# Tomeu7/AO-MARL

Measured on AMD Instinct MI355X. Metric: env steps/sec (AO frames/sec), higher is better.
Workload: dtype f32

## Files before the change

### ao_marl_amd/agents.py

```python
import math
from collections import OrderedDict

import numpy as np
import torch

LOG_SIG_MIN = -20.0


class AgentLayout(object):

    def __init__(self, nmodes, n_zernike_start_end, n_agents_modal, include_tip_tilt=True,
                 window_n_zernike=-1, include_tip_tilt_windowed=False, n_filtered=0,
                 state_keys=("dm_history_2", "dm_history_1", "dm_before_linear", "dm_residual"),
                 state_block=None):
        lo, hi = n_zernike_start_end
        assert lo > -1 and hi > -1 and hi > lo
        total_controlled = hi - lo
        assert total_controlled % n_agents_modal == 0
        local = total_controlled // n_agents_modal
        self.nmodes = nmodes
        self.start = lo
        self.local_controlled_modes = local
        self.agents = OrderedDict()
        wid = 1
        for m in range(lo, hi, local):
            self.agents[wid] = (m, m + local)
            wid += 1
        self.include_tip_tilt = include_tip_tilt
        if include_tip_tilt:
            self.agents[wid] = (nmodes - 2, nmodes)
            total_controlled += 2
        self.total_controlled_modes = total_controlled
        self.n_agents = len(self.agents)
        self.window = window_n_zernike
        self.block = state_block if state_block is not None else \
            (nmodes if window_n_zernike > -1 else total_controlled)
        self.state_keys = tuple(state_keys)
        self.indices_of_state = OrderedDict()
        o = 0
        for k in self.state_keys:
            self.indices_of_state[k] = (o, o + self.block)
            o += self.block
        self.state_dim = o
        if window_n_zernike > -1:
            self.modes_chosen = self._windowed(window_n_zernike, include_tip_tilt_windowed,
                                               n_filtered)
        else:
            self.modes_chosen = self._original()
        self.action_slices = OrderedDict()
        for w, (a, b) in self.agents.items():
            if include_tip_tilt and (a, b) == (nmodes - 2, nmodes):
                self.action_slices[w] = (total_controlled - 2, total_controlled)
            else:
                self.action_slices[w] = (a - lo, b - lo)
        self.action_dim = total_controlled
        self.action_modes = np.r_[np.arange(lo, hi), [nmodes - 2, nmodes - 1]] \
            if include_tip_tilt else np.arange(lo, hi)

    def _original(self):
        out = OrderedDict()
        for w, (a, b) in self.agents.items():
            if self.include_tip_tilt and (a, b) == (self.nmodes - 2, self.nmodes):
                bot, top = self.total_controlled_modes - 2 - self.start, \
                    self.total_controlled_modes - self.start
            else:
                bot, top = a - self.start, b - self.start
            parts = []
            for k, (s0, s1) in self.indices_of_state.items():
                if k in "wfs":
                    parts.append(np.arange(s0, s1))
                else:
                    parts.append(np.arange(s0 + bot, s0 + top))
            out[w] = np.concatenate(parts)
        return out

    def _windowed(self, w_n, tt_windowed, n_filtered):
        out = OrderedDict()
        n_ag = len(self.agents)
        for w, (a, b) in self.agents.items():
            parts = []
            if self.include_tip_tilt and w == n_ag:
                for k, (s0, s1) in self.indices_of_state.items():
                    if k in "wfs":
                        parts.append(np.arange(s0, s1))
                    else:
                        idx = np.arange(s1 - 2, s1)
                        if tt_windowed:
                            idx = np.concatenate([idx, np.arange(0, int(2 * w_n))])
                        parts.append(idx)
                out[w] = np.concatenate(parts)
                break
            for k, (s0, s1) in self.indices_of_state.items():
                if k in "wfs":
                    parts.append(np.arange(s0, s1))
                    continue
                end_point = s1 - (n_filtered - 2)
                length = end_point - s0
                if a - w_n < 0:
                    diff = a - w_n
                    ini, end = 0, b + w_n - diff
                elif b + w_n > length:
                    diff = b + w_n - length
                    ini, end = a - int(w_n) - diff, length
                else:
                    ini, end = a - w_n, b + w_n
                parts.append(np.arange(s0 + ini, s0 + end))
            out[w] = np.concatenate(parts)
        return out

    def state_shapes(self):
        return [len(v) for v in self.modes_chosen.values()]

    def action_shapes(self):
        return [b - a for (a, b) in self.agents.values()]


def _xavier_uniform(gen, fan_out, fan_in, gain=1.0):
    a = gain * math.sqrt(6.0 / (fan_in + fan_out))
    return (torch.rand(fan_out, fan_in, generator=gen) * 2 - 1) * a


class BatchedGaussianPolicy(object):

    def __init__(self, layout, hidden=256, num_layers=2, log_sig_max=2.0, action_scale=1.0,
                 action_bias=0.0, last_layer_zero=True, seed=1234, device="cuda:0"):
        self.layout, self.H, self.L = layout, hidden, num_layers
        self.log_sig_max, self.scale, self.bias = log_sig_max, action_scale, action_bias
        self.device = torch.device(device)
        ins, acts = layout.state_shapes(), layout.action_shapes()
        A, in_max, act_max = layout.n_agents, max(ins), max(acts)
        self.A, self.in_max, self.act_max = A, in_max, act_max
        g = torch.Generator().manual_seed(seed)
        W1 = torch.zeros(A, in_max, hidden)
        Wh = [torch.zeros(A, hidden, hidden) for _ in range(num_layers - 1)]
        Wm, Ws = torch.zeros(A, hidden, act_max), torch.zeros(A, hidden, act_max)
        gather = torch.full((A, in_max), layout.state_dim, dtype=torch.long)
        for i, (w, idx) in enumerate(layout.modes_chosen.items()):
            W1[i, :ins[i], :] = _xavier_uniform(g, hidden, ins[i]).T
            for h in Wh:
                h[i] = _xavier_uniform(g, hidden, hidden).T
            if not last_layer_zero:
                Wm[i, :, :acts[i]] = _xavier_uniform(g, acts[i], hidden).T
                Ws[i, :, :acts[i]] = _xavier_uniform(g, acts[i], hidden).T
            gather[i, :ins[i]] = torch.as_tensor(idx, dtype=torch.long)
        dev = self.device
        self.W1, self.Wh, self.Wm, self.Ws = W1.to(dev), [h.to(dev) for h in Wh], Wm.to(dev), \
            Ws.to(dev)
        self.b1 = torch.zeros(A, 1, hidden, device=dev)
        self.bh = [torch.zeros(A, 1, hidden, device=dev) for _ in range(num_layers - 1)]
        self.bm = torch.zeros(A, 1, act_max, device=dev)
        self.bs = torch.zeros(A, 1, act_max, device=dev)
        self.gather = gather.to(dev)
        ag = torch.zeros(layout.action_dim, dtype=torch.long)
        lo = torch.zeros(layout.action_dim, dtype=torch.long)
        for i, (w, (a, b)) in enumerate(layout.action_slices.items()):
            ag[a:b] = i
            lo[a:b] = torch.arange(b - a)
        self.sc_agent, self.sc_local = ag.to(dev), lo.to(dev)
        self.gen = torch.Generator(device=dev).manual_seed(seed)
        self.gather_i32 = self.gather.to(torch.int32).contiguous()
        self.sc_agent_i32, self.sc_local_i32 = self.sc_agent.to(torch.int32), self.sc_local.to(torch.int32)
        self.seed, self._draws = int(seed), 0
        self._native = None
        self.use_native = self.device.type == "cuda"
        self.native_forward, self._desc = True, None
        self.layer_by_layer = False

    def _refresh_native(self):
        t = lambda w: w.transpose(1, 2).contiguous()
        self._native = dict(
                W1=t(self.W1), b1=self.b1[:, 0].contiguous(),
                Wh=[t(w) for w in self.Wh], bh=[b[:, 0].contiguous() for b in self.bh],
                Whead=torch.cat([t(self.Wm), t(self.Ws)], dim=1).contiguous(),
                bhead=torch.cat([self.bm[:, 0], self.bs[:, 0]], dim=1).contiguous())

    def load_agent(self, i, state_dict):
        ins, acts = self.layout.state_shapes()[i], self.layout.action_shapes()[i]
        with torch.no_grad():
            self.W1[i].zero_()
            self.W1[i, :ins] = state_dict["linear1.weight"].T.to(self.device)
            self.b1[i, 0] = state_dict["linear1.bias"].to(self.device)
            for j in range(self.L - 1):
                self.Wh[j][i] = state_dict["hidden.%d.weight" % j].T.to(self.device)
                self.bh[j][i, 0] = state_dict["hidden.%d.bias" % j].to(self.device)
            self.Wm[i].zero_(); self.Ws[i].zero_()
            self.Wm[i, :, :acts] = state_dict["mean_linear.weight"].T.to(self.device)
            self.Ws[i, :, :acts] = state_dict["log_std_linear.weight"].T.to(self.device)
            self.bm[i, 0, :acts] = state_dict["mean_linear.bias"].to(self.device)
            self.bs[i, 0, :acts] = state_dict["log_std_linear.bias"].to(self.device)
        self._native = None

    def split_states(self, state):
        if self.use_native and not state.requires_grad:
            from . import libaomarl as la
            return la.split_states(state.to(torch.float32), self.gather_i32)
        padded = torch.cat([state, state.new_zeros(state.shape[0], 1)], dim=1)
        return padded[:, self.gather].permute(1, 0, 2).contiguous()

    def _native_head(self, state):
        from . import libaomarl as la
        if self._native is None:
            self._refresh_native()
        n = self._native
        x = self.split_states(state.to(torch.float32))
        x = la.linear_batched(x, n["W1"], n["b1"], relu=True)
        for W, b in zip(n["Wh"], n["bh"]):
            x = la.linear_batched(x, W, b, relu=True)
        return la.linear_batched(x, n["Whead"], n["bhead"], relu=False)

    def _actor_desc(self, nenv):
        from . import libaomarl as la
        import ctypes as C
        if self._native is None:
            self._refresh_native()
        if self._desc is not None and self._desc[0].nenv == nenv and self._desc[4] is self._native and \
                bool(self._desc[0].flags) == self.layer_by_layer:
            return self._desc[0]
        n, A, H = self._native, self.A, self.H
        d = la.ActorDesc()
        d.n_agents, d.nenv, d.state_dim, d.in_max, d.act_max = A, nenv, self.layout.state_dim, \
            self.in_max, self.act_max
        d.hidden, d.n_hidden, d.action_dim = H, self.L, self.layout.action_dim
        z = lambda *sh: torch.empty(*sh, dtype=torch.float32, device=self.device)
        scratch = dict(x=z(A, nenv, self.in_max), h0=z(A, nenv, H), h1=z(A, nenv, H),
                       head=z(A, nenv, 2 * self.act_max))
        nh = max(self.L - 1, 1)
        Wh = (C.c_void_p * nh)(*[w.data_ptr() for w in n["Wh"]])
        bh = (C.c_void_p * nh)(*[b.data_ptr() for b in n["bh"]])
        d.gather, d.W1, d.b1 = self.gather_i32.data_ptr(), n["W1"].data_ptr(), n["b1"].data_ptr()
        d.Wh, d.bh = Wh, bh
        d.Whead, d.bhead = n["Whead"].data_ptr(), n["bhead"].data_ptr()
        d.sc_agent, d.sc_local = self.sc_agent_i32.data_ptr(), self.sc_local_i32.data_ptr()
        d.log_sig_min, d.log_sig_max, d.scale, d.bias = LOG_SIG_MIN, self.log_sig_max, self.scale, self.bias
        for k, t in scratch.items():
            setattr(d, k, t.data_ptr())
        d.flags = la.ACTOR_LAYER_BY_LAYER if self.layer_by_layer else 0
        tiled = None
        if not self.layer_by_layer and H % 16 == 0:
            tiled = dict(W1=la.tile_weights(n["W1"]), Wh=[la.tile_weights(w) for w in n["Wh"]],
                         Whead=la.tile_weights(n["Whead"]))
            tiled["ptrs"] = (C.c_void_p * nh)(*[w.data_ptr() for w in tiled["Wh"]])
            d.W1_tiled, d.Wh_tiled, d.Whead_tiled = tiled["W1"].data_ptr(), tiled["ptrs"], \
                tiled["Whead"].data_ptr()
        self._desc = (d, scratch, Wh, bh, n, tiled)
        return d

    out_ring, _ring, _ring_i = 0, None, 0

    def reset_output_ring(self):
        self._ring_i = 0

    def _select_action_one_call(self, state, eval_mode, eps, out=None):
        from . import libaomarl as la
        import ctypes as C
        nenv = state.shape[0]
        d = self._actor_desc(nenv)
        self._draws += 1
        if self.out_ring:
            if self._ring is None or self._ring[0][0].shape[0] != nenv:
                self._ring = [(torch.empty(nenv, self.layout.action_dim, dtype=torch.float32, device=self.device),
                               torch.empty(nenv, self.layout.action_dim, dtype=torch.float32, device=self.device))
                              for _ in range(self.out_ring)]
                self._ring_i = 0
            a, m = self._ring[self._ring_i]
            self._ring_i = (self._ring_i + 1) % self.out_ring
        else:
            a = torch.empty(nenv, self.layout.action_dim, dtype=torch.float32, device=self.device)
            m = torch.empty_like(a)
        if out is not None:
            if out.shape != a.shape or out.dtype != torch.float32 or not out.is_contiguous() or out.device != a.device:
                raise ValueError("select_action: out must be a contiguous float32 [nenv, action_dim] tensor on the policy's device")
            if eval_mode:
                m = out
            else:
                a = out
        if eps is not None:
            eps = eps.to(torch.float32).contiguous()
        la.check(la.load().aomarl_actor_forward(
                C.byref(d), state.data_ptr(), eps.data_ptr() if eps is not None else None,
                self.seed & 0xFFFFFFFF, self._draws & 0xFFFFFFFF, a.data_ptr(), m.data_ptr(),
                la.raw_stream(self.device)))
        return (m if eval_mode else a), m

    def forward(self, state):
        if self.use_native:
            head = self._native_head(state)
            mean = head[:, :, :self.act_max]
            log_std = head[:, :, self.act_max:].clamp(LOG_SIG_MIN, self.log_sig_max)
            return mean, log_std
        x = self.split_states(state.to(torch.float32))
        x = torch.relu(torch.baddbmm(self.b1, x, self.W1))
        for W, b in zip(self.Wh, self.bh):
            x = torch.relu(torch.baddbmm(b, x, W))
        mean = torch.baddbmm(self.bm, x, self.Wm)
        log_std = torch.baddbmm(self.bs, x, self.Ws).clamp(LOG_SIG_MIN, self.log_sig_max)
        return mean, log_std

    def _assemble(self, per_agent):
        return per_agent[self.sc_agent, :, self.sc_local].T.contiguous()

    def select_action(self, state, eval_mode=False, eps=None, out=None):
        if self.use_native and self.native_forward and state.dtype == torch.float32 and \
                state.dim() == 2 and state.shape[1] == self.layout.state_dim:
            return self._select_action_one_call(state if state.is_contiguous() else state.contiguous(), eval_mode, eps, out)
        a, m = self._select_action(state, eval_mode, eps)
        if out is not None:
            out.copy_(a)
            a = out
        return a, m

    @torch.no_grad()
    def _select_action(self, state, eval_mode=False, eps=None):
        if self.use_native and self.native_forward and state.dtype == torch.float32 and \
                state.dim() == 2 and state.shape[1] == self.layout.state_dim:
            return self._select_action_one_call(state.contiguous(), eval_mode, eps)
        if self.use_native:
            from . import libaomarl as la
            head = self._native_head(state)
            self._draws += 1
            a, m = la.policy_sample(head, self.act_max, self.sc_agent_i32, self.sc_local_i32,
                                    LOG_SIG_MIN, self.log_sig_max, self.scale, self.bias, self.seed,
                                    self._draws, eps=eps)
            return (m if eval_mode else a), m
        mean, log_std = self.forward(state)
        if eps is None:
            e = torch.randn(mean.shape, generator=self.gen, device=self.device)
        else:
            e = torch.zeros_like(mean)
            e[self.sc_agent, :, self.sc_local] = eps.T
        x_t = mean + log_std.exp() * e
        action = torch.tanh(x_t) * self.scale + self.bias
        mu = torch.tanh(mean) * self.scale + self.bias
        a, m = self._assemble(action), self._assemble(mu)
        return (m if eval_mode else a), m


class BatchedQNetwork(object):

    def __init__(self, layout, hidden=256, extra_hidden=0, seed=4321, device="cuda:0"):
        self.layout, self.device = layout, torch.device(device)
        ins, acts = layout.state_shapes(), layout.action_shapes()
        A = layout.n_agents
        self.in_max, self.act_max = max(ins), max(acts)
        g = torch.Generator().manual_seed(seed)
        dev = self.device

        def stack(fan_in_list, fan_out, pad_in):
            W = torch.zeros(A, pad_in, fan_out)
            for i, fi in enumerate(fan_in_list):
                W[i, :fi] = _xavier_uniform(g, fan_out, fi).T
            return W.to(dev)

        self.q = []
        for _ in range(2):
            Win = torch.zeros(A, self.in_max + self.act_max, hidden)
            for i in range(A):
                w = _xavier_uniform(g, hidden, ins[i] + acts[i]).T
                Win[i, :ins[i]] = w[:ins[i]]
                Win[i, self.in_max:self.in_max + acts[i]] = w[ins[i]:]
            hid = [stack([hidden] * A, hidden, hidden) for _ in range(extra_hidden)]
            out = stack([hidden] * A, 1, hidden)
            self.q.append((Win.to(dev), hid, out))

    @torch.no_grad()
    def forward(self, split_state, split_action):
        x = torch.cat([split_state, split_action], dim=2)
        res = []
        for Win, hid, out in self.q:
            h = torch.relu(torch.bmm(x, Win))
            for W in hid:
                h = torch.relu(torch.bmm(h, W))
            res.append(torch.bmm(h, out))
        return res[0], res[1]
```

### ao_marl_amd/csrc/aomarl_capi.hip

```cpp
#include "aomarl_kernels.hip"
#include "aomarl_qf4_host.h"
#include "aomarl_step_plan_host.h"

#include <math.h>
#include <stdlib.h>
#include <stdarg.h>
#include <stdio.h>
#include <string.h>

#include <algorithm>
#include <climits>
#include <string>
#include <vector>

static thread_local char g_err[512] = "";

int fail(const char *fmt, ...) {
  va_list ap;
  va_start(ap, fmt);
  vsnprintf(g_err, sizeof(g_err), fmt, ap);
  va_end(ap);
  return 1;
}


struct aomarl_ctx {
  DevSys sys;
  std::vector<void *> owned;
  int nlayers = 0, ndm = 0;
  int dim[AOMARL_MAX_LAYERS], ns[AOMARL_MAX_LAYERS], abclass[AOMARL_MAX_LAYERS];
  float deltax[AOMARL_MAX_LAYERS], deltay[AOMARL_MAX_LAYERS];
  int nclass = 0;
  int maxdim = 0, maxK = 0;
  float gain = 0.f, delay = 0.f;
  bool spot_fast = false;
  bool force_generic_dm = false, force_valu_target = false;
  bool force_generic_spot = false, force_generic_target = false, force_unfused_frame = false;
  int dft_mode = -1;
  bool reset_untransposed = false;
  int small_chain = 1;
  hipEvent_t ride_ev = nullptr;
  bool rode = false;
  int residual_shortcut = 0;
  int small_move = 1;
  bool small_ok = false;
  int reset_streams = 2;
  bool reset_prefetch_whole = true;
  hipEvent_t ev_reset = nullptr, ev_reset2[3] = {nullptr, nullptr, nullptr};
  bool no_extrude_sg = false;
  bool defer_dm_shape = false;
  int fused_debug = 0;
  bool prefetch_atmos = false, premoved = false;
  bool frame_wait_pending = false;
  bool screens_dirty_main = true;
  float cmat_scale = 1.f, v2m_scale = 1.f, m2v_scale = 1.f, s2m_scale = 1.f, ab_scale[AOMARL_MAX_LAYERS] = {1.f, 1.f, 1.f, 1.f, 1.f, 1.f, 1.f, 1.f};
  bool subpixel_flow = false;
  float frac_x[AOMARL_MAX_LAYERS] = {0, 0, 0, 0, 0, 0, 0, 0}, frac_y[AOMARL_MAX_LAYERS] = {0, 0, 0, 0, 0, 0, 0, 0};
  bool graph_step = false, capturing = false, side_joined = false, fork_recorded = false;
  hipEvent_t ev_fork = nullptr;
  struct StepGraph { std::vector<long long> key; hipGraphExec_t exec; hipGraph_t graph; unsigned long long arith[AR_N]; int fw_variant[6]; };
  std::vector<StepGraph> graphs;
  unsigned long long graph_hits = 0, graph_captures = 0;
  unsigned long long cfg_epoch = 0;
  const int32_t *sel_checked = nullptr;
  int sel_checked_n = 0, sel_checked_nm = 0;
  int fw_variant[6] = {0, 0, 0, 0, 0, 0};
  char fw_name[96] = {0};
  bool time_fw = false;
  std::vector<hipEvent_t> fw_ev;
  size_t fw_ev_used = 0;
  std::vector<hipEvent_t> fw_ev_retired;
  hipStream_t atm_stream = nullptr, psf_stream = nullptr;
  hipEvent_t ev_frame = nullptr, ev_moved = nullptr, ev_psf = nullptr;
  hipEvent_t ev_frame_cur = nullptr;
  bool frame_marked = false;
  struct FramePipe {
    bool have_twin = false, active = false;
    const float *owner_screens = nullptr;
    aomarl_state twin;
    int par = 0;
    hipStream_t fstream = nullptr;
    hipEvent_t ev_cmd = nullptr, ev_commit = nullptr, ev_done[2] = {nullptr, nullptr}, ev_psf[2] = {nullptr, nullptr};
    hipEvent_t ev_done_cur[2] = {nullptr, nullptr};
    bool psf_out[2] = {false, false};
    bool cmd_covers_commit = false;
    bool cmd_covers_psf = false;
    int32_t *snap[2] = {nullptr, nullptr};
    size_t snap_ints = 0;
    unsigned long long steps = 0, overlapped = 0, behind = 0;
  } pipe;
  int32_t *snap_target = nullptr;
  bool snap_complete = false;
  bool pipe_enabled = true;
  bool pipe_internal = false;
  hipEvent_t ev_frame_prev = nullptr;
  bool need_prev = false, group_overlap = false;
  bool psf_side = false;
  const float *pre_screens = nullptr;
  int pre_b = 0, pre_n = 0;
  float *cmat = nullptr;
  int ld_cmat = 0;
  int nmodes = 0, nact = 0, ld_v2m = 0, ld_m2v = 0;
  float *v2m = nullptr, *m2v = nullptr, *freedom = nullptr;
  float *s2m = nullptr;
  int s2m_nmodes = 0;
  int32_t *amodes = nullptr, *amode_inv = nullptr;
  float *env_gain = nullptr;
  int env_gain_n = 0;
  float *mgain = nullptr;
  int mgain_rows = 0, mgain_nm = 0;
  std::vector<float> h_mgain;
  uint32_t *seed_stage = nullptr;
  int seed_stage_n = 0;
  struct ResetPrefetch *rp = nullptr;
  float *timg = nullptr;
  std::vector<int32_t> h_grid;
  std::vector<float> h_prof, h_spupil, h_tt;
  float *geoW = nullptr, *geoUx = nullptr, *geoUy = nullptr, *geoPlanes = nullptr;
  int32_t *geoMap = nullptr;
  int geo_ldw = 0, geo_gw = 0, geo_gh = 0, geo_npzt = 0, geo_ldr = 0;
};

static int pipe_drop(aomarl_ctx *c, void *stream);
static void rp_free(aomarl_ctx *c);
static int fw_ev_rewind(aomarl_ctx *c) {
  const hipEvent_t held[4] = {c->pipe.ev_done_cur[0], c->pipe.ev_done_cur[1], c->ev_frame_cur, c->ev_frame_prev};
  for (size_t i = 0; i < c->fw_ev.size(); i++)
    for (int k = 0; k < 4; k++)
      if (held[k] && c->fw_ev[i] == held[k]) {
        hipEvent_t ne;
        HIPCHK(hipEventCreate(&ne));
        c->fw_ev_retired.push_back(c->fw_ev[i]);
        c->fw_ev[i] = ne;
        break;
      }
  if (c->fw_ev_retired.size() > 64 && !c->pipe.active) {
    bool live = false;
    for (hipEvent_t e : c->fw_ev_retired) for (int k = 0; k < 4; k++) live = live || e == held[k];
    if (!live) { for (hipEvent_t e : c->fw_ev_retired) (void)hipEventDestroy(e); c->fw_ev_retired.clear(); }
  }
  c->fw_ev_used = 0;
  return 0;
}
static int frame_fused_impl(aomarl_ctx *c, aomarl_state *st, int b, int n, int flags, void *stream, int slot);
static int next_part_one_sense(aomarl_ctx *c, aomarl_state *st, int b, int n, float *accumx, float *accumy, int image_flags, void *stream);

static unsigned long long g_cfg_epoch = 0;
const char *aomarl_last_error(void) { return g_err; }
int aomarl_abi_version(void) { return AOMARL_ABI_VERSION; }

int aomarl_set_precision(int mode) {
  g_cfg_epoch++;
  if (mode != AOMARL_PRECISION_F32 && mode != AOMARL_PRECISION_SPLIT_F16) return fail("set_precision: unknown mode %d", mode);
  g_precision = mode;
  g_gemm.split_f16 = mode == AOMARL_PRECISION_SPLIT_F16;
  return 0;
}
int aomarl_get_precision(void) { return g_precision; }
int aomarl_gemm_saturated(unsigned *count, void *stream) {
  if (!count) return fail("gemm_saturated: null argument");
  *count = 0;
  int dev = 0;
  HIPCHK(hipGetDevice(&dev));
  if (dev < 0 || dev >= 64 || !g_gemm_sat[dev]) return 0;
  hipStream_t s = (hipStream_t)stream;
  HIPCHK(hipMemcpyAsync(count, g_gemm_sat[dev], sizeof(unsigned), hipMemcpyDeviceToHost, s));
  HIPCHK(hipStreamSynchronize(s));
  if (*count) HIPCHK(hipMemsetAsync(g_gemm_sat[dev], 0, sizeof(unsigned), s));
  return 0;
}
int aomarl_arith_families(void) { return AR_N; }
const char *aomarl_arith_family_name(int i) { return (i >= 0 && i < AR_N) ? g_arith_name[i] : ""; }
unsigned long long aomarl_arith_launches(int i) { return (i >= 0 && i < AR_N) ? g_arith[i] : 0ULL; }
void aomarl_arith_reset(void) { for (int i = 0; i < AR_N; i++) g_arith[i] = 0ULL; }

template <typename T>
static int upload(aomarl_ctx *c, const T *host, size_t n, T **dev) {
  *dev = nullptr;
  if (n == 0) return 0;
  if (!host) return fail("null host array in descriptor");
  void *p = nullptr;
  HIPCHK(hipMalloc(&p, n * sizeof(T)));
  c->owned.push_back(p);
  HIPCHK(hipMemcpy(p, host, n * sizeof(T), hipMemcpyHostToDevice));
  *dev = (T *)p;
  return 0;
}

static bool is_int(float v) { return floorf(v) == v; }

int aomarl_create(const aomarl_desc *d, aomarl_ctx **out) {
  if (!d || !out) return fail("aomarl_create: null argument");
  if (d->abi_version != AOMARL_ABI_VERSION)
    return fail("aomarl_create: ABI version %d, library is %d", d->abi_version, AOMARL_ABI_VERSION);
  if (d->nlayers < 0 || d->nlayers > AOMARL_MAX_LAYERS) return fail("nlayers out of range");
// ... 684 lines not shown
```

### ao_marl_amd/csrc/aomarl_capi_agents.hip

```cpp
__global__ void k_split_states(int nenv, int state_dim, int in_max, const int32_t *__restrict__ gather,
                               const float *__restrict__ state, float *__restrict__ out) {
  const int a = blockIdx.z, e = blockIdx.y, k = blockIdx.x * blockDim.x + threadIdx.x;
  if (k >= in_max) return;
  const int g = gather[a * in_max + k];
  out[((long long)a * nenv + e) * in_max + k] = g < state_dim ? state[(long long)e * state_dim + g] : 0.f;
}

__global__ void k_policy_sample(int nenv, int act_max, int action_dim, const float *__restrict__ head,
                                float ls_min, float ls_max, float scale, float bias,
                                const int32_t *__restrict__ sc_agent, const int32_t *__restrict__ sc_local,
                                const float *__restrict__ eps_in, uint32_t seed, uint32_t counter,
                                float *__restrict__ action, float *__restrict__ mean) {
  const int e = blockIdx.y, g = blockIdx.x * blockDim.x + threadIdx.x;
  if (g >= action_dim) return;
  const int a = sc_agent[g], l = sc_local[g];
  const float *h = head + ((long long)a * nenv + e) * (2 * act_max);
  const float m = h[l];
  const float ls = fminf(fmaxf(h[act_max + l], ls_min), ls_max);
  const float eps = eps_in ? eps_in[(long long)e * action_dim + g]
                           : philox_normal(seed, 7u, counter, (uint32_t)e, (uint32_t)g);
  const float x = m + expf(ls) * eps;
  action[(long long)e * action_dim + g] = tanhf(x) * scale + bias;
  mean[(long long)e * action_dim + g] = tanhf(m) * scale + bias;
}

struct ActorArgs {
  int A, nenv, state_dim, in_max, act_max, H, n_hidden, action_dim;
  const int32_t *gather;
  const float *W1, *b1, *Wh[8], *bh[8], *Whead, *bhead;
  const int32_t *sc_agent, *sc_local;
  float ls_min, ls_max, scale, bias;
  const float *state, *eps;
  uint32_t seed, counter;
  float *action, *mean;
};

__global__ void k_actor_tile_weights(int N, int K, int ntile, int ksteps, const float *__restrict__ src,
                                     float *__restrict__ dst) {
  const long long per = (long long)ntile * ksteps * 256;
  const long long i = (long long)blockIdx.x * blockDim.x + threadIdx.x;
  if (i >= per) return;
  const int a = blockIdx.y;
  const int jj = (int)(i & 3), lane = (int)((i >> 2) & 63);
  const long long t = i >> 8;
  const int sidx = (int)(t % ksteps), n = (int)(t / ksteps);
  const int row = 16 * n + (lane & 15), col = 16 * sidx + 4 * (lane >> 4) + jj;
  dst[(long long)a * per + i] = (row < N && col < K) ? src[((long long)a * N + row) * K + col] : 0.f;
}

__device__ __forceinline__ int af_at(int row, int col) {
  return (((col >> 4) * 64 + ((col >> 2) & 3) * 16 + row) << 2) + (col & 3);
}

__device__ __forceinline__ void af_layer(const float *__restrict__ Xs, int ksteps, const float *__restrict__ W,
                                         const float *__restrict__ b, int N, bool relu, float *__restrict__ Out) {
  const int lane = threadIdx.x & 63, wave = threadIdx.x >> 6, r = lane & 15, kk = lane >> 4;
  const int ntile = (N + 15) / 16, npairs = (ntile + 1) / 2;
  constexpr int D = 2;
  for (int pair = wave; pair < npairs; pair += 8) {
    const float4 *wa = reinterpret_cast<const float4 *>(W) + (long long)(2 * pair) * ksteps * 64 + lane;
    const float4 *wb = reinterpret_cast<const float4 *>(W) + (long long)min(2 * pair + 1, ntile - 1) * ksteps * 64 + lane;
    const float4 *xs = reinterpret_cast<const float4 *>(Xs) + lane;
    f32x4 acc0 = {0.f, 0.f, 0.f, 0.f}, acc1 = {0.f, 0.f, 0.f, 0.f};
    auto fma8 = [&](const float4 x, const float4 a, const float4 c) {
      acc0 = __builtin_amdgcn_mfma_f32_16x16x4f32(x.x, a.x, acc0, 0, 0, 0);
      acc1 = __builtin_amdgcn_mfma_f32_16x16x4f32(x.x, c.x, acc1, 0, 0, 0);
      acc0 = __builtin_amdgcn_mfma_f32_16x16x4f32(x.y, a.y, acc0, 0, 0, 0);
      acc1 = __builtin_amdgcn_mfma_f32_16x16x4f32(x.y, c.y, acc1, 0, 0, 0);
      acc0 = __builtin_amdgcn_mfma_f32_16x16x4f32(x.z, a.z, acc0, 0, 0, 0);
      acc1 = __builtin_amdgcn_mfma_f32_16x16x4f32(x.z, c.z, acc1, 0, 0, 0);
      acc0 = __builtin_amdgcn_mfma_f32_16x16x4f32(x.w, a.w, acc0, 0, 0, 0);
      acc1 = __builtin_amdgcn_mfma_f32_16x16x4f32(x.w, c.w, acc1, 0, 0, 0);
    };
    float4 ra[D], rb[D], qa[D], qb[D];
    auto fill = [&](float4 (&a)[D], float4 (&c)[D], int s0) {
#pragma unroll
      for (int u = 0; u < D; u++) {
        const int st = min(s0 + u, ksteps - 1) * 64;
        a[u] = wa[st]; c[u] = wb[st];
      }
    };
    auto drain = [&](const float4 (&a)[D], const float4 (&c)[D], int s0) {
#pragma unroll
      for (int u = 0; u < D; u++) fma8(xs[(s0 + u) * 64], a[u], c[u]);
    };
    fill(ra, rb, 0);
    int s = 0;
    for (; s + 2 * D <= ksteps; s += 2 * D) {
      fill(qa, qb, s + D);
      __builtin_amdgcn_sched_barrier(0);
      drain(ra, rb, s);
      __builtin_amdgcn_sched_barrier(0);
      fill(ra, rb, s + 2 * D);
      __builtin_amdgcn_sched_barrier(0);
      drain(qa, qb, s + D);
      __builtin_amdgcn_sched_barrier(0);
    }
    fill(qa, qb, s + D);
    __builtin_amdgcn_sched_barrier(0);
#pragma unroll
    for (int u = 0; u < D; u++)
      if (s + u < ksteps) fma8(xs[(s + u) * 64], ra[u], rb[u]);
#pragma unroll
    for (int u = 0; u < D; u++)
      if (s + D + u < ksteps) fma8(xs[(s + D + u) * 64], qa[u], qb[u]);
    const int ca = 32 * pair + r, cb = ca + 16;
    const float ba = (b && ca < N) ? b[ca] : 0.f, bb = (b && cb < N) ? b[cb] : 0.f;
#pragma unroll
    for (int t = 0; t < 4; t++) {
      float va = acc0[t] + ba, vb = acc1[t] + bb;
      if (relu) { va = fmaxf(va, 0.f); vb = fmaxf(vb, 0.f); }
      if (ca < N) Out[af_at(4 * kk + t, ca)] = va;
      if (cb < N) Out[af_at(4 * kk + t, cb)] = vb;
    }
  }
}

__global__ __launch_bounds__(512) void k_actor_fused(ActorArgs p) {
  extern __shared__ __attribute__((aligned(16))) float af_lds[];
  const int tiles = (p.nenv + 15) / 16;
  const int q = blockIdx.x & 7, idx = blockIdx.x >> 3;
  const int a = q + 8 * (idx / tiles), e0 = (idx % tiles) * 16;
  if (a >= p.A) return;
  const int tid = threadIdx.x;
  const int H = p.H, no = 2 * p.act_max;
  const int ks1 = (p.in_max + 15) / 16, ksh = H / 16, nth = H / 16, nto = (no + 15) / 16;
  const int img1 = 256 * max(ksh, nto), img0 = max(256 * ks1, img1);
  float *R0 = af_lds, *R1 = af_lds + img0;
  int *alist = reinterpret_cast<int *>(af_lds + img0 + img1);
  if (tid == 0) alist[0] = 0;
  __syncthreads();
  for (int g = tid; g < p.action_dim; g += 512)
    if (p.sc_agent[g] == a) alist[1 + atomicAdd(&alist[0], 1)] = g;
  for (int k = tid; k < 16 * ks1; k += 512) {
    const int g = k < p.in_max ? p.gather[a * p.in_max + k] : p.state_dim;
    const bool col = g < p.state_dim;
    const float *src = p.state + (col ? g : 0);
    float v[16];
#pragma unroll
    for (int r = 0; r < 16; r++) v[r] = src[(long long)min(e0 + r, p.nenv - 1) * p.state_dim];
#pragma unroll
    for (int r = 0; r < 16; r++) R0[af_at(r, k)] = (col && e0 + r < p.nenv) ? v[r] : 0.f;
  }
  __syncthreads();
  af_layer(R0, ks1, p.W1 + (long long)a * nth * ks1 * 256, p.b1 + (long long)a * H, H, true, R1);
  __syncthreads();
  float *cur = R1, *nxt = R0;
  for (int l = 0; l + 1 < p.n_hidden; l++) {
    af_layer(cur, ksh, p.Wh[l] + (long long)a * nth * ksh * 256, p.bh[l] + (long long)a * H, H, true, nxt);
    __syncthreads();
    float *t = cur; cur = nxt; nxt = t;
  }
  af_layer(cur, ksh, p.Whead + (long long)a * nto * ksh * 256, p.bhead + (long long)a * no, no, false, nxt);
  __syncthreads();
  const int r = tid & 15, e = e0 + r;
  if (e >= p.nenv) return;
  const int nact = min(alist[0], p.act_max);
  for (int i = tid >> 4; i < nact; i += 32) {
    const int g = alist[1 + i];
    const int l = p.sc_local[g];
    const float m = nxt[af_at(r, l)];
    const float ls = fminf(fmaxf(nxt[af_at(r, p.act_max + l)], p.ls_min), p.ls_max);
    const float eps = p.eps ? p.eps[(long long)e * p.action_dim + g]
                            : philox_normal(p.seed, 7u, p.counter, (uint32_t)e, (uint32_t)g);
    const float x = m + expf(ls) * eps;
    p.action[(long long)e * p.action_dim + g] = tanhf(x) * p.scale + p.bias;
    p.mean[(long long)e * p.action_dim + g] = tanhf(m) * p.scale + p.bias;
  }
}

struct StateBlocks {
  const float *src[8], *mean[8], *std[8];
  int ld[8], dim[8], off[8];
  int nblocks, total;
  const int32_t *sel;
  const float *part; int nsplit, pn; float alpha; float *sum_out;
};

__global__ void k_assemble_state(int nenv, StateBlocks sb, float *__restrict__ out) {
  const int e = blockIdx.y, j = blockIdx.x * blockDim.x + threadIdx.x;
  auto psum = [&](int col) {
    return sb.alpha * slab_sum<4>(sb.nsplit, [&](int z) { return sb.part[((long long)z * nenv + e) * sb.pn + col]; });
  };
  if (j >= sb.total) {
    const int col = j - sb.total;
    if (sb.part && col < sb.pn) sb.sum_out[(long long)e * sb.pn + col] = psum(col);
    return;
  }
  int b = 0;
#pragma unroll
  for (int k = 1; k < 8; k++) if (k < sb.nblocks && j >= sb.off[k]) b = k;
  const int i = j - sb.off[b];
  const int col = sb.sel ? sb.sel[i] : i;
  float v = (sb.part && b == sb.nblocks - 1) ? psum(col) : sb.src[b][(long long)e * sb.ld[b] + col];
  if (sb.mean[b]) v = (v - sb.mean[b][i]) / sb.std[b][i];
  out[(long long)e * sb.total + j] = v;
}

__global__ void k_agent_rewards(int nenv, int nmodes, int n_agents, const float *__restrict__ res, int ld,
                                const int32_t *__restrict__ lohi, float factor, float *__restrict__ out) {
  const int e = blockIdx.y, a = blockIdx.x, lane = threadIdx.x;
  const int lo = lohi[2 * a], hi = lohi[2 * a + 1];
  float s = 0.f;
  for (int m = lo + lane; m < hi; m += 64) { const float v = res[(long long)e * ld + m]; s += v * v; }
  s = wave_sum(s);
  if (lane == 0) out[(long long)e * n_agents + a] = -factor * s / (float)(hi - lo);
}

int aomarl_split_states(int nenv, int state_dim, int n_agents, int in_max, const int32_t *gather,
                        const float *state, float *out, void *stream) {
  if (!gather || !state || !out) return fail("split_states: null pointer");
  if (nenv <= 0 || n_agents <= 0 || in_max <= 0) return 0;
  hipLaunchKernelGGL(k_split_states, dim3((in_max + 255) / 256, nenv, n_agents), dim3(256), 0,
                     (hipStream_t)stream, nenv, state_dim, in_max, gather, state, out);
  LAUNCHCHK();
  return 0;
}

int aomarl_policy_sample(int nenv, int act_max, int action_dim, const float *head, float log_sig_min,
                         float log_sig_max, float scale, float bias, const int32_t *sc_agent,
                         const int32_t *sc_local, const float *eps, uint32_t seed, uint32_t counter,
                         float *action, float *mean, void *stream) {
  if (!head || !sc_agent || !sc_local || !action || !mean) return fail("policy_sample: null pointer");
  if (nenv <= 0 || action_dim <= 0) return 0;
  hipLaunchKernelGGL(k_policy_sample, dim3((action_dim + 255) / 256, nenv), dim3(256), 0,
                     (hipStream_t)stream, nenv, act_max, action_dim, head, log_sig_min, log_sig_max, scale,
                     bias, sc_agent, sc_local, eps, seed, counter, action, mean);
  LAUNCHCHK();
  return 0;
}

static int state_blocks_fill(int nblocks, const float *const *src, const int32_t *ld, const int32_t *dim,
                             const float *const *mean, const float *const *std_, const int32_t *sel, StateBlocks *out) {
  if (!src || !ld || !dim) return fail("assemble_state: null pointer");
  if (nblocks < 1 || nblocks > 8) return fail("assemble_state: 1..8 blocks");
  StateBlocks &sb = *out;
  int off = 0;
  for (int k = 0; k < 8; k++) {
    const bool on = k < nblocks;
    sb.src[k] = on ? src[k] : nullptr; sb.ld[k] = on ? ld[k] : 0; sb.dim[k] = on ? dim[k] : 0;
    sb.mean[k] = (on && mean) ? mean[k] : nullptr; sb.std[k] = (on && std_) ? std_[k] : nullptr;
    sb.off[k] = off;
    if (on) {
      if (!src[k] || dim[k] <= 0 || (!sel && ld[k] < dim[k])) return fail("assemble_state: bad block %d", k);
      if ((sb.mean[k] == nullptr) != (sb.std[k] == nullptr)) return fail("assemble_state: mean/std must come together");
      off += dim[k];
    }
  }
  sb.nblocks = nblocks; sb.total = off; sb.sel = sel;
  sb.part = nullptr; sb.nsplit = 0; sb.pn = 0; sb.alpha = 1.f; sb.sum_out = nullptr;
  return 0;
}

struct AssemblePart { const float *part; int nsplit, pn; float alpha; float *sum_out; };
static int assemble_state_impl(int nenv, int nblocks, const float *const *src, const int32_t *ld,
                               const int32_t *dim, const float *const *mean, const float *const *std_,
                               const int32_t *sel, float *out, void *stream, const AssemblePart *pt = nullptr);

int aomarl_assemble_state(int nenv, int nblocks, const float *const *src, const int32_t *ld,
                          const int32_t *dim, const float *const *mean, const float *const *std_,
                          float *out, void *stream) {
  return assemble_state_impl(nenv, nblocks, src, ld, dim, mean, std_, nullptr, out, stream);
}

int aomarl_assemble_state_cols(int nenv, int nblocks, const float *const *src, const int32_t *ld,
                               const int32_t *dim, const float *const *mean, const float *const *std_,
                               const int32_t *sel, float *out, void *stream) {
  return assemble_state_impl(nenv, nblocks, src, ld, dim, mean, std_, sel, out, stream);
}

static int assemble_state_impl(int nenv, int nblocks, const float *const *src, const int32_t *ld,
                               const int32_t *dim, const float *const *mean, const float *const *std_,
                               const int32_t *sel, float *out, void *stream, const AssemblePart *pt) {
  if (!out) return fail("assemble_state: null pointer");
  StateBlocks sb;
  int rc = state_blocks_fill(nblocks, src, ld, dim, mean, std_, sel, &sb);
  if (rc) return rc;
  int extra = 0;
  if (pt && pt->part && pt->nsplit > 0) {
    sb.part = pt->part; sb.nsplit = pt->nsplit; sb.pn = pt->pn; sb.alpha = pt->alpha; sb.sum_out = pt->sum_out;
    extra = pt->pn;
  }
  if (nenv <= 0) return 0;
  hipLaunchKernelGGL(k_assemble_state, dim3((sb.total + extra + 255) / 256, nenv), dim3(256), 0, (hipStream_t)stream,
                     nenv, sb, out);
  LAUNCHCHK();
  return 0;
}

int aomarl_agent_rewards(int nenv, int nmodes, int n_agents, const float *res_modes, int ld,
                         const int32_t *lohi, float factor, float *out, void *stream) {
  if (!res_modes || !lohi || !out) return fail("agent_rewards: null pointer");
  if (ld < nmodes) return fail("agent_rewards: ld < nmodes");
  if (nenv <= 0 || n_agents <= 0) return 0;
  hipLaunchKernelGGL(k_agent_rewards, dim3(n_agents, nenv), dim3(64), 0, (hipStream_t)stream, nenv, nmodes,
                     n_agents, res_modes, ld, lohi, factor, out);
  LAUNCHCHK();
  return 0;
}
```

### ao_marl_amd/csrc/aomarl_capi_stages.hip

```cpp
static int dm_shape_impl(aomarl_ctx *c, aomarl_state *st, int b, int n, const float *volts,
                         bool skip_stack, void *stream) {
  const float *v = volts ? volts : st->voltage + (size_t)b * st->ld_actu;
  const int ldv = volts ? c->sys.nactu : st->ld_actu;
  DevState ds = dev_state(st);
  for (int k = 0; k < c->ndm; k++) {
    const DevDm &D = c->sys.dms[k];
    const int np = D.dim * D.dim;
    if (D.type == AOMARL_DM_TT)
      hipLaunchKernelGGL(k_dm_shape, dim3(1, n), dim3(64), 0, (hipStream_t)stream, c->sys, ds, b, k, v, ldv);
    else if (skip_stack)
      continue;
    else if (D.sep && !c->force_generic_dm)
      hipLaunchKernelGGL(k_dm_shape_sep, dim3((D.dim + DMS_TX - 1) / DMS_TX, (D.dim + DMS_TY - 1) / DMS_TY, n),
                         dim3(256), 0, (hipStream_t)stream, c->sys, ds, b, k, v, ldv);
    else
      hipLaunchKernelGGL(k_dm_shape, dim3((np + 255) / 256, n), dim3(256), 0, (hipStream_t)stream, c->sys, ds, b, k, v, ldv);
    LAUNCHCHK();
  }
  return 0;
}

int aomarl_comp_dm_shape(aomarl_ctx *c, aomarl_state *st, int b, int n, const float *volts, void *stream) {
  int rc = check_range(c, st, b, n);
  if (rc) return rc;
  if (n == 0) return 0;
  return dm_shape_impl(c, st, b, n, volts, false, stream);
}

int aomarl_dm_from_voltage_available(aomarl_ctx *c) {
  return c && c->sys.fused_ok && c->sys.otf_ok && !c->force_unfused_frame ? 1 : 0;
}

int aomarl_get_dm_shape(aomarl_ctx *c, aomarl_state *st, int b, int n, int k, float *dst, void *stream) {
  int rc = check_range(c, st, b, n);
  if (rc) return rc;
  if (k < 0 || k >= c->ndm || !dst) return fail("get_dm_shape: bad argument");
  if (n == 0) return 0;
  hipLaunchKernelGGL(k_get_dm_shape, dim3(256, n), dim3(256), 0, (hipStream_t)stream, c->sys, dev_state(st), b, k, dst);
  LAUNCHCHK();
  return 0;
}

int aomarl_set_option(aomarl_ctx *c, const char *name, int value) {
  if (!name) return fail("set_option: null argument");
  g_cfg_epoch++;
  if (c) c->cfg_epoch++;
  if (!strcmp(name, "gemm_kgroups")) {
    if (value != 0 && value != 1 && value != 2 && value != 4) return fail("gemm_kgroups: 0, 1, 2 or 4");
    g_gemm_kgroups = value;
    return 0;
  }
  if (!strcmp(name, "gemm_xcd_map")) { g_gemm.xcd = value != 0; return 0; }
  if (!strcmp(name, "gemm_target_blocks")) { g_gemm.target_blocks = value > 0 ? value : 0; return 0; }
  if (!strcmp(name, "gemm_split_f16")) { g_gemm.split_f16 = value != 0; return 0; }
  if (!strcmp(name, "precision")) return aomarl_set_precision(value);
  if (!c) return fail("set_option: null context");
  if (!strcmp(name, "force_generic_dm")) { c->force_generic_dm = value != 0; return 0; }
  if (!strcmp(name, "force_valu_target")) { c->force_valu_target = value != 0; return 0; }
  if (!strcmp(name, "defer_dm_shape")) { c->defer_dm_shape = value != 0; return 0; }
  if (!strcmp(name, "frame_pipeline")) {
    if (c->pipe.active) return fail("frame_pipeline: a frame is in flight (reset first)");
    c->pipe_enabled = value != 0; return 0;
  }
  if (!strcmp(name, "small_move")) { c->small_move = value != 0; return 0; }
  if (!strcmp(name, "small_chain")) { c->small_chain = value != 0; return 0; }
  if (!strcmp(name, "renew_frame_stream")) {
    auto &P = c->pipe;
    if (P.active) return fail("renew_frame_stream: a frame is in flight (reset first)");
    if (P.fstream) {
      HIPCHK(hipStreamSynchronize(P.fstream));
      HIPCHK(hipStreamDestroy(P.fstream));
      P.fstream = nullptr;
      HIPCHK(hipStreamCreateWithFlags(&P.fstream, hipStreamNonBlocking));
    }
    return 0;
  }
  if (!strcmp(name, "residual_shortcut")) {
    if (value && (!c->s2m || c->s2m_nmodes < 1)) return fail("residual_shortcut: no v2m . cmat matrix (aomarl_set_slopes2modes)");
    c->residual_shortcut = value != 0;
    return 0;
  }
  if (!strcmp(name, "reset_streams")) { c->reset_streams = value < 1 ? 1 : (value > 4 ? 4 : value); return 0; }
  if (!strcmp(name, "reset_prefetch_whole")) { c->reset_prefetch_whole = value != 0; return 0; }
  if (!strcmp(name, "extrude_unfused")) { c->no_extrude_sg = value != 0; return 0; }
  if (!strcmp(name, "reset_untransposed")) { c->reset_untransposed = value != 0; return 0; }
  if (!strcmp(name, "time_frame_kernel")) {
    c->time_fw = value > 0;
    { const int rrc = fw_ev_rewind(c); if (rrc) return rrc; }
    while (c->fw_ev.size() < 2 * (size_t)std::max(value, 0)) {
      hipEvent_t e;
      HIPCHK(hipEventCreate(&e));
      c->fw_ev.push_back(e);
    }
    return 0;
  }
  if (!strcmp(name, "prefetch_atmos")) { c->prefetch_atmos = value != 0; return 0; }
  if (!strcmp(name, "subpixel_flow")) { c->subpixel_flow = value != 0; return 0; }
  if (!strcmp(name, "graph_step")) { c->graph_step = value != 0; return 0; }
  if (!strcmp(name, "fused_debug")) { c->fused_debug = value; return 0; }
  if (!strcmp(name, "force_f32_dft")) { c->dft_mode = value < 0 ? -1 : (value != 0 ? 0 : 1); return 0; }
  if (!strcmp(name, "force_unfused_frame")) { c->force_unfused_frame = value != 0; return 0; }
  if (!strcmp(name, "force_generic_spot")) { c->force_generic_spot = value != 0; return 0; }
  if (!strcmp(name, "force_generic_target")) { c->force_generic_target = value != 0; return 0; }
  return fail("set_option: unknown option %s", name);
}

static DevSys traced_sys(const aomarl_ctx *c) {
  DevSys sy = c->sys;
  if (c->subpixel_flow)
    for (int l = 0; l < c->nlayers; l++) {
      sy.layers[l].wxo += c->frac_x[l]; sy.layers[l].txo += c->frac_x[l];
      sy.layers[l].wyo += c->frac_y[l]; sy.layers[l].tyo += c->frac_y[l];
    }
  return sy;
}

int aomarl_raytrace_wfs(aomarl_ctx *c, aomarl_state *st, int b, int n, int flags, void *stream) {
  int rc = check_range(c, st, b, n);
  if (rc) return rc;
  rc = atmos_wait_pending(c, stream);
  if (rc) return rc;
  if (!st->wfs_phase) return fail("raytrace_wfs needs st->wfs_phase");
  if (n == 0) return 0;
  const int np = c->sys.n * c->sys.n;
  hipLaunchKernelGGL(k_raytrace<false>, dim3((np + 255) / 256, n), dim3(256), 0, (hipStream_t)stream, traced_sys(c), dev_state(st), b, flags);
  LAUNCHCHK();
  return 0;
}

int aomarl_raytrace_target(aomarl_ctx *c, aomarl_state *st, int b, int n, int flags, void *stream) {
  int rc = check_range(c, st, b, n);
  if (rc) return rc;
  rc = atmos_wait_pending(c, stream);
  if (rc) return rc;
  if (!st->tar_phase) return fail("raytrace_target needs st->tar_phase");
  if (n == 0) return 0;
  const int np = c->sys.pupdiam * c->sys.pupdiam;
  hipLaunchKernelGGL(k_raytrace<true>, dim3((np + 255) / 256, n), dim3(256), 0, (hipStream_t)stream, traced_sys(c), dev_state(st), b, flags);
  LAUNCHCHK();
  return 0;
}

__global__ void k_inc_u32(uint32_t *p, int n) {
  int i = blockIdx.x * blockDim.x + threadIdx.x;
  if (i < n) p[i] += 1u;
}

int aomarl_comp_image(aomarl_ctx *c, aomarl_state *st, int b, int n, int flags, void *stream) {
  int rc = check_range(c, st, b, n);
  if (rc) return rc;
  rc = atmos_wait_pending(c, stream);
  if (rc) return rc;
  if (n == 0) return 0;
  const bool from_buf = flags & AOMARL_IMG_FROM_PHASE_BUFFER;
  const bool noise = (flags & AOMARL_IMG_NOISE) && c->sys.noise >= 0.f;
  const bool cube = flags & AOMARL_IMG_WRITE_BINCUBE;
  const int cog = (flags & AOMARL_IMG_COG) ? 1 : 0;
  if (from_buf && !st->wfs_phase) return fail("comp_image: FROM_PHASE_BUFFER needs st->wfs_phase");
  if (!from_buf && !c->sys.wfs_all_int)
    return fail("comp_image: fused raytrace needs integer layer offsets; use raytrace_wfs + FROM_PHASE_BUFFER");
  if (cube && !st->bincube) return fail("comp_image: WRITE_BINCUBE needs st->bincube");
  if (!cube && !cog) return fail("comp_image: nothing to produce (neither bincube nor slopes)");
  const int na = (flags & AOMARL_IMG_NO_ATMOS) ? 1 : 0, nd = (flags & AOMARL_IMG_NO_DMS) ? 1 : 0;
  hipStream_t s = (hipStream_t)stream;
  DevState ds = dev_state(st);
  int gx = (16384 + 4 * n - 1) / (4 * n);
  gx = std::max(1, std::min(gx, (c->sys.nvalid + 3) / 4));
  dim3 grid(gx, n), blk(256);
#define SPOT(FB, NZ, WC) hipLaunchKernelGGL((k_wfs_spot<FB, NZ, WC>), grid, blk, 0, s, c->sys, ds, b, na, nd, cog)
#define FAST(NL, NZ, WC) hipLaunchKernelGGL((k_wfs_spot_fast<NL, NZ, WC>), grid, blk, 0, s, c->sys, ds, b, cog)
  const bool fast_ok = !from_buf && !na && !nd && !c->force_generic_spot && c->ndm == 2 &&
                       c->sys.dms[0].type == AOMARL_DM_PZT && c->sys.dms[1].type == AOMARL_DM_TT &&
                       (c->nlayers == 1 || c->nlayers == 3);
  if (fast_ok) {
    if (c->nlayers == 1) {
      if (noise) { if (cube) FAST(1, true, true); else FAST(1, true, false); }
      else { if (cube) FAST(1, false, true); else FAST(1, false, false); }
    } else {
      if (noise) { if (cube) FAST(3, true, true); else FAST(3, true, false); }
      else { if (cube) FAST(3, false, true); else FAST(3, false, false); }
    }
  } else if (from_buf) {
    if (noise) { if (cube) SPOT(true, true, true); else SPOT(true, true, false); }
    else { if (cube) SPOT(true, false, true); else SPOT(true, false, false); }
  } else {
    if (noise) { if (cube) SPOT(false, true, true); else SPOT(false, true, false); }
    else { if (cube) SPOT(false, false, true); else SPOT(false, false, false); }
  }
#undef SPOT
#undef FAST
  LAUNCHCHK();
  hipLaunchKernelGGL(k_inc_u32, dim3((n + 255) / 256), dim3(256), 0, s, st->frame + b, n);
  LAUNCHCHK();
  return 0;
}

int aomarl_do_centroids(aomarl_ctx *c, aomarl_state *st, int b, int n, void *stream) {
  int rc = check_range(c, st, b, n);
  if (rc) return rc;
  if (!st->bincube) return fail("do_centroids needs st->bincube");
  if (n == 0) return 0;
  hipLaunchKernelGGL(k_cog, dim3((c->sys.nvalid + 3) / 4, n), dim3(256), 0, (hipStream_t)stream, c->sys, dev_state(st), b);
  LAUNCHCHK();
  return 0;
}

int aomarl_slopes_geom(aomarl_ctx *c, aomarl_state *st, int b, int n, void *stream) {
  int rc = check_range(c, st, b, n);
  if (rc) return rc;
  if (!st->wfs_phase) return fail("slopes_geom needs st->wfs_phase");
  if (n == 0) return 0;
  hipLaunchKernelGGL(k_slopes_geom, dim3((c->sys.nvalid + 3) / 4, n), dim3(256), 0, (hipStream_t)stream, c->sys, dev_state(st), b);
  LAUNCHCHK();
  return 0;
}

__global__ void k_mgain_scale(float *__restrict__ modes, int ldm, int nm, float gain, const float *__restrict__ env_gain,
                              const float *__restrict__ mgain, int mg_rows, int env_begin) {
// ... 331 lines not shown
```

### ao_marl_amd/csrc/aomarl_capi_step.hip

```cpp
long long aomarl_actor_tiled_floats(int n_agents, int N, int K) {
  return (long long)n_agents * ((N + 15) / 16) * ((K + 15) / 16) * 256;
}

int aomarl_actor_tile_weights(int n_agents, int N, int K, const float *src, float *dst, void *stream) {
  if (!src || !dst) return fail("actor_tile_weights: null pointer");
  if (n_agents <= 0 || N <= 0 || K <= 0) return fail("actor_tile_weights: bad sizes");
  const int ntile = (N + 15) / 16, ksteps = (K + 15) / 16;
  const long long per = (long long)ntile * ksteps * 256;
  hipLaunchKernelGGL(k_actor_tile_weights, dim3((unsigned)((per + 255) / 256), n_agents), dim3(256), 0,
                     (hipStream_t)stream, N, K, ntile, ksteps, src, dst);
  LAUNCHCHK();
  return 0;
}

int aomarl_actor_forward(const aomarl_actor_desc *d, const float *state, const float *eps, uint32_t seed,
                         uint32_t counter, float *action, float *mean, void *stream) {
  if (!d || !state || !action || !mean) return fail("actor_forward: null argument");
  if (d->n_hidden < 1 || d->n_hidden > 8) return fail("actor_forward: 1..8 hidden layers");
  const int A = d->n_agents, n = d->nenv, H = d->hidden;
  if (A <= 0 || n <= 0) return 0;
  if (!(d->flags & AOMARL_ACTOR_LAYER_BY_LAYER) && d->W1_tiled && d->Whead_tiled && H % 16 == 0) {
    const int ks1 = (d->in_max + 15) / 16, nto = (2 * d->act_max + 15) / 16;
    const size_t img1 = (size_t)256 * std::max(H / 16, nto), img0 = std::max((size_t)256 * ks1, img1);
    const size_t lds = (img0 + img1 + d->act_max + 4) * sizeof(float);
    static bool big_lds = false;
    if (!big_lds && lds > 64 * 1024 && lds <= 128 * 1024) {
      HIPCHK(hipFuncSetAttribute(reinterpret_cast<const void *>(k_actor_fused), hipFuncAttributeMaxDynamicSharedMemorySize, 128 * 1024));
      big_lds = true;
    }
    if (lds <= 128 * 1024) {
      ActorArgs p;
      p.A = A; p.nenv = n; p.state_dim = d->state_dim; p.in_max = d->in_max; p.act_max = d->act_max; p.H = H;
      p.n_hidden = d->n_hidden; p.action_dim = d->action_dim;
      p.gather = d->gather; p.W1 = d->W1_tiled; p.b1 = d->b1;
      for (int l = 0; l < 8; l++) {
        p.Wh[l] = l + 1 < d->n_hidden ? d->Wh_tiled[l] : nullptr;
        p.bh[l] = l + 1 < d->n_hidden ? d->bh[l] : nullptr;
        if (l + 1 < d->n_hidden && !p.Wh[l]) return fail("actor_forward: tiled hidden weights missing");
      }
      if (((uintptr_t)p.W1 | (uintptr_t)d->Whead_tiled) & 15) return fail("actor_forward: tiled weights must be 16-byte aligned");
      p.Whead = d->Whead_tiled; p.bhead = d->bhead; p.sc_agent = d->sc_agent; p.sc_local = d->sc_local;
      p.ls_min = d->log_sig_min; p.ls_max = d->log_sig_max; p.scale = d->scale; p.bias = d->bias;
      p.state = state; p.eps = eps; p.seed = seed; p.counter = counter; p.action = action; p.mean = mean;
      const int tiles = (n + 15) / 16, groups = (A + 7) / 8;
      hipLaunchKernelGGL(k_actor_fused, dim3(8 * tiles * groups), dim3(512), lds, (hipStream_t)stream, p);
      g_arith[AR_ACTOR_F32]++;
      LAUNCHCHK();
      return 0;
    }
  }
  if (!d->x || !d->h0 || !d->h1 || !d->head) return fail("actor_forward: the layer-by-layer path needs its scratch buffers");
  int rc = aomarl_split_states(n, d->state_dim, A, d->in_max, d->gather, state, d->x, stream);
  if (rc) return rc;
  rc = aomarl_gemm_nt_batched(A, n, H, d->in_max, d->x, d->in_max, (long long)n * d->in_max, d->W1, d->in_max,
                              (long long)H * d->in_max, d->b1, H, d->h0, H, (long long)n * H, 1, stream);
  if (rc) return rc;
  float *cur = d->h0, *nxt = d->h1;
  for (int l = 0; l + 1 < d->n_hidden; l++) {
    rc = aomarl_gemm_nt_batched(A, n, H, H, cur, H, (long long)n * H, d->Wh[l], H, (long long)H * H, d->bh[l], H,
                                nxt, H, (long long)n * H, 1, stream);
    if (rc) return rc;
    std::swap(cur, nxt);
  }
  const int no = 2 * d->act_max;
  rc = aomarl_gemm_nt_batched(A, n, no, H, cur, H, (long long)n * H, d->Whead, H, (long long)no * H, d->bhead, no,
                              d->head, no, (long long)n * no, 0, stream);
  if (rc) return rc;
  return aomarl_policy_sample(n, d->act_max, d->action_dim, d->head, d->log_sig_min, d->log_sig_max, d->scale,
                              d->bias, d->sc_agent, d->sc_local, eps, seed, counter, action, mean, stream);
}

static int env_step_validate(aomarl_ctx *c, aomarl_state *st, aomarl_env_glue *g, const float *action, float *state_out,
                             float *reward_out) {
  if (!c || !st || !g || !state_out) return fail("env_step: null argument");
  if (g->nhist < 0 || g->nhist > 5) return fail("env_step: 0..5 command histories");
  const int n = st->nenv, nm = g->nmodes, R = g->nhist + 1;
  if (g->ring_pos < 0 || g->ring_pos >= R) return fail("env_step: ring position out of range");
  int rc = check_range(c, st, 0, n);
  if (rc) return rc;
  if (!c->v2m || !c->m2v) return fail("env_step: no modal basis (aomarl_set_modal)");
  if (nm != c->nmodes) return fail("env_step: glue has %d modes, the basis %d", nm, c->nmodes);
  if (action && c->nact <= 0) return fail("env_step: no action modes set");
  if (!g->modes_ring || !g->res_modes) return fail("env_step: glue->modes_ring / glue->res_modes are null");
  if (reward_out && (g->n_agents <= 0 || !g->lohi)) return fail("env_step: reward_out needs glue->n_agents > 0 and glue->lohi");
  if (g->dm_dim <= 0 || g->dm_dim > nm || (!g->sel && g->dm_dim != nm))
    return fail("env_step: glue->dm_dim = %d does not fit %d modes%s", g->dm_dim, nm, g->sel ? "" : " (no column selection given)");
  if ((g->mean_dm || g->std_dm || g->mean_res || g->std_res) && !(g->mean_dm && g->std_dm && g->mean_res && g->std_res))
    return fail("env_step: standardisation needs all of mean_dm, std_dm, mean_res, std_res (or none)");
  if (c->env_gain)
    return fail("env_step: per-environment integrator gains are set on this context (aomarl_set_env_gains); env_step "
                "takes ONE scalar gain -- clear them (aomarl_set_env_gains(ctx, NULL, 0)) or step call by call");
  if (g->sel && (c->sel_checked != g->sel || c->sel_checked_n != g->dm_dim || c->sel_checked_nm != nm)) {
    std::vector<int32_t> h((size_t)g->dm_dim);
    HIPCHK(hipDeviceSynchronize());
    HIPCHK(hipMemcpy(h.data(), g->sel, sizeof(int32_t) * h.size(), hipMemcpyDeviceToHost));
    for (size_t i = 0; i < h.size(); i++)
      if (h[i] < 0 || h[i] >= nm) return fail("env_step: glue->sel[%zu] = %d is outside the %d modes", i, h[i], nm);
    c->sel_checked = g->sel; c->sel_checked_n = g->dm_dim; c->sel_checked_nm = nm;
  }
  return 0;
}

template <class F>
__device__ __forceinline__ void small_gemv(const float *__restrict__ W, int ldw, int no, int K, const float *xs, F done) {
  const int tid = threadIdx.x, q = tid & 3, per = blockDim.x >> 2;
  for (int o0 = 0; o0 < no; o0 += per) {
    const int o = o0 + (tid >> 2);
    float a0 = 0.f, a1 = 0.f;
    if (o < no) {
      const float *row = W + (long long)o * ldw;
      int k = q;
      for (; k + 28 < K; k += 32) {
        float r[8];
#pragma unroll
        for (int u = 0; u < 8; u++) r[u] = row[k + 4 * u];
#pragma unroll
        for (int u = 0; u < 8; u += 2) { a0 = fmaf(xs[k + 4 * u], r[u], a0); a1 = fmaf(xs[k + 4 * u + 4], r[u + 1], a1); }
      }
      for (; k + 4 < K; k += 8) { a0 = fmaf(xs[k], row[k], a0); a1 = fmaf(xs[k + 4], row[k + 4], a1); }
      if (k < K) a0 = fmaf(xs[k], row[k], a0);
    }
    float y = a0 + a1;
    y += __shfl_xor(y, 1);
    y += __shfl_xor(y, 2);
    if (o < no && q == 0) done(o, y);
  }
}
struct SmallHead {
  int nm, na, nact, n_agents, ld_m2v, ld_actu, ktt, do_strehl;
  float gain, factor, wa, wb, wc;
  const float *m0, *m1, *action, *freedom, *m2v, *PEND;
  const int32_t *amode_inv, *lohi;
  float *modes_out, *rew;
};
__global__ __launch_bounds__(256) void k_small_head(DevSys sys, DevState st, SmallHead p) {
  __shared__ float sm[SMALL_NM], sv[SMALL_NA];
  const int e = blockIdx.x, tid = threadIdx.x, lane = tid & 63, wv = tid >> 6;
  for (int m = tid; m < p.nm; m += 256) {
    float v = p.m0[(long long)e * p.nm + m] + p.gain * p.m1[(long long)e * p.nm + m];
    if (p.action) {
      const int j = p.amode_inv[m];
      if (j >= 0) v += p.action[(long long)e * p.nact + j] * p.freedom[m];
    }
    sm[m] = v;
    if (p.modes_out) p.modes_out[(long long)e * p.nm + m] = v;
  }
  if (p.rew)
    for (int a = wv; a < p.n_agents; a += 4) {
      const int lo = p.lohi[2 * a], hi = p.lohi[2 * a + 1];
      float q = 0.f;
      for (int m = lo + lane; m < hi; m += 64) { const float v = p.m1[(long long)e * p.nm + m]; q += v * v; }
      q = wave_sum(q);
      if (lane == 0) p.rew[(long long)e * p.n_agents + a] = -p.factor * q / (float)(hi - lo);
    }
  __syncthreads();
  small_gemv(p.m2v, p.ld_m2v, p.na, p.nm, sm, [&](int a, float c0) {
    const long long o = (long long)e * p.ld_actu + a;
    const float c1 = st.com1[o], c2 = st.com2[o];
    const float v = p.wa * c0 + p.wb * c1 + p.wc * c2;
    st.com[o] = c0; st.voltage[o] = v; st.com2[o] = c1; st.com1[o] = c0;
    sv[a] = v;
  });
  __syncthreads();
  if (p.ktt >= 0 && tid < 3) {
    const DevDm &D = sys.dms[p.ktt];
    float *shape = st.dm_shape + (long long)e * sys.shape_stride + D.shape_off;
    if (tid < 2) shape[tid] = sv[D.com_off + tid];
    if (tid == 2 && sys.fused_ok) {
      const DevDm &Z = sys.dms[0];
      const int half = sys.pupdiam / 2, zp = (half + Z.toy) * Z.dim + half + Z.tox;
      const int ss2 = Z.ss * Z.ss, s0 = Z.influstart[zp], cn = Z.ninflu[zp];
      float acc = 0.f;
      for (int t = 0; t < cn; t++) {
        const int pos = Z.influpos[s0 + t];
        acc += Z.influ[pos] * sv[Z.com_off + pos / ss2];
      }
      shape[2] = acc;
    }
  }
  if (p.do_strehl) strehl_commit_body(sys, st, 0, e, p.PEND);
}

struct SmallTail {
  int nsl, na, nm, ld_cmat, ld_v2m, ld_actu;
  float gain;
  const float *cmat, *v2m;
  float *res_modes;
};
__global__ __launch_bounds__(256) void k_small_tail(DevState st, SmallTail p, StateBlocks sb, float *__restrict__ out) {
  __shared__ float ss[SMALL_NSL], se[SMALL_NA], sr[SMALL_NM];
  const int e = blockIdx.x, tid = threadIdx.x;
  for (int k = tid; k < p.nsl; k += 256) ss[k] = st.slopes[(long long)e * p.nsl + k];
  __syncthreads();
  small_gemv(p.cmat, p.ld_cmat, p.na, p.nsl, ss, [&](int a, float acc) {
    const float v = -acc;
    const long long o = (long long)e * p.ld_actu + a;
    st.err[o] = v;
    st.com[o] += p.gain * v;
    se[a] = v;
  });
  __syncthreads();
  small_gemv(p.v2m, p.ld_v2m, p.nm, p.na, se, [&](int m, float acc) {
    p.res_modes[(long long)e * p.nm + m] = acc;
    sr[m] = acc;
  });
  __syncthreads();
  for (int j = tid; j < sb.total; j += 256) {
    int b = 0;
#pragma unroll
    for (int k = 1; k < 8; k++) if (k < sb.nblocks && j >= sb.off[k]) b = k;
    const int i = j - sb.off[b];
    const int col = sb.sel ? sb.sel[i] : i;
    float v = (b == sb.nblocks - 1) ? sr[col] : sb.src[b][(long long)e * sb.ld[b] + col];
    if (sb.mean[b]) v = (v - sb.mean[b][i]) / sb.std[b][i];
    out[(long long)e * sb.total + j] = v;
  }
}

static StepFacts step_facts(aomarl_ctx *c, const aomarl_state *st, const aomarl_env_glue *g, const float *accumx,
                            const float *accumy) {
  StepFacts f;
  int ntt = 0, nother = 0;
  f.ktt = -1;
  for (int k = 0; k < c->ndm; k++) {
    if (c->sys.dms[k].type == AOMARL_DM_TT) { f.ktt = k; ntt++; } else nother++;
  }
  f.unfused = (g->flags & AOMARL_ENV_STEP_UNFUSED) != 0;
  f.one_tt = ntt == 1; f.no_other_dm = nother == 0;
  f.defer_shape = c->defer_dm_shape && aomarl_dm_from_voltage_available(c);
  f.mgain = c->mgain != nullptr; f.env_gain = c->env_gain != nullptr;
  f.small_opt = c->small_chain != 0;
  f.nactu = c->sys.nactu; f.nslope = c->sys.nslope; f.nmodes = g->nmodes;
  f.cmat = c->cmat != nullptr;
  f.shortcut_opt = c->residual_shortcut != 0;
  f.s2m_match = c->s2m && c->s2m_nmodes == g->nmodes;
  f.denoiser = g->denoiser != nullptr;
  const auto &P = c->pipe;
  f.twin = P.have_twin; f.pipe_opt = c->pipe_enabled; f.owner = st && P.owner_screens == st->screens;
  f.prefetch = c->prefetch_atmos; f.delay_one = c->delay == 1.f; f.noiseless = c->sys.noise < 0.f;
  f.accum = accumx && accumy; f.subpixel = c->subpixel_flow; f.frame_fused = aomarl_frame_fused_available(c) != 0;
  f.in_flight = P.active && f.owner;
  f.graph_step = c->graph_step; f.capturing = c->capturing;
  return f;
}

static int env_step_head_fused(aomarl_ctx *c, aomarl_state *st, aomarl_state *stv, aomarl_env_glue *g, const float *action,
                               float gain, float *reward_out, HeadKind head, int ktt, bool ahead, hipEvent_t psf_ev, void *stream) {
  hipStream_t s = (hipStream_t)stream;
  const int n = st->nenv, nm = g->nmodes, R = g->nhist + 1, na = c->sys.nactu;
  const size_t slot = (size_t)n * nm;
  float *newest = g->modes_ring + (size_t)g->ring_pos * slot;
  float *mnew = g->modes_ring + (size_t)((g->ring_pos + 1) % R) * slot;
  Work w = work_layout(c, st->nenv);
  DevState dsv = dev_state(stv);
  const DelayWeights dw = delay_weights(c->delay, ahead);
  if (head == HEAD_SMALL) {
    SmallHead p;
    p.wa = dw.wa; p.wb = dw.wb; p.wc = dw.wc;
    p.nm = nm; p.na = na; p.nact = c->nact; p.n_agents = reward_out ? g->n_agents : 0; p.ld_m2v = c->ld_m2v;
    p.ld_actu = st->ld_actu; p.ktt = ktt; p.do_strehl = 1; p.gain = gain; p.factor = g->reward_factor;
    p.m0 = newest; p.m1 = g->res_modes; p.action = action; p.freedom = c->freedom; p.m2v = c->m2v;
    p.PEND = stv->work + w.PEND; p.amode_inv = c->amode_inv; p.lohi = g->lohi; p.modes_out = mnew; p.rew = reward_out;
    if (psf_ev) HIPCHK(hipStreamWaitEvent(s, psf_ev, 0));
    else if (stv == st) { int rc = psf_wait_pending(c, stream); if (rc) return rc; }
    hipExtLaunchKernelGGL(k_small_head, dim3(n), dim3(256), 0, s, nullptr, ahead ? c->pipe.ev_cmd : nullptr, 0, c->sys, dsv, p);
    LAUNCHCHK();
    if (ahead) c->pipe.cmd_covers_commit = true;
    return 0;
  }
  float *modes = st->work + w.MODES;
  const int cx = (nm + 255) / 256;
  bool psf_waited = false;
  if (ahead && psf_ev) { HIPCHK(hipStreamWaitEvent(s, psf_ev, 0)); psf_waited = true; }
  hipLaunchKernelGGL(k_compose_rewards, dim3(cx + (reward_out ? g->n_agents : 0), n), dim3(256), 0, s, nm, newest,
                     g->res_modes, gain, action, c->nact, c->amode_inv, c->freedom, modes, w.ldm, mnew, cx,
                     g->n_agents, g->lohi, g->reward_factor, reward_out);
  LAUNCHCHK();
  GemmArgs ga(n, na, nm, 1.0f, modes, w.ldm, c->m2v, c->ld_m2v, 0.0f, st->com, st->ld_actu, s);
  ga.ws = st->work + w.GEMM; ga.ws_floats = w.gemm_floats; ga.slabs_only = true; ga.min_chunk = 288;
  ga.fast = true; ga.sa = 16.f; ga.sb = c->m2v_scale;
  const GemmDone gd = launch_gemm_nt(ga);
  const int nsp = gd.slabs;
  const float alpha = gd.slab_alpha;
  LAUNCHCHK();
  if (ahead) {
    hipExtLaunchKernelGGL(k_delay_ahead, dim3((na + 255) / 256, 2 * n), dim3(256), 0, s, nullptr, c->pipe.ev_cmd, 0, c->sys, dsv, na,
                          st->ld_actu, n, nsp > 0 ? st->work + w.GEMM : nullptr, nsp, alpha, ktt);
    LAUNCHCHK();
    c->pipe.cmd_covers_psf = psf_waited;
  } else {
    if (nsp > 0)
      hipLaunchKernelGGL(k_delay_sum, dim3((na + 255) / 256, n), dim3(256), 0, s, dsv, na, st->ld_actu, dw.wa, dw.wb, dw.wc, 0, 1,
                         st->work + w.GEMM, nsp, alpha, n);
    else
      hipLaunchKernelGGL(k_delay, dim3((na + 255) / 256, n), dim3(256), 0, s, dsv, na, st->ld_actu, dw.wa, dw.wb, dw.wc, 0, 1);
    LAUNCHCHK();
  }
  if (psf_ev) { if (!psf_waited) HIPCHK(hipStreamWaitEvent(s, psf_ev, 0)); }
  else if (stv == st) { int rc = psf_wait_pending(c, stream); if (rc) return rc; }
  hipLaunchKernelGGL(k_post_delay, dim3(ahead ? n : 2 * n), dim3(256), 0, s, c->sys, dsv, 0, n, stv->work + w.PEND, 1, ktt,
                     stv->voltage, st->ld_actu);
  LAUNCHCHK();
  if (ahead) { HIPCHK(hipEventRecord(c->pipe.ev_commit, s)); c->pipe.cmd_covers_commit = false; }
  return 0;
}

struct StepBlocks {
  const float *src[8], *mean[8], *sd[8];
  int32_t ld[8], dim[8];
  int nb;
  bool norm;
};
static StepBlocks step_blocks(const aomarl_env_glue *g, int n, int nxt) {
  const int nm = g->nmodes, R = g->nhist + 1;
  const size_t slot = (size_t)n * nm;
  StepBlocks B;
  B.nb = 0;
  auto add = [&](const float *src, const float *mean, const float *sd) {
    B.src[B.nb] = src; B.mean[B.nb] = mean; B.sd[B.nb] = sd; B.ld[B.nb] = nm; B.dim[B.nb] = g->dm_dim; B.nb++;
  };
  for (int h = g->nhist; h >= 1; h--) add(g->modes_ring + (size_t)((nxt - h + R * 8) % R) * slot, g->mean_dm, g->std_dm);
  add(g->modes_ring + (size_t)nxt * slot, g->mean_dm, g->std_dm);
  add(g->res_modes, g->mean_res, g->std_res);
  B.norm = g->mean_dm && g->std_dm && g->mean_res && g->std_res;
  return B;
}

static int tail_slab_product(aomarl_ctx *c, aomarl_state *st, aomarl_env_glue *g, int K, float alpha, const float *A, int lda,
                             const float *B, int ldb, float scale_b, hipStream_t s, AssemblePart *part) {
  const int n = st->nenv, nm = g->nmodes;
  Work w = work_layout(c, n);
  GemmArgs ga(n, nm, K, alpha, A, lda, B, ldb, 0.0f, g->res_modes, nm, s);
  ga.ws = st->work + w.GEMM; ga.ws_floats = w.gemm_floats; ga.slabs_only = true; ga.min_chunk = 288;
  ga.fast = true; ga.sb = scale_b;
  const GemmDone gd = launch_gemm_nt(ga);
  LAUNCHCHK();
  if (gd.slabs > 0) *part = {st->work + w.GEMM, gd.slabs, nm, gd.slab_alpha, g->res_modes};
  return 0;
}

static int env_step_tail(aomarl_ctx *c, aomarl_state *st, aomarl_env_glue *g, TailKind kind, aomarl_state *view,
                         float *state_out, void *stream) {
  hipStream_t s = (hipStream_t)stream;
  const int n = st->nenv, nm = g->nmodes, na = c->sys.nactu, nsl = c->sys.nslope;
  const int nxt = (g->ring_pos + 1) % (g->nhist + 1);
  int rc = 0;
  if (tail_runs_do_control(kind)) {
    rc = aomarl_do_control(c, view, 0, n, stream);
    if (rc) return rc;
  }
  const StepBlocks B = step_blocks(g, n, nxt);
  const float *const *mean = B.norm ? B.mean : nullptr, *const *sd = B.norm ? B.sd : nullptr;
  AssemblePart part = {nullptr, 0, 0, 1.f, nullptr};
  switch (kind) {
  case TAIL_SMALL: {
    StateBlocks sb;
    rc = state_blocks_fill(B.nb, B.src, B.ld, B.dim, mean, sd, g->sel, &sb);
    if (rc) return rc;
    SmallTail p;
    p.nsl = nsl; p.na = na; p.nm = nm; p.ld_cmat = c->ld_cmat; p.ld_v2m = c->ld_v2m; p.ld_actu = st->ld_actu;
    p.gain = c->gain; p.cmat = c->cmat; p.v2m = c->v2m; p.res_modes = g->res_modes;
    hipLaunchKernelGGL(k_small_tail, dim3(n), dim3(256), 0, s, dev_state(view), p, sb, state_out);
    LAUNCHCHK();
    g->ring_pos = nxt;
    return 0;
  }
  case TAIL_SHORTCUT:
    rc = tail_slab_product(c, st, g, nsl, -1.0f, view->slopes, nsl, c->s2m, c->ld_cmat, c->s2m_scale, s, &part);
    break;
  case TAIL_FUSED:
    rc = tail_slab_product(c, st, g, na, 1.0f, st->err, st->ld_actu, c->v2m, c->ld_v2m, c->v2m_scale, s, &part);
    break;
  case TAIL_STAGES:
    rc = aomarl_volts2modes(c, st, n, st->err, st->ld_actu, g->res_modes, stream);
    break;
  }
  if (rc) return rc;
  rc = assemble_state_impl(n, B.nb, B.src, B.ld, B.dim, mean, sd, g->sel, state_out, stream, &part);
  if (rc) return rc;
  g->ring_pos = nxt;
  return 0;
}

static int env_step_body(aomarl_ctx *c, aomarl_state *st, aomarl_env_glue *g, const float *action, float gain,
                         float *accumx, float *accumy, float *state_out, float *reward_out, const StepFacts &f,
                         const StepPlan &plan, void *stream) {
  int rc = env_step_validate(c, st, g, action, state_out, reward_out);
  if (rc) return rc;
  const int n = st->nenv, nm = g->nmodes, R = g->nhist + 1;
  const size_t slot = (size_t)n * nm;
  float *newest = g->modes_ring + (size_t)g->ring_pos * slot;
  float *mnew = g->modes_ring + (size_t)((g->ring_pos + 1) % R) * slot;
  if (plan.head != HEAD_STAGES) {
    rc = env_step_head_fused(c, st, st, g, action, gain, reward_out, plan.head, f.ktt, false, nullptr, stream);
    if (rc) return rc;
  } else {
    rc = aomarl_rl_control_modes(c, st, 0, n, newest, g->res_modes, gain, action, mnew, stream);
    if (rc) return rc;
    rc = aomarl_apply_control(c, st, 0, n, AOMARL_APPLY_COMP_VOLTAGE | (c->defer_dm_shape ? AOMARL_APPLY_DEFER_STACK_SHAPE : 0), stream);
    if (rc) return rc;
    rc = aomarl_comp_strehl(c, st, 0, n, stream);
    if (rc) return rc;
    if (reward_out) {
      rc = aomarl_agent_rewards(n, nm, g->n_agents, g->res_modes, nm, g->lohi, g->reward_factor, reward_out, stream);
      if (rc) return rc;
    }
  }
  if (plan.sense == SENSE_DENOISER) {
    if (!st->bincube) return fail("env_step: the denoiser needs st->bincube");
    if (!aomarl_frame_fused_available(c)) return fail("env_step: denoiser branch needs the one-pass frame kernel");
    rc = aomarl_move_atmos(c, st, 0, n, accumx, accumy, stream);
    if (rc) return rc;
    const bool defer = c->defer_dm_shape && aomarl_dm_from_voltage_available(c);
    rc = aomarl_frame_fused(c, st, 0, n, AOMARL_IMG_NOISE | AOMARL_IMG_WRITE_BINCUBE | (defer ? AOMARL_IMG_DM_FROM_VOLTAGE : 0), stream);
    if (rc) return rc;
    const long long nimg = (long long)n * c->sys.nvalid;
    rc = g->denoiser_f32 ? aomarl_denoiser_apply_f32((aomarl_denoiser *)g->denoiser, st->bincube, nimg, stream)
                         : aomarl_denoiser_apply_split_f16((aomarl_denoiser *)g->denoiser, st->bincube, nimg, stream);
    if (rc) return rc;
    if (c->prefetch_atmos && !c->premoved) {
      rc = aomarl_prefetch_atmos(c, st, 0, n, accumx, accumy, stream);
      if (rc) return rc;
    }
    rc = aomarl_do_centroids(c, st, 0, n, stream);
  } else {
    rc = next_part_one_sense(c, st, 0, n, accumx, accumy, 0, stream);
  }
  if (rc) return rc;
  return env_step_tail(c, st, g, plan.tail, st, state_out, stream);
}

static aomarl_state pipe_view(aomarl_ctx *c, const aomarl_state *st, int par) {
  aomarl_state v = *st;
  if (par) {
    v.slopes = c->pipe.twin.slopes; v.voltage = c->pipe.twin.voltage; v.dm_shape = c->pipe.twin.dm_shape;
    v.work = c->pipe.twin.work;
  }
  return v;
}

static int pipe_init(aomarl_ctx *c, const aomarl_state *st) {
  auto &P = c->pipe;
  int rc = side_stream(c);
  if (rc) return rc;
  if (!P.fstream) {
    HIPCHK(hipStreamCreateWithFlags(&P.fstream, hipStreamNonBlocking));
    HIPCHK(hipEventCreateWithFlags(&P.ev_cmd, hipEventDisableTiming));
    HIPCHK(hipEventCreateWithFlags(&P.ev_commit, hipEventDisableTiming));
    for (int k = 0; k < 2; k++) {
      HIPCHK(hipEventCreateWithFlags(&P.ev_done[k], hipEventDisableTiming));
      HIPCHK(hipEventCreateWithFlags(&P.ev_psf[k], hipEventDisableTiming));
    }
  }
  const size_t ints = (size_t)st->nenv * c->nlayers * 2;
  if (P.snap_ints < ints) {
    for (int k = 0; k < 2; k++) {
      if (P.snap[k]) (void)hipFree(P.snap[k]);
      P.snap[k] = nullptr;
      HIPCHK(hipMalloc((void **)&P.snap[k], sizeof(int32_t) * ints));
    }
    P.snap_ints = ints;
  }
  return 0;
}

static int pipe_launch_frame(aomarl_ctx *c, aomarl_state *st, int q, void *stream) {
  auto &P = c->pipe;
  (void)stream;
  HIPCHK(hipStreamWaitEvent(P.fstream, P.ev_cmd, 0));
  if (!c->premoved || c->pre_screens != st->screens || c->pre_b != 0 || c->pre_n != st->nenv)
    return fail("frame pipeline: no prefetched atmosphere frame of the whole batch is pending");
  HIPCHK(hipStreamWaitEvent(P.fstream, c->ev_moved, 0));
  c->premoved = false;
  aomarl_state v = pipe_view(c, st, q);
  v.origin = P.snap[q];
  return frame_fused_impl(c, &v, 0, st->nenv, AOMARL_IMG_COG | AOMARL_IMG_NOISE | AOMARL_IMG_DM_FROM_VOLTAGE,
                          (void *)P.fstream, q);
}

static int pipe_prefetch(aomarl_ctx *c, aomarl_state *st, float *accumx, float *accumy, int older, int newest) {
  auto &P = c->pipe;
  if (c->premoved) return fail("frame pipeline: a prefetched frame is already pending");
  c->side_joined = false;
  c->ev_frame_prev = P.ev_done_cur[older]; c->need_prev = true;
  c->ev_frame_cur = P.ev_done_cur[newest]; c->frame_wait_pending = true;
  c->snap_target = P.snap[older]; c->snap_complete = true;
  c->ride_ev = c->ev_moved; c->rode = false;
  int rc = move_atmos_now(c, st, 0, st->nenv, accumx, accumy, (void *)c->atm_stream);
  c->ride_ev = nullptr;
  const bool complete = c->snap_complete;
  c->snap_target = nullptr;
  if (!rc && !complete && c->need_prev && c->frame_wait_pending)
    rc = hipStreamWaitEvent(c->atm_stream, c->ev_frame_prev, 0) == hipSuccess ? 0 : fail("frame pipeline: hipStreamWaitEvent failed");
  c->ev_frame_prev = nullptr; c->need_prev = false; c->frame_wait_pending = false; c->group_overlap = false;
  if (rc) return rc;
  if (!complete)
    HIPCHK(hipMemcpyAsync(P.snap[older], st->origin, sizeof(int32_t) * (size_t)st->nenv * c->nlayers * 2,
                          hipMemcpyDeviceToDevice, c->atm_stream));
  c->screens_dirty_main = false;
  if (!(c->rode && complete)) HIPCHK(hipEventRecord(c->ev_moved, c->atm_stream));
  c->premoved = true; c->pre_screens = st->screens; c->pre_b = 0; c->pre_n = st->nenv;
  return 0;
}

static int env_step_pipelined(aomarl_ctx *c, aomarl_state *st, aomarl_env_glue *g, const float *action, float gain,
                              float *accumx, float *accumy, float *state_out, float *reward_out, const StepFacts &f,
                              const StepPlan &plan, void *stream) {
  auto &P = c->pipe;
  hipStream_t s = (hipStream_t)stream;
  const int n = st->nenv, ktt = f.ktt;
  if (!P.active) {
    int rc = env_step_body(c, st, g, action, gain, accumx, accumy, state_out, reward_out, f, plan, stream);
    if (rc) return rc;
    if (!c->premoved || !c->psf_side) return 0;
    rc = pipe_init(c, st);
    if (rc) return rc;
    P.ev_done_cur[0] = c->ev_frame_cur;
    HIPCHK(hipEventRecord(P.ev_psf[0], c->psf_stream));
    P.psf_out[0] = true; P.psf_out[1] = false;
    c->psf_side = false;
    aomarl_state v1 = pipe_view(c, st, 1);
    HIPCHK(hipMemcpyAsync(v1.voltage, st->com1, sizeof(float) * (size_t)n * st->ld_actu, hipMemcpyDeviceToDevice, s));
    Work w = work_layout(c, st->nenv);
    hipLaunchKernelGGL(k_post_delay, dim3(2 * n), dim3(256), 0, s, c->sys, dev_state(&v1), 0, n, v1.work + w.PEND, 0, ktt,
                       v1.voltage, st->ld_actu);
    LAUNCHCHK();
    HIPCHK(hipEventRecord(P.ev_cmd, s));
    HIPCHK(hipEventRecord(P.ev_commit, s));
    P.cmd_covers_commit = false;
    HIPCHK(hipMemcpyAsync(P.snap[1], st->origin, sizeof(int32_t) * (size_t)n * c->nlayers * 2, hipMemcpyDeviceToDevice,
                          c->atm_stream));
    HIPCHK(hipEventRecord(c->ev_moved, c->atm_stream));
    c->pipe_internal = true;
    rc = pipe_launch_frame(c, st, 1, stream);
    if (!rc) rc = pipe_prefetch(c, st, accumx, accumy, 0, 1);
    c->pipe_internal = false;
    if (rc) return rc;
    P.active = true; P.par = 1;
    return 0;
  }
  const int p = P.par, q = 1 - p;
  c->pipe_internal = true;
  int rc = env_step_validate(c, st, g, action, state_out, reward_out);
  aomarl_state vq = pipe_view(c, st, q), vp = pipe_view(c, st, p);
  hipEvent_t pe = P.psf_out[q] ? P.ev_psf[q] : nullptr;
  if (!rc) rc = env_step_head_fused(c, st, &vq, g, action, gain, reward_out, plan.head, ktt, true, pe, stream);
  if (!rc && pe && !P.cmd_covers_commit && !P.cmd_covers_psf && hipStreamWaitEvent(P.fstream, pe, 0) != hipSuccess) rc = fail("frame pipeline: hipStreamWaitEvent failed");
  if (!rc) { P.psf_out[q] = false; P.cmd_covers_psf = false; rc = pipe_launch_frame(c, st, q, stream); }
  if (!rc) rc = pipe_prefetch(c, st, accumx, accumy, p, q);
  if (!rc && hipStreamWaitEvent(s, P.ev_done_cur[p], 0) != hipSuccess) rc = fail("frame pipeline: hipStreamWaitEvent failed");
  if (!rc) rc = env_step_tail(c, st, g, plan.tail, &vp, state_out, stream);
  c->pipe_internal = false;
  if (rc) return rc;
  P.par = q; P.steps++;
  return 0;
}

static int pipe_drop(aomarl_ctx *c, void *stream) {
  auto &P = c->pipe;
  hipStream_t s = (hipStream_t)stream;
  if (P.ev_done_cur[P.par]) HIPCHK(hipStreamWaitEvent(s, P.ev_done_cur[P.par], 0));
  for (int k = 0; k < 2; k++)
    if (P.psf_out[k]) { HIPCHK(hipStreamWaitEvent(s, P.ev_psf[k], 0)); P.psf_out[k] = false; }
  P.active = false; P.par = 0;
  return 0;
}

int aomarl_set_frame_pipeline(aomarl_ctx *c, const aomarl_state *st, const aomarl_state *twin) {
  if (!c) return fail("set_frame_pipeline: null context");
  auto &P = c->pipe;
  if (P.active) return fail("set_frame_pipeline: a frame is in flight (reset first)");
  if (!twin) { P.have_twin = false; P.owner_screens = nullptr; return 0; }
  if (!st) return fail("set_frame_pipeline: null state");
  int rc = check_range(c, st, 0, st->nenv);
  if (rc) return rc;
  if (twin->nenv != st->nenv || twin->ld_actu != st->ld_actu) return fail("set_frame_pipeline: the twin's nenv / ld_actu differ");
  if (twin->screens != st->screens || twin->origin != st->origin || twin->seeds != st->seeds || twin->ext_count != st->ext_count ||
      twin->com != st->com || twin->com1 != st->com1 || twin->com2 != st->com2 || twin->err != st->err ||
      twin->strehl != st->strehl || twin->le_img != st->le_img || twin->frame != st->frame)
    return fail("set_frame_pipeline: the twin must share every buffer of the state except slopes, voltage, dm_shape, work");
  if (!twin->slopes || !twin->voltage || !twin->dm_shape || !twin->work || twin->slopes == st->slopes ||
      twin->voltage == st->voltage || twin->dm_shape == st->dm_shape || twin->work == st->work)
    return fail("set_frame_pipeline: the twin needs slopes, voltage, dm_shape and work buffers of its own");
  P.twin = *twin; P.have_twin = true; P.owner_screens = st->screens;
  return 0;
}

int aomarl_frame_pipeline_state(aomarl_ctx *c, int *in_flight, int *consumed_in_twin, unsigned long long *steps,
                                unsigned long long *overlapped) {
  if (!c) return fail("frame_pipeline_state: null context");
  if (in_flight) *in_flight = c->pipe.active ? 1 : 0;
  if (consumed_in_twin) *consumed_in_twin = c->pipe.active ? (1 - c->pipe.par) : 0;
  if (steps) *steps = c->pipe.steps;
  if (overlapped) *overlapped = c->pipe.overlapped;
  return 0;
}



static bool step_plan_uniform(const aomarl_ctx *c, int n, const float *accumx, const float *accumy, Plan &p) {
  const int nl = c->nlayers;
  for (int e = 0; e < n; e++)
    for (int l = 0; l < nl; l++) {
      const int kx = (int)(accumx[(size_t)e * nl + l] + c->deltax[l]), ky = (int)(accumy[(size_t)e * nl + l] + c->deltay[l]);
      if (e == 0) { p.kx[l] = kx; p.ky[l] = ky; }
      else if (p.kx[l] != kx || p.ky[l] != ky) return false;
    }
  return true;
}

int aomarl_policy_env_step(aomarl_ctx *c, aomarl_state *st, aomarl_env_glue *g, const aomarl_actor_desc *d,
                           const float *state, const float *eps, uint32_t seed, uint32_t counter, float gain,
                           float *accumx, float *accumy, float *action, float *mean, float *state_out,
                           float *reward_out, void *stream) {
  if (!c || !st || !g || !d || !state || !action || !mean || !state_out) return fail("policy_env_step: null argument");
  if (d->nenv != st->nenv) return fail("policy_env_step: the actors are set up for %d environments, the state has %d", d->nenv, st->nenv);
  int rc = aomarl_actor_forward(d, state, eps, seed, counter, action, mean, stream);
  if (rc) return rc;
  return aomarl_env_step(c, st, g, action, gain, accumx, accumy, state_out, reward_out, stream);
}

int aomarl_do_control_reduced(aomarl_ctx *c, aomarl_state *st, void *stream) {
  if (!c || !st) return fail("do_control_reduced: null argument");
  auto &P = c->pipe;
  if (!(P.active && P.owner_screens == st->screens)) return aomarl_do_control(c, st, 0, st->nenv, stream);
  aomarl_state v = pipe_view(c, st, 1 - P.par);
  c->pipe_internal = true;
  const int rc = aomarl_do_control(c, &v, 0, st->nenv, stream);
  c->pipe_internal = false;
  return rc;
}

int aomarl_env_step_shortcut(aomarl_ctx *c, const aomarl_env_glue *g) {
  if (!c || !g) return 0;
  return step_plan(step_facts(c, nullptr, g, nullptr, nullptr)).tail == TAIL_SHORTCUT ? 1 : 0;
}

int aomarl_env_step(aomarl_ctx *c, aomarl_state *st, aomarl_env_glue *g, const float *action, float gain,
                    float *accumx, float *accumy, float *state_out, float *reward_out, void *stream) {
  if (!c || !st || !g || !state_out) return fail("env_step: null argument");
  const StepFacts f = step_facts(c, st, g, accumx, accumy);
  const StepPlan sp = step_plan(f);
  if (sp.route == PIPELINED)
    return env_step_pipelined(c, st, g, action, gain, accumx, accumy, state_out, reward_out, f, sp, stream);
  if (sp.route == REFUSED_IN_FLIGHT)
    return fail("env_step: a pipelined frame is in flight but this call is not eligible for the frame pipeline "
                "(options, glue or arguments changed within an episode, or aomarl_set_modal_gains): reset first");
  if (sp.route == PLAIN) return env_step_body(c, st, g, action, gain, accumx, accumy, state_out, reward_out, f, sp, stream);
  const int n = st->nenv, nl = c->nlayers;
  Plan plan;
  const bool pf = c->prefetch_atmos;
  const bool steady = stream && aomarl_frame_fused_available(c) && accumx && accumy &&
                      (pf ? (c->premoved && c->pre_screens == st->screens && c->pre_b == 0 && c->pre_n == n) : !c->premoved) &&
                      (!g->sel || (c->sel_checked == g->sel && c->sel_checked_n == g->dm_dim && c->sel_checked_nm == g->nmodes)) &&
                      g->nhist >= 0 && g->nhist <= 5 && g->ring_pos >= 0 && g->ring_pos <= g->nhist &&
                      step_plan_uniform(c, n, accumx, accumy, plan);
  if (!steady) return env_step_body(c, st, g, action, gain, accumx, accumy, state_out, reward_out, f, sp, stream);
  hipStream_t s = (hipStream_t)stream;
  int rc = 0;
  if (pf) {
    rc = side_stream(c);
    if (rc) return rc;
    if (!c->side_joined) {
      HIPCHK(hipStreamWaitEvent(s, c->ev_moved, 0));
      if (c->psf_side) HIPCHK(hipStreamWaitEvent(s, c->ev_psf, 0));
      c->side_joined = true;
    }
  } else if (c->psf_side) {
    rc = psf_wait_pending(c, stream);
    if (rc) return rc;
  }
  std::vector<long long> key;
  auto kp = [&](const void *p) { key.push_back((long long)(uintptr_t)p); };
  for (int l = 0; l < nl; l++) { key.push_back(plan.kx[l]); key.push_back(plan.ky[l]); }
  key.push_back(g->ring_pos); key.push_back(g->nhist); key.push_back(g->nmodes); key.push_back(g->dm_dim);
  key.push_back(g->n_agents); key.push_back(g->flags); key.push_back(g->denoiser_f32);
  { int gi; memcpy(&gi, &gain, sizeof(gi)); key.push_back(gi); memcpy(&gi, &g->reward_factor, sizeof(gi)); key.push_back(gi); }
  kp(st); kp(st->screens); kp(st->com); kp(st->voltage); kp(st->slopes); kp(st->work); kp(st->bincube); kp(st->strehl);
  kp(action); kp(state_out); kp(reward_out); kp(stream);
  kp(g->sel); kp(g->mean_dm); kp(g->std_dm); kp(g->mean_res); kp(g->std_res); kp(g->lohi); kp(g->modes_ring); kp(g->res_modes);
  kp(g->denoiser); kp(c->cmat); kp(c->v2m); kp(c->m2v); kp(c->freedom); kp(c->amode_inv);
  key.push_back(n); key.push_back(g_precision); key.push_back(g_gemm.split_f16 ? 1 : 0); key.push_back(c->dft_mode);
  key.push_back(pf ? 1 : 0); key.push_back(c->small_move); key.push_back(c->small_chain); key.push_back(c->residual_shortcut);
  key.push_back(c->defer_dm_shape ? 1 : 0); key.push_back(g_gemm.target_blocks); key.push_back(c->fused_debug);
  { int gi; memcpy(&gi, &c->gain, sizeof(gi)); key.push_back(gi); }
  key.push_back((long long)c->cfg_epoch); key.push_back((long long)g_cfg_epoch);
  aomarl_ctx::StepGraph *hit = nullptr;
  for (auto &sg : c->graphs)
    if (sg.key == key) { hit = &sg; break; }
  if (hit) {
    HIPCHK(hipGraphLaunch(hit->exec, s));
    for (int e = 0; e < n; e++)
      for (int l = 0; l < nl; l++) {
        const float ax = accumx[(size_t)e * nl + l] + c->deltax[l], ay = accumy[(size_t)e * nl + l] + c->deltay[l];
        accumx[(size_t)e * nl + l] = ax - (float)(int)ax;
        accumy[(size_t)e * nl + l] = ay - (float)(int)ay;
        if (e == 0) { c->frac_x[l] = ax - (float)(int)ax; c->frac_y[l] = ay - (float)(int)ay; }
      }
    g->ring_pos = (g->ring_pos + 1) % (g->nhist + 1);
    if (pf) {
      c->premoved = true; c->psf_side = true; c->side_joined = true;
      c->frame_marked = true; c->frame_wait_pending = false; c->screens_dirty_main = false;
    } else {
      c->frame_marked = false; c->screens_dirty_main = true;
    }
    for (int i = 0; i < AR_N; i++) g_arith[i] += hit->arith[i];
    memcpy(c->fw_variant, hit->fw_variant, sizeof(c->fw_variant));
    c->graph_hits++;
    return 0;
  }
  if (g_gemm.split_f16) (void)gemm_sat_counter();
  if (c->graphs.size() >= 256) {
    for (auto &sg : c->graphs) { (void)hipGraphExecDestroy(sg.exec); (void)hipGraphDestroy(sg.graph); }
    c->graphs.clear();
  }
  unsigned long long before[AR_N];
  for (int i = 0; i < AR_N; i++) before[i] = g_arith[i];
  struct Snap {
    std::vector<float> ax, ay; int ring_pos; bool premoved, psf_side, side_joined, frame_marked, frame_wait_pending, screens_dirty_main;
    float fx[AOMARL_MAX_LAYERS], fy[AOMARL_MAX_LAYERS];
  } snap;
  snap.ax.assign(accumx, accumx + (size_t)n * nl); snap.ay.assign(accumy, accumy + (size_t)n * nl);
  snap.ring_pos = g->ring_pos; snap.premoved = c->premoved; snap.psf_side = c->psf_side; snap.side_joined = c->side_joined;
  snap.frame_marked = c->frame_marked; snap.frame_wait_pending = c->frame_wait_pending; snap.screens_dirty_main = c->screens_dirty_main;
  memcpy(snap.fx, c->frac_x, sizeof(snap.fx)); memcpy(snap.fy, c->frac_y, sizeof(snap.fy));
  auto restore = [&]() {
    memcpy(accumx, snap.ax.data(), sizeof(float) * snap.ax.size()); memcpy(accumy, snap.ay.data(), sizeof(float) * snap.ay.size());
    g->ring_pos = snap.ring_pos; c->premoved = snap.premoved; c->psf_side = snap.psf_side; c->side_joined = snap.side_joined;
    c->frame_marked = snap.frame_marked; c->frame_wait_pending = snap.frame_wait_pending; c->screens_dirty_main = snap.screens_dirty_main;
    memcpy(c->frac_x, snap.fx, sizeof(snap.fx)); memcpy(c->frac_y, snap.fy, sizeof(snap.fy));
    for (int i = 0; i < AR_N; i++) g_arith[i] = before[i];
  };
  HIPCHK(hipStreamBeginCapture(s, hipStreamCaptureModeRelaxed));
  c->capturing = true; c->fork_recorded = false;
  rc = env_step_body(c, st, g, action, gain, accumx, accumy, state_out, reward_out, f, sp, stream);
  hipError_t je = hipSuccess;
  if (!rc && pf) {
    if (c->psf_side) je = hipStreamWaitEvent(s, c->ev_psf, 0);
    if (je == hipSuccess && c->premoved) je = hipStreamWaitEvent(s, c->ev_moved, 0);
  }
  c->capturing = false;
  hipGraph_t graph = nullptr;
  const hipError_t ee = hipStreamEndCapture(s, &graph);
  if (rc) { if (graph) (void)hipGraphDestroy(graph); restore(); return rc; }
  if (je != hipSuccess || ee != hipSuccess || !graph) {
    if (graph) (void)hipGraphDestroy(graph);
    restore();
    return fail("env_step: graph capture failed: %s", hipGetErrorString(je != hipSuccess ? je : ee));
  }
  if (pf) c->side_joined = true;
  aomarl_ctx::StepGraph sg;
  sg.key = key; sg.graph = graph; sg.exec = nullptr;
  for (int i = 0; i < AR_N; i++) sg.arith[i] = g_arith[i] - before[i];
  memcpy(sg.fw_variant, c->fw_variant, sizeof(sg.fw_variant));
  {
    const hipError_t ie = hipGraphInstantiate(&sg.exec, graph, nullptr, nullptr, 0);
    if (ie != hipSuccess) {
      (void)hipGraphDestroy(graph);
      restore();
      return fail("env_step: hipGraphInstantiate failed: %s", hipGetErrorString(ie));
    }
  }
  {
    const hipError_t le = hipGraphLaunch(sg.exec, s);
    if (le != hipSuccess) {
      (void)hipGraphExecDestroy(sg.exec); (void)hipGraphDestroy(graph);
      restore();
      return fail("env_step: hipGraphLaunch failed: %s", hipGetErrorString(le));
    }
  }
  c->graphs.push_back(sg);
  c->graph_captures++;
  return 0;
}

int aomarl_graph_stats(aomarl_ctx *c, unsigned long long *captures, unsigned long long *replays) {
  if (!c || !captures || !replays) return fail("graph_stats: null argument");
  *captures = c->graph_captures; *replays = c->graph_hits;
  return 0;
}
```

### ao_marl_amd/csrc/aomarl_step_plan_host.h

```cpp
#pragma once

constexpr int SMALL_NM = 512, SMALL_NA = 512, SMALL_NSL = 1024;
constexpr long long SMALL_CMAT = 65536;

struct StepFacts {
  bool unfused;
  bool one_tt;
  bool no_other_dm;
  bool defer_shape;
  int ktt;
  bool mgain, env_gain;
  bool small_opt;
  int nactu, nslope, nmodes;
  bool cmat;
  bool shortcut_opt;
  bool s2m_match;
  bool denoiser;
  bool twin, pipe_opt, owner;
  bool prefetch, delay_one, noiseless, accum, subpixel, frame_fused;
  bool in_flight;
  bool graph_step, capturing;
};

enum StepRoute { PIPELINED, REFUSED_IN_FLIGHT, PLAIN, PLAIN_MAY_REPLAY };
enum HeadKind { HEAD_STAGES, HEAD_FUSED, HEAD_SMALL };
enum SenseKind { SENSE_DENOISER, SENSE_FRAME };
enum TailKind { TAIL_STAGES, TAIL_FUSED, TAIL_SMALL, TAIL_SHORTCUT };

struct StepPlan {
  StepRoute route;
  HeadKind head;
  SenseKind sense;
  TailKind tail;
};

static inline bool step_small_fits(int nactu, int nslope, int nmodes) {
  return nactu <= SMALL_NA && nslope <= SMALL_NSL && nmodes <= SMALL_NM && (long long)nactu * nslope <= SMALL_CMAT;
}

static inline bool tail_runs_do_control(TailKind t) { return t == TAIL_STAGES || t == TAIL_FUSED; }

static inline StepPlan step_plan(const StepFacts &f) {
  const bool fused = !f.unfused && f.one_tt && (f.defer_shape || f.no_other_dm) && !f.mgain;
  const bool small = fused && f.small_opt && step_small_fits(f.nactu, f.nslope, f.nmodes) && f.cmat && !f.env_gain;
  const bool shortcut = fused && !small && !f.denoiser && f.shortcut_opt && f.s2m_match && !f.env_gain;
  const bool pipelined = fused && !f.denoiser && !f.graph_step && !f.capturing && f.defer_shape && f.twin && f.pipe_opt &&
                         f.owner && f.prefetch && f.delay_one && f.noiseless && f.accum && !f.subpixel && f.frame_fused;
  StepPlan p;
  p.head = !fused ? HEAD_STAGES : small ? HEAD_SMALL : HEAD_FUSED;
  p.sense = f.denoiser ? SENSE_DENOISER : SENSE_FRAME;
  p.tail = !fused ? TAIL_STAGES : shortcut ? TAIL_SHORTCUT : (small && !f.denoiser) ? TAIL_SMALL : TAIL_FUSED;
  p.route = pipelined ? PIPELINED
          : f.in_flight ? REFUSED_IN_FLIGHT
          : (!f.graph_step || f.capturing || f.mgain) ? PLAIN : PLAIN_MAY_REPLAY;
  return p;
}

struct DelayWeights { float wa, wb, wc; };
static inline DelayWeights delay_weights(float delay, bool ahead) {
  DelayWeights w = delay <= 1.f ? DelayWeights{1.f - delay, delay, 0.f} : DelayWeights{0.f, 2.f - delay, delay - 1.f};
  if (ahead) w = DelayWeights{w.wb, w.wc, 0.f};
  return w;
}
```

### ao_marl_amd/csrc/step_plan_host_check.cpp

```cpp
#include "aomarl_step_plan_host.h"
#include <stdio.h>
#include <string.h>

#define REQUIRE(c)                                                                       \
  do {                                                                                   \
    if (!(c)) { fprintf(stderr, "%s:%d: %s failed\n", __FILE__, __LINE__, #c); return 1; } \
  } while (0)

static const char *const kNames[24] = {"unfused", "one_tt", "no_other_dm", "defer_shape", "mgain", "env_gain", "small_opt", "fits",
                                       "cmat", "shortcut_opt", "s2m_match", "denoiser", "in_flight", "graph_step", "capturing",
                                       "twin", "pipe_opt", "owner", "prefetch", "delay_one", "noiseless", "accum", "!subpixel", "frame_fused"};
enum { CHAIN_BITS = 12, ROUTE_BITS = 3, PIPE_BITS = 9, ALL_BITS = CHAIN_BITS + ROUTE_BITS + PIPE_BITS };
static const unsigned PIPE_ALL = ((1u << PIPE_BITS) - 1) << (CHAIN_BITS + ROUTE_BITS);

static StepFacts facts(unsigned b) {
#define bit(k) (((b >> (k)) & 1u) != 0)
  StepFacts f;
  f.unfused = bit(0); f.one_tt = bit(1); f.no_other_dm = bit(2); f.defer_shape = bit(3); f.ktt = f.one_tt ? 1 : -1;
  f.mgain = bit(4); f.env_gain = bit(5); f.small_opt = bit(6);
  f.nactu = bit(7) ? 90 : SMALL_NA + 1; f.nslope = 152; f.nmodes = 85;
  f.cmat = bit(8); f.shortcut_opt = bit(9); f.s2m_match = bit(10); f.denoiser = bit(11);
  f.in_flight = bit(12); f.graph_step = bit(13); f.capturing = bit(14);
  f.twin = bit(15); f.pipe_opt = bit(16); f.owner = bit(17); f.prefetch = bit(18); f.delay_one = bit(19);
  f.noiseless = bit(20); f.accum = bit(21); f.subpixel = !bit(22); f.frame_fused = bit(23);
  return f;
#undef bit
}

static const char *const kRoute[] = {"PIPELINED", "REFUSED_IN_FLIGHT", "PLAIN", "PLAIN_MAY_REPLAY"};
static const char *const kHead[] = {"HEAD_STAGES", "HEAD_FUSED", "HEAD_SMALL"};
static const char *const kSense[] = {"SENSE_DENOISER", "SENSE_FRAME"};
static const char *const kTail[] = {"TAIL_STAGES", "TAIL_FUSED", "TAIL_SMALL", "TAIL_SHORTCUT"};

int main(int argc, char **argv) {
  const bool table = argc >= 2 && !strcmp(argv[1], "--table");
  REQUIRE(step_small_fits(SMALL_NA, 128, SMALL_NM) && !step_small_fits(SMALL_NA + 1, 1, 1));
  REQUIRE(step_small_fits(64, SMALL_NSL, 1) && !step_small_fits(1, SMALL_NSL + 1, 1) && !step_small_fits(65, SMALL_NSL, 1));
  REQUIRE(!step_small_fits(1, 1, SMALL_NM + 1) && step_small_fits(256, 256, 1) && !step_small_fits(257, 256, 1));
  REQUIRE(step_small_fits(90, 152, 85));
  const struct { float d; bool ahead; float wa, wb, wc; } dw[] = {
      {0.f, false, 1.f, 0.f, 0.f}, {0.25f, false, 0.75f, 0.25f, 0.f}, {1.f, false, 0.f, 1.f, 0.f}, {1.75f, false, 0.f, 0.25f, 0.75f},
      {2.f, false, 0.f, 0.f, 1.f}, {1.f, true, 1.f, 0.f, 0.f}, {0.25f, true, 0.25f, 0.f, 0.f}, {1.75f, true, 0.25f, 0.75f, 0.f}};
  for (const auto &t : dw) {
    const DelayWeights w = delay_weights(t.d, t.ahead);
    REQUIRE(w.wa == t.wa && w.wb == t.wb && w.wc == t.wc);
  }
  unsigned long long count = 0, seen_route[4] = {0, 0, 0, 0}, seen_head[3] = {0, 0, 0}, seen_tail[4] = {0, 0, 0, 0};
  static StepPlan chain[1u << CHAIN_BITS];
  for (unsigned b = 0; b < (1u << CHAIN_BITS); b++) chain[b] = step_plan(facts(b));
  for (unsigned b = 0; b < (1u << ALL_BITS); b++) {
    const StepFacts f = facts(b);
    const StepPlan p = step_plan(f);
    const bool fused_head = p.head != HEAD_STAGES;
    const bool pipe_conditions = (b & PIPE_ALL) == PIPE_ALL;
    count++; seen_route[p.route]++; seen_head[p.head]++; seen_tail[p.tail]++;
    REQUIRE(fused_head == (p.tail != TAIL_STAGES));
    REQUIRE(p.tail != TAIL_SMALL || p.head == HEAD_SMALL);
    if (p.tail == TAIL_SHORTCUT || p.tail == TAIL_SMALL) REQUIRE(fused_head && !f.denoiser && !f.env_gain);
    if (p.route == PIPELINED) REQUIRE(fused_head && !f.denoiser && !f.mgain && !f.graph_step && !f.capturing && pipe_conditions && f.defer_shape);
    if (f.mgain) REQUIRE(p.head == HEAD_STAGES && p.tail == TAIL_STAGES && p.route != PIPELINED && p.route != PLAIN_MAY_REPLAY);
    if (f.unfused) REQUIRE(p.head == HEAD_STAGES && p.tail == TAIL_STAGES);
    REQUIRE((p.sense == SENSE_DENOISER) == f.denoiser);
    if (p.sense == SENSE_DENOISER) REQUIRE(tail_runs_do_control(p.tail));
    REQUIRE(tail_runs_do_control(p.tail) == (p.tail == TAIL_STAGES || p.tail == TAIL_FUSED));
    REQUIRE(chain[b & ((1u << CHAIN_BITS) - 1) & ~(1u << 11)].head == p.head);
    if (fused_head && !f.denoiser && !f.env_gain && f.small_opt && f.cmat && step_small_fits(f.nactu, f.nslope, f.nmodes)) REQUIRE(p.tail == TAIL_SMALL);
    if (p.tail == TAIL_SHORTCUT) REQUIRE(p.head == HEAD_FUSED && f.shortcut_opt && f.s2m_match);
    if (p.head == HEAD_SMALL) REQUIRE(f.small_opt && f.cmat && step_small_fits(f.nactu, f.nslope, f.nmodes));
    REQUIRE((p.route == REFUSED_IN_FLIGHT) == (f.in_flight && p.route != PIPELINED));
    if (p.route == PLAIN_MAY_REPLAY) REQUIRE(f.graph_step && !f.capturing);
    if (p.route == PLAIN && !f.mgain) REQUIRE(!f.graph_step || f.capturing);
    { const StepPlan &q = chain[b & ((1u << CHAIN_BITS) - 1)]; REQUIRE(q.head == p.head && q.sense == p.sense && q.tail == p.tail); }
  }
  for (int k = 0; k < 4; k++) REQUIRE(seen_route[k] > 0 && seen_tail[k] > 0);
  for (int k = 0; k < 3; k++) REQUIRE(seen_head[k] > 0);
  if (table) {
    printf("# chain:");
    for (int k = 0; k < CHAIN_BITS; k++) printf(" %s", kNames[k]);
    printf(" -> head sense tail\n");
    for (unsigned b = 0; b < (1u << CHAIN_BITS); b++) {
      const StepPlan p = step_plan(facts(b));
      for (int k = 0; k < CHAIN_BITS; k++) putchar('0' + ((b >> k) & 1u));
      printf(" %s %s %s\n", kHead[p.head], kSense[p.sense], kTail[p.tail]);
    }
    const int rbits[9] = {0, 1, 2, 3, 4, 11, 12, 13, 14};
    printf("# route:");
    for (int k : rbits) printf(" %s", kNames[k]);
    printf(" -> the pipeline's own conditions (");
    for (int k = CHAIN_BITS + ROUTE_BITS; k < ALL_BITS; k++) printf("%s%s", kNames[k], k + 1 < ALL_BITS ? ", " : "");
    printf(") all hold | each one alone fails\n");
    for (unsigned r = 0; r < (1u << 9); r++) {
      unsigned b = 0;
      for (int k = 0; k < 9; k++) b |= ((r >> k) & 1u) << rbits[k];
      const StepRoute all = step_plan(facts(b | PIPE_ALL)).route;
      const StepRoute one = step_plan(facts((b | PIPE_ALL) & ~(1u << (CHAIN_BITS + ROUTE_BITS)))).route;
      for (int k = CHAIN_BITS + ROUTE_BITS; k < ALL_BITS; k++) REQUIRE(step_plan(facts((b | PIPE_ALL) & ~(1u << k))).route == one);
      for (unsigned o = 0; o < (1u << CHAIN_BITS); o++) {
        if (o & 0x81Fu) continue;
        REQUIRE(step_plan(facts(b | o | PIPE_ALL)).route == all && step_plan(facts((b | o | PIPE_ALL) & ~(1u << 20))).route == one);
      }
      for (int k = 0; k < 9; k++) putchar('0' + ((r >> k) & 1u));
      printf(" %s | %s\n", kRoute[all], kRoute[one]);
    }
  }
  printf("step_plan_host_check: ok (%llu combinations)\n", count);
  return 0;
}
```

### ao_marl_amd/libaomarl.py

```python
import ctypes as C
import os
import subprocess

import numpy as np

HERE = os.path.dirname(os.path.abspath(__file__))
LIB_PATH = os.environ.get("AOMARL_LIB") or os.path.join(HERE, "libaomarl_hip.so")
MAX_LAYERS, MAX_DMS, ABI_VERSION = 8, 4, 4
PRECISION_F32, PRECISION_SPLIT_F16 = 0, 1

DM_PZT, DM_TT = 0, 1
TRACE_ATMOS, TRACE_DMS, TRACE_RESET, TRACE_MASK = 1, 2, 4, 8
IMG_FROM_PHASE_BUFFER, IMG_NOISE, IMG_WRITE_BINCUBE, IMG_COG, IMG_NO_ATMOS, IMG_NO_DMS = \
    1, 2, 4, 8, 16, 32
IMG_DM_FROM_VOLTAGE = 64
APPLY_COMP_VOLTAGE, APPLY_DEFER_STACK_SHAPE = 1, 2

_fp = C.POINTER(C.c_float)
_ip = C.POINTER(C.c_int32)
_up = C.POINTER(C.c_uint32)


class DmDesc(C.Structure):
    _fields_ = [("type", C.c_int32), ("dim", C.c_int32), ("nact", C.c_int32),
                ("influsize", C.c_int32), ("ninflupos", C.c_int64), ("influ", _fp),
                ("influpos", _ip), ("ninflu", _ip), ("influstart", _ip),
                ("wfs_xoff", C.c_float), ("wfs_yoff", C.c_float), ("tar_xoff", C.c_float),
                ("tar_yoff", C.c_float)]


class LayerDesc(C.Structure):
    _fields_ = [("dim", C.c_int32), ("nstencil", C.c_int32), ("A", _fp), ("B", _fp),
                ("istx", _up), ("isty", _up), ("deltax", C.c_float), ("deltay", C.c_float),
                ("amplitude", C.c_float), ("wfs_xoff", C.c_float), ("wfs_yoff", C.c_float),
                ("tar_xoff", C.c_float), ("tar_yoff", C.c_float)]


class Desc(C.Structure):
    _fields_ = [("abi_version", C.c_int32), ("n", C.c_int32), ("pupdiam", C.c_int32),
                ("mpupil", _fp), ("spupil", _fp),
                ("nvalid", C.c_int32), ("pdiam", C.c_int32), ("nfft", C.c_int32),
                ("npix", C.c_int32), ("nrebin", C.c_int32), ("nxsub", C.c_int32),
                ("phasemap", _ip), ("halfxy", _fp), ("binmap", _ip), ("flux", _fp),
                ("validsubsx", _ip), ("validsubsy", _ip),
                ("nphot", C.c_float), ("wfs_lambda", C.c_float), ("noise", C.c_float),
                ("cog_offset", C.c_float), ("cog_scale", C.c_float), ("subapd", C.c_float),
                ("nlayers", C.c_int32), ("layers", LayerDesc * MAX_LAYERS),
                ("ndm", C.c_int32), ("dms", DmDesc * MAX_DMS),
                ("tar_lambda", C.c_float), ("npsf", C.c_int32), ("strehl_halfwin", C.c_int32),
                ("nactu", C.c_int32), ("nslope", C.c_int32), ("gain", C.c_float),
                ("delay", C.c_float)]


class State(C.Structure):
    _fields_ = [("nenv", C.c_int32), ("ld_actu", C.c_int32), ("screens", C.c_void_p),
                ("origin", C.c_void_p), ("seeds", C.c_void_p), ("ext_count", C.c_void_p),
                ("com", C.c_void_p), ("com1", C.c_void_p), ("com2", C.c_void_p),
                ("err", C.c_void_p), ("voltage", C.c_void_p), ("slopes", C.c_void_p),
                ("dm_shape", C.c_void_p), ("bincube", C.c_void_p), ("wfs_phase", C.c_void_p),
                ("tar_phase", C.c_void_p), ("strehl", C.c_void_p), ("le_img", C.c_void_p),
                ("frame", C.c_void_p), ("work", C.c_void_p)]


_vp, _i, _f = C.c_void_p, C.c_int, C.c_float
_range = [_vp, C.POINTER(State), _i, _i]
SYMBOLS = [
    ("aomarl_last_error", C.c_char_p, []),
    ("aomarl_abi_version", _i, []),
    ("aomarl_set_precision", _i, [_i]),
    ("aomarl_get_precision", _i, []),
    ("aomarl_gemm_saturated", _i, [C.POINTER(C.c_uint), _vp]),
    ("aomarl_arith_families", _i, []),
    ("aomarl_arith_family_name", C.c_char_p, [_i]),
    ("aomarl_arith_launches", C.c_ulonglong, [_i]),
    ("aomarl_arith_reset", None, []),
    ("aomarl_create", _i, [C.POINTER(Desc), C.POINTER(_vp)]),
    ("aomarl_destroy", _i, [_vp]),
    ("aomarl_set_cmat", _i, [_vp, _fp]),
    ("aomarl_set_gain", _i, [_vp, _f]),
    ("aomarl_set_env_gains", _i, [_vp, _fp, _i]),
    ("aomarl_set_modal_gains", _i, [_vp, _fp, _i, _i]),
    ("aomarl_get_modal_gains", _i, [_vp, _fp, C.POINTER(_i), C.POINTER(_i)]),
    ("aomarl_set_modal", _i, [_vp, _i, _fp, _fp, _fp, _i, _ip]),
    ("aomarl_workspace_floats", C.c_size_t, [_vp, _i]),
    ("aomarl_screen_stride", C.c_size_t, [_vp]),
    ("aomarl_dmshape_stride", C.c_size_t, [_vp]),
    ("aomarl_reset", _i, _range + [_up, _fp, _fp, _vp]),
    ("aomarl_target_image", _i, _range + [_vp, _vp]),
    ("aomarl_strehl_fit", _i, _range + [_vp]),
    ("aomarl_reset_prefetch_begin", _i, _range + [_up, _vp]),
    ("aomarl_reset_prefetch_advance", _i, [_vp, _i, _vp, C.POINTER(_i)]),
    ("aomarl_reset_prefetch_cancel", _i, [_vp]),
    ("aomarl_reset_adopt", _i, _range + [_up, _fp, _fp, _vp, _vp]),
    ("aomarl_move_atmos", _i, _range + [_fp, _fp, _vp]),
    ("aomarl_prefetch_atmos", _i, _range + [_fp, _fp, _vp]),
    ("aomarl_set_wind", _i, [_vp, _i, C.c_float, C.c_float, _i]),
    ("aomarl_set_stencil", _i, [_vp, _i, _i, _up, _i]),
    ("aomarl_set_r0", _i, [_vp, _fp, _i]),
    ("aomarl_get_layer", _i, [_vp, _i, _fp, _fp, _fp]),
    ("aomarl_extrude", _i, _range + [_i, _ip, _ip, _vp]),
    ("aomarl_get_screen", _i, _range + [_i, _vp, _vp]),
    ("aomarl_set_screen", _i, _range + [_i, _vp, _vp]),
    ("aomarl_raytrace_wfs", _i, _range + [_i, _vp]),
    ("aomarl_raytrace_target", _i, _range + [_i, _vp]),
    ("aomarl_comp_image", _i, _range + [_i, _vp]),
    ("aomarl_do_centroids", _i, _range + [_vp]),
    ("aomarl_slopes_geom", _i, _range + [_vp]),
    ("aomarl_do_control", _i, _range + [_vp]),
    ("aomarl_set_com", _i, _range + [_vp, _vp]),
    ("aomarl_rl_control", _i, _range + [_vp, _vp]),
    ("aomarl_rl_control_modes", _i, _range + [_vp, _vp, C.c_float, _vp, _vp, _vp]),
    ("aomarl_apply_control", _i, _range + [_i, _vp]),
    ("aomarl_comp_dm_shape", _i, _range + [_vp, _vp]),
    ("aomarl_get_dm_shape", _i, _range + [_i, _vp, _vp]),
    ("aomarl_set_option", _i, [_vp, C.c_char_p, _i]),
    ("aomarl_target_psf", _i, _range + [_vp]),
    ("aomarl_gemm_batched", _i, [_i, _i, _i, _i, _i, _i, _vp, _i, C.c_longlong, _vp, _i, C.c_longlong, _vp,
                                 C.c_longlong, _vp, _i, C.c_longlong, _i, _i, _vp]),
    ("aomarl_sac_layout", _i, [_vp, _vp, _vp, _vp, _vp]),
    ("aomarl_sac_create", _i, [_vp, C.POINTER(C.c_void_p)]),
    ("aomarl_sac_destroy", _i, [_vp]),
    ("aomarl_sac_update", _i, [_vp, _vp, _vp, _vp, _vp, _vp, C.c_longlong, _vp, _vp, _vp, C.c_uint32,
                               C.c_uint32, _i, _i, _vp, _vp]),
    ("aomarl_split_states", _i, [_i, _i, _i, _i, _vp, _vp, _vp, _vp]),
    ("aomarl_policy_sample", _i, [_i, _i, _i, _vp, C.c_float, C.c_float, C.c_float, C.c_float, _vp, _vp,
                                  _vp, C.c_uint32, C.c_uint32, _vp, _vp, _vp]),
    ("aomarl_assemble_state", _i, [_i, _i, C.POINTER(C.c_void_p), _ip, _ip, C.POINTER(C.c_void_p),
                                   C.POINTER(C.c_void_p), _vp, _vp]),
    ("aomarl_assemble_state_cols", _i, [_i, _i, C.POINTER(C.c_void_p), _ip, _ip, C.POINTER(C.c_void_p),
                                        C.POINTER(C.c_void_p), _vp, _vp, _vp]),
    ("aomarl_agent_rewards", _i, [_i, _i, _i, _vp, _i, _vp, C.c_float, _vp, _vp]),
    ("aomarl_actor_tiled_floats", C.c_longlong, [_i, _i, _i]),
    ("aomarl_actor_tile_weights", _i, [_i, _i, _i, _vp, _vp, _vp]),
    ("aomarl_actor_forward", _i, [_vp, _vp, _vp, C.c_uint32, C.c_uint32, _vp, _vp, _vp]),
    ("aomarl_env_step", _i, [_vp, C.POINTER(State), _vp, _vp, _f, _fp, _fp, _vp, _vp, _vp]),
    ("aomarl_policy_env_step", _i, [_vp, C.POINTER(State), _vp, _vp, _vp, _vp, C.c_uint32, C.c_uint32, _f, _fp, _fp,
                                    _vp, _vp, _vp, _vp, _vp]),
    ("aomarl_env_step_shortcut", _i, [_vp, _vp]),
    ("aomarl_do_control_reduced", _i, [_vp, C.POINTER(State), _vp]),
    ("aomarl_graph_stats", _i, [_vp, C.POINTER(C.c_ulonglong), C.POINTER(C.c_ulonglong)]),
    ("aomarl_set_frame_pipeline", _i, [_vp, C.POINTER(State), C.POINTER(State)]),
    ("aomarl_frame_pipeline_state", _i, [_vp, C.POINTER(_i), C.POINTER(_i), C.POINTER(C.c_ulonglong),
                                         C.POINTER(C.c_ulonglong)]),
    ("aomarl_frame_kernel_name", C.c_char_p, [_vp]),
    ("aomarl_frame_kernel_time", _i, [_vp, C.POINTER(C.c_double), C.POINTER(_i)]),
    ("aomarl_denoiser_create", _i, [C.POINTER(_fp), C.POINTER(_fp), C.POINTER(C.c_void_p)]),
    ("aomarl_denoiser_apply", _i, [_vp, _vp, C.c_longlong, _vp]),
    ("aomarl_denoiser_apply_f32", _i, [_vp, _vp, C.c_longlong, _vp]),
    ("aomarl_denoiser_apply_split_f16", _i, [_vp, _vp, C.c_longlong, _vp]),
    ("aomarl_denoiser_overflow", _i, [_vp, C.POINTER(C.c_uint), _vp]),
    ("aomarl_denoiser_destroy", _i, [_vp]),
    ("aomarl_denoiser_trainer_create", _i, [C.POINTER(_fp), C.POINTER(_fp), C.c_double, C.c_double, C.c_double,
                                            C.c_double, _i, C.POINTER(C.c_void_p)]),
    ("aomarl_denoiser_trainer_destroy", _i, [_vp]),
    ("aomarl_denoiser_trainer_step", _i, [_vp, _vp, _vp, C.c_longlong, _vp, _vp]),
    ("aomarl_denoiser_trainer_grads", _i, [_vp, _vp, _vp, C.c_longlong, C.POINTER(C.c_void_p),
                                           C.POINTER(C.c_void_p), _vp, _vp]),
    ("aomarl_denoiser_trainer_get", _i, [_vp, C.POINTER(C.c_void_p), C.POINTER(C.c_void_p), _vp]),
    ("aomarl_roket_create", _i, [_vp, C.POINTER(C.c_void_p)]),
    ("aomarl_roket_destroy", _i, [_vp]),
    ("aomarl_roket_step", _i, [_vp, _vp, _vp, _vp, _vp, _vp, _vp, _vp, _i, _vp]),
    ("aomarl_roket_moments", _i, [_vp, _vp, _vp, C.POINTER(C.c_longlong), _vp]),
    ("aomarl_roket_reset", _i, [_vp]),
    ("aomarl_roket_history", _i, [_vp, _vp, _vp, _vp]),
    ("aomarl_modopti_create", _i, [_vp, C.POINTER(C.c_void_p)]),
    ("aomarl_modopti_destroy", _i, [_vp]),
    ("aomarl_modopti_reset", _i, [_vp]),
    ("aomarl_modopti_accumulate", _i, [_vp, _vp, _i, C.c_longlong, _vp]),
    ("aomarl_modopti_result", _i, [_vp, _vp, _vp, _ip, C.POINTER(C.c_longlong), _vp]),
    ("aomarl_psfrec_create", _i, [_vp, C.POINTER(C.c_void_p)]),
    ("aomarl_psfrec_destroy", _i, [_vp]),
    ("aomarl_psfrec_accumulate", _i, [_vp, _vp, _vp, _i, _vp]),
    ("aomarl_psfrec_finish", _i, [_vp, _vp, _vp, _vp, _vp, _vp]),
    ("aomarl_psfrec_reset", _i, [_vp]),
    ("aomarl_groot_create", _i, [_vp, C.POINTER(C.c_void_p)]),
    ("aomarl_groot_destroy", _i, [_vp]),
    ("aomarl_groot_form", _i, [_vp, _vp, _vp, _vp, _i, _vp, _i, C.c_longlong, _vp]),
    ("aomarl_groot_sandwich", _i, [_vp, _vp, _i, _i, _vp, _i, _i, _vp, _i, _i, _vp]),
    ("aomarl_target_psf_buffer", _i, _range + [_vp]),
    ("aomarl_set_geo", _i, [_vp, _fp]),
    ("aomarl_geo_workspace_floats", C.c_size_t, [_vp, _i]),
    ("aomarl_geo_control", _i, _range + [_vp, _vp]),
    ("aomarl_frame_fused_available", _i, [_vp]),
    ("aomarl_dm_from_voltage_available", _i, [_vp]),
    ("aomarl_materialize_dm_shape", _i, _range + [_vp]),
    ("aomarl_frame_fused", _i, _range + [_i, _vp]),
    ("aomarl_comp_strehl", _i, _range + [_vp]),
    ("aomarl_reset_strehl", _i, _range + [_vp]),
    ("aomarl_volts2modes", _i, [_vp, C.POINTER(State), _i, _vp, _i, _vp, _vp]),
    ("aomarl_set_slopes2modes", _i, [_vp, _i, _fp]),
    ("aomarl_slopes2modes", _i, _range + [_vp, _vp]),
    ("aomarl_next_part_one", _i, _range + [_fp, _fp, _i, _vp]),
    ("aomarl_next_part_two", _i, _range + [_vp, _vp]),
    ("aomarl_gemm_nt", _i, [_i, _i, _i, _f, _vp, _i, _vp, _i, _f, _vp, _i, _vp]),
    ("aomarl_gemm_nt_split", _i, [_i, _i, _i, _f, _vp, _i, _vp, _i, _f, _vp, _i, _f, _f, _vp, C.c_longlong, _vp]),
    ("aomarl_gemm_nt_batched", _i, [_i, _i, _i, _i, _vp, _i, C.c_longlong, _vp, _i, C.c_longlong,
                                    _vp, C.c_longlong, _vp, _i, C.c_longlong, _i, _vp]),
    ("aomarl_gemm_nt_probe", _i, [_i, _i, _i, _f, _vp, _i, _vp, _i, _f, _vp, _i, _vp, C.c_longlong, _vp, _vp]),
    ("aomarl_gemm_g_probe", _i, [_vp, _vp]),
]

_lib = None


GEMM_KERNEL_P, GEMM_KERNEL_NT, GEMM_KERNEL_NT_H = 1, 2, 3
GEMM_XCD_ON, GEMM_XCD_OFF = 1, 2


class GemmProbe(C.Structure):
    _fields_ = [(n, C.c_int32) for n in ("kernel", "wm", "wn", "ksplit", "xcd", "pick_M", "slabs_only")] + \
               [("scale_a", C.c_float), ("scale_b", C.c_float)] + \
               [(n, C.c_int32) for n in ("r_kernel", "r_wm", "r_wn", "r_nz", "r_kchunk", "r_slabs")] + \
               [("r_alpha", C.c_float)] + \
               [(n, C.c_int32) for n in ("p_wm", "p_wn", "p_nz", "p_kchunk")] + \
               [(n, C.c_int32) for n in ("epi_mode", "epi_ldcom", "epi_nact")] + [("epi_gain", C.c_float)] + \
               [(n, C.c_void_p) for n in ("epi_com", "epi_gain_row", "epi_action", "epi_amode_inv", "epi_freedom")] + \
               [("r_fused", C.c_int32)]


class GemmGArgs(C.Structure):
    _fields_ = [(n, C.c_int32) for n in ("groups", "ak", "bk", "M", "N", "K")] + \
               [("A", C.c_void_p), ("lda", C.c_int32), ("sA", C.c_longlong),
                ("B", C.c_void_p), ("ldb", C.c_int32), ("sB", C.c_longlong),
                ("C", C.c_void_p), ("ldc", C.c_int32), ("sC", C.c_longlong),
                ("bias", C.c_void_p), ("sBias", C.c_longlong), ("relu", C.c_int32),
                ("mask", C.c_void_p), ("ldm", C.c_int32), ("sM", C.c_longlong),
                ("colsum", C.c_void_p), ("sCs", C.c_longlong),
                ("force_wm", C.c_int32), ("force_wn", C.c_int32)]


class SacDesc(C.Structure):
    _fields_ = [(n, C.c_int32) for n in ("n_agents", "batch", "in_max", "act_max", "hidden", "hidden_critic",
                                         "n_hidden",
                                         "state_dim", "action_dim")] + \
               [("state_gather", C.c_void_p), ("action_gather", C.c_void_p), ("n_act", C.c_void_p),
                ("target_entropy", C.c_void_p)] + \
               [(n, C.c_float) for n in ("gamma", "tau", "lr", "beta1", "beta2", "adam_eps", "log_sig_min",
                                         "log_sig_max", "action_scale", "action_bias")] + \
               [(n, C.c_void_p) for n in ("policy", "policy_m", "policy_v", "policy_grad", "critic",
                                          "critic_m", "critic_v", "critic_grad", "critic_target",
                                          "log_alpha", "log_alpha_m", "log_alpha_v", "log_alpha_grad",
                                          "alpha")]


class ActorDesc(C.Structure):
    _fields_ = [(n, C.c_int32) for n in ("n_agents", "nenv", "state_dim", "in_max", "act_max", "hidden",
                                         "n_hidden", "action_dim")] + \
               [("gather", C.c_void_p), ("W1", C.c_void_p), ("b1", C.c_void_p),
                ("Wh", C.POINTER(C.c_void_p)), ("bh", C.POINTER(C.c_void_p)),
                ("Whead", C.c_void_p), ("bhead", C.c_void_p), ("sc_agent", C.c_void_p),
                ("sc_local", C.c_void_p)] + \
               [(n, C.c_float) for n in ("log_sig_min", "log_sig_max", "scale", "bias")] + \
               [(n, C.c_void_p) for n in ("x", "h0", "h1", "head")] + [("flags", C.c_int32)] + \
               [("W1_tiled", C.c_void_p), ("Wh_tiled", C.POINTER(C.c_void_p)), ("Whead_tiled", C.c_void_p)]


ACTOR_LAYER_BY_LAYER = 1


class EnvGlue(C.Structure):
    _fields_ = [(n, C.c_int32) for n in ("nmodes", "dm_dim", "n_agents", "nhist", "ring_pos")] + \
               [(n, C.c_void_p) for n in ("sel", "mean_dm", "std_dm", "mean_res", "std_res", "lohi")] + \
               [("reward_factor", C.c_float), ("modes_ring", C.c_void_p), ("res_modes", C.c_void_p),
                ("denoiser", C.c_void_p), ("denoiser_f32", C.c_int32), ("flags", C.c_int32)]


ENV_STEP_UNFUSED = 1


class RoketDesc(C.Structure):
    _fields_ = [(n, C.c_int32) for n in ("nenv", "nactu", "ld_actu", "nmodes", "nfiltered", "delay")] + \
               [("g", C.c_float), ("gamma", C.c_float), ("RD", _fp), ("P", _fp), ("Btt", _fp)]


class ModoptiDesc(C.Structure):
    _fields_ = [(n, C.c_int32) for n in ("nenv", "nmodes", "ngain", "nskip")] + [("delay", C.c_float), ("gains", _fp)]


class PsfRecDesc(C.Structure):
    _fields_ = [(n, C.c_int32) for n in ("p", "N", "npts", "nactu", "ld_actu")] + \
               [("lit", _ip), ("if_data", _fp), ("if_indices", _ip), ("if_indptr", _ip), ("tt", _fp),
                ("denmask", _fp), ("mask", _fp), ("otftel", _fp)]


_dp = C.POINTER(C.c_double)
GROOT_CERR, GROOT_CALIAS_XX, GROOT_CALIAS_YY, GROOT_DCMM_XX, GROOT_DCMM_YY = range(5)


class GrootDesc(C.Structure):
    _fields_ = [(n, C.c_int32) for n in ("n_max", "batch_max", "m_max", "k_max")] + [("tabx", _dp), ("taby", _dp)]


class GrootFormDesc(C.Structure):
    _fields_ = [(n, C.c_int32) for n in ("model", "batch", "nlayers", "npts")] + [("x0", C.c_double)] + \
               [(n, _dp) for n in ("w", "sx", "sy", "L0")]


def dptr(a):
    return a.ctypes.data_as(_dp)


class AomarlError(RuntimeError):
    pass


def build(force=False):
    src_dir = os.path.join(HERE, "csrc")
    cmd = ["make", "-s", "-C", src_dir]
    if force:
        cmd.insert(1, "-B")
    subprocess.check_call(cmd)
    return LIB_PATH


def load():
    global _lib
    if _lib is not None:
        return _lib
    if not os.path.exists(LIB_PATH):
        raise AomarlError(
                "libaomarl_hip.so is missing (%s). Build it with `python -c 'import "
                "__graft_entry__ as g; g.build()'` or `make -C ao_marl_amd/csrc`. There is no CPU "
                "fallback for the product path." % LIB_PATH)
    try:
        import torch
    except ImportError:
        pass
    L = C.CDLL(LIB_PATH)
    for name, res, args in SYMBOLS:
        try:
            fn = getattr(L, name)
        except AttributeError:
            raise AomarlError("libaomarl_hip.so does not export %s" % name)
        fn.restype, fn.argtypes = res, args
    if L.aomarl_abi_version() != ABI_VERSION:
        raise AomarlError("libaomarl_hip.so ABI %d != binding %d" %
                          (L.aomarl_abi_version(), ABI_VERSION))
    _lib = L
    mode = os.environ.get("AOMARL_PRECISION", "").strip().lower()
    if mode:
        set_precision(mode)
    return L


_PRECISIONS = {"f32": PRECISION_F32, "fp32": PRECISION_F32, "split_f16": PRECISION_SPLIT_F16,
               "split-f16": PRECISION_SPLIT_F16, "fast": PRECISION_SPLIT_F16}


def set_precision(mode):
    if isinstance(mode, str):
        if mode.lower() not in _PRECISIONS:
            raise ValueError("unknown precision %r (f32 | split_f16)" % mode)
        mode = _PRECISIONS[mode.lower()]
    check(load().aomarl_set_precision(int(mode)))


def get_precision():
    return "split_f16" if load().aomarl_get_precision() == PRECISION_SPLIT_F16 else "f32"


def gemm_saturated(stream=None):
    n = C.c_uint(0)
    check(load().aomarl_gemm_saturated(C.byref(n), stream))
    return int(n.value)


def arith_launches(reset=False):
    L = load()
    out = {L.aomarl_arith_family_name(i).decode(): int(L.aomarl_arith_launches(i))
           for i in range(L.aomarl_arith_families())}
    if reset:
        L.aomarl_arith_reset()
    return out


def dtype_string(launches):
    split = sorted(k.split(":")[0] for k, v in launches.items() if v and k.endswith(":split_f16_mfma"))
    f32 = sorted(k.split(":")[0] for k, v in launches.items() if v and k.endswith(":f32_mfma"))
    if not split:
        return "f32"
    s = "f16x2-split operands (hi+lo, 22-bit mantissa), f32 accumulate in: " + ", ".join(split)
    if f32:
        s += "; f32 in: " + ", ".join(f32)
    return s + "; f32 vector arithmetic elsewhere"


def raw_stream(device):
    import torch
    idx = device.index if isinstance(device, torch.device) else torch.device(device).index
    if idx is None:
        idx = torch.cuda.current_device()
    return C.c_void_p(torch._C._cuda_getCurrentRawStream(idx))


def check(rc):
    if rc != 0:
        raise AomarlError(load().aomarl_last_error().decode("utf-8", "replace"))


def fptr(a):
    return a.ctypes.data_as(_fp)


def iptr(a):
    return a.ctypes.data_as(_ip)


# ... 178 lines not shown
```

### ao_marl_amd/sim.py

```python
import ctypes as C

import numpy as np
import torch

from . import libaomarl as la
from . import system


def _ld4(n):
    return (n + 3) & ~3


def hip_calibration_id():
    import os
    st = os.stat(la.LIB_PATH)
    return ("hip", os.path.abspath(la.LIB_PATH), int(st.st_size), int(st.st_mtime_ns), str(la.get_precision()))


class HipSim(object):
    def __init__(self, s, nenv, device="cuda:0", keep_bincube=False, keep_phase=False):
        if not torch.cuda.is_available():
            raise la.AomarlError("HipSim needs a GPU (torch.cuda.is_available() is False); the "
                                 "product path has no CPU fallback")
        self.lib = la.load()
# ... 44 lines not shown
            t[k] = torch.zeros(n, self.ld_actu, **f32)
        t["slopes"] = torch.zeros(n, s.nslope, **f32)
        t["dm_shape"] = torch.zeros(n, self.shape_stride, **f32)
        t["bincube"] = torch.zeros(n, s.nvalid, s.npix * s.npix, **f32) if self.keep_bincube \
            else None
        t["wfs_phase"] = torch.zeros(n, s.n, s.n, **f32) if self.keep_phase else None
        t["tar_phase"] = torch.zeros(n, s.pupdiam, s.pupdiam, **f32) if self.keep_phase else None
        t["strehl"] = torch.zeros(n, 8, **f32)
        t["le_img"] = torch.zeros(n, W * W, **f32)
        t["frame"] = torch.zeros(n, **i32)
        t["work"] = torch.zeros(int(self.lib.aomarl_workspace_floats(self.ctx, n)), **f32)
        self.t = t
        st = la.State()
        st.nenv, st.ld_actu = n, self.ld_actu
        for k, v in t.items():
            setattr(st, k, v.data_ptr() if v is not None else None)
        self.st = st
        self._st_ref = C.byref(st)
        self.accumx = np.zeros((n, max(s.nscreens, 1)), dtype=np.float32)
        self.accumy = np.zeros((n, max(s.nscreens, 1)), dtype=np.float32)

    def _stream(self):
        return la.raw_stream(self.device)

    def __del__(self):
        try:
            if getattr(self, "ctx", None):
                torch.cuda.synchronize(self.device)
                self.lib.aomarl_destroy(self.ctx)
                self.ctx = None
        except Exception:
            pass

    def _range(self, env_begin, env_count):
        if env_count is None:
            env_count = self.nenv - env_begin
        return env_begin, env_count

    @property
    def com(self):
        return self.t["com"][:, :self.s.nactu]

    @property
    def err(self):
        return self.t["err"][:, :self.s.nactu]

    @property
    def voltage(self):
        return self._frame_buf("voltage")[:, :self.s.nactu]

    @property
    def slopes(self):
        return self._frame_buf("slopes")

    def enable_frame_pipeline(self, on=True):
        if not on:
            la.check(self.lib.aomarl_set_frame_pipeline(self.ctx, C.byref(self.st), None))
            self._twin, self._twin_st = None, None
            return
        if getattr(self, "_twin", None) is not None:
            return
        f32 = dict(dtype=torch.float32, device=self.device)
        tw = {"voltage": torch.zeros(self.nenv, self.ld_actu, **f32),
              "slopes": torch.zeros(self.nenv, self.s.nslope, **f32),
              "dm_shape": torch.empty(self.nenv, self.shape_stride, **f32),
              "work": torch.zeros(self.t["work"].numel(), **f32)}
        st2 = la.State()
        for name, _ in la.State._fields_:
            setattr(st2, name, getattr(self.st, name))
        for k, v in tw.items():
            setattr(st2, k, v.data_ptr())
        la.check(self.lib.aomarl_set_frame_pipeline(self.ctx, C.byref(self.st), C.byref(st2)))
        self._twin, self._twin_st = tw, st2

    def frame_pipeline_state(self):
        a, b = C.c_int(0), C.c_int(0)
        n, o = C.c_ulonglong(0), C.c_ulonglong(0)
        la.check(self.lib.aomarl_frame_pipeline_state(self.ctx, C.byref(a), C.byref(b), C.byref(n), C.byref(o)))
        return bool(a.value), bool(b.value), int(n.value), int(o.value)

    def _frame_buf(self, name):
        if getattr(self, "_twin", None) is not None and self.frame_pipeline_state()[1]:
            return self._twin[name]
        return self.t[name]

    @property
    def strehl(self):
        s = self.t["strehl"]
        avg = torch.where(s[:, 4] > 0, s[:, 3] / s[:, 4].clamp(min=1), torch.zeros_like(s[:, 3]))
        return torch.stack([s[:, 0], s[:, 1], s[:, 2], avg], dim=1)

    @property
    def strehl_fit(self):
        la.check(self.lib.aomarl_strehl_fit(self.ctx, C.byref(self.st), 0, self.nenv, self._stream()))
        s = self.t["strehl"]
        avg = torch.where(s[:, 4] > 0, s[:, 3] / s[:, 4].clamp(min=1), torch.zeros_like(s[:, 3]))
        return torch.stack([s[:, 6], s[:, 7], s[:, 2], avg], dim=1)

    def dm_shape(self, k, env_begin=0, env_count=None):
        b, n = self._range(env_begin, env_count)
        self._ensure_shape()
        d = self.s.dms[k]
        out = torch.empty(n, d.dim, d.dim, dtype=torch.float32, device=self.device)
        la.check(self.lib.aomarl_get_dm_shape(self.ctx, C.byref(self.st), b, n, k,
                                              out.data_ptr(), self._stream()))
        return out

    def set_option(self, name, value):
        la.check(self.lib.aomarl_set_option(self.ctx, name.encode(), int(value)))
        if name == "prefetch_atmos":
            self.prefetch = bool(value)
        if name == "graph_step":
            self.graph_step = bool(value)
        if name == "force_unfused_frame" and value:
            self._set_defer(False)

    def dm_from_voltage_available(self):
        return bool(self.lib.aomarl_dm_from_voltage_available(self.ctx))

    def env_step(self, glue, action, gain, state_out, reward_out=None):
        want = self.defer_shape and (self._defer_on or self.dm_from_voltage_available())
        if want != self._defer_on:
            self._set_defer(want)
        ptrs = self.__dict__.get("_accum_ptrs")
        if ptrs is None or ptrs[0] is not self.accumx or ptrs[1] is not self.accumy:
            ptrs = self._accum_ptrs = (self.accumx, self.accumy, la.fptr(self.accumx), la.fptr(self.accumy))
        la.check(self.lib.aomarl_env_step(self.ctx, self._st_ref, glue._ref if hasattr(glue, "_ref") else C.byref(glue),
                                          action.data_ptr(), gain, ptrs[2], ptrs[3], state_out.data_ptr(),
                                          reward_out.data_ptr() if reward_out is not None else None,
                                          self._stream()))
        self._stale = self._defer_on
        if self.prefetch and not self.pending_atmos:
            self.pending_atmos, self._pending_range = True, (0, self.nenv)

    def policy_env_step(self, glue, desc, state, eps, seed, counter, gain, action, mean, state_out, reward_out=None):
        want = self.defer_shape and (self._defer_on or self.dm_from_voltage_available())
        if want != self._defer_on:
            self._set_defer(want)
        ptrs = self.__dict__.get("_accum_ptrs")
        if ptrs is None or ptrs[0] is not self.accumx or ptrs[1] is not self.accumy:
            ptrs = self._accum_ptrs = (self.accumx, self.accumy, la.fptr(self.accumx), la.fptr(self.accumy))
        la.check(self.lib.aomarl_policy_env_step(
                self.ctx, self._st_ref, glue._ref if hasattr(glue, "_ref") else C.byref(glue), C.byref(desc),
                state.data_ptr(), eps.data_ptr() if eps is not None else None, seed & 0xFFFFFFFF, counter & 0xFFFFFFFF,
                gain, ptrs[2], ptrs[3], action.data_ptr(), mean.data_ptr(), state_out.data_ptr(),
                reward_out.data_ptr() if reward_out is not None else None, self._stream()))
        self._stale = self._defer_on
        if self.prefetch and not self.pending_atmos:
            self.pending_atmos, self._pending_range = True, (0, self.nenv)

    def renew_frame_stream(self):
        la.check(self.lib.aomarl_set_option(self.ctx, b"renew_frame_stream", 1))

    def graph_stats(self):
        a, b = C.c_ulonglong(0), C.c_ulonglong(0)
        la.check(self.lib.aomarl_graph_stats(self.ctx, C.byref(a), C.byref(b)))
        return int(a.value), int(b.value)

    def _set_defer(self, on):
        on = bool(on)
        if on != self._defer_on:
            la.check(self.lib.aomarl_set_option(self.ctx, b"defer_dm_shape", int(on)))
            self._defer_on = on
        if not on:
            self._ensure_shape()

    def _ensure_shape(self):
        if self._stale:
            la.check(self.lib.aomarl_materialize_dm_shape(self.ctx, C.byref(self.st), 0, self.nenv,
                                                          self._stream()))
            self._stale = False

    def screen(self, layer, env_begin=0, env_count=None):
        b, n = self._range(env_begin, env_count)
        d = self.s.screen_dim[layer]
        out = torch.empty(n, d, d, dtype=torch.float32, device=self.device)
        la.check(self.lib.aomarl_get_screen(self.ctx, C.byref(self.st), b, n, layer,
                                            out.data_ptr(), self._stream()))
        return out

    def set_screen(self, layer, screens, env_begin=0, env_count=None):
        b, n = self._range(env_begin, env_count)
        d = self.s.screen_dim[layer]
        src = torch.as_tensor(screens, dtype=torch.float32, device=self.device).contiguous()
        if src.shape != (n, d, d):
            raise ValueError("screens must be [env_count, %d, %d]" % (d, d))
        la.check(self.lib.aomarl_set_screen(self.ctx, C.byref(self.st), b, n, layer,
                                            src.data_ptr(), self._stream()))

    def set_cmat(self, cmat):
        if getattr(self, "_s2m_rows", 0):
            self.set_slopes2modes(None)
        cmat = np.ascontiguousarray(cmat, dtype=np.float32)
        if cmat.shape != (self.s.nactu, self.s.nslope):
            raise ValueError("cmat must be [nactu, nslope]")
        la.check(self.lib.aomarl_set_cmat(self.ctx, la.fptr(cmat)))

    def set_gain(self, gain):
        la.check(self.lib.aomarl_set_gain(self.ctx, float(gain)))

    def set_env_gains(self, gains):
        if gains is None:
            la.check(self.lib.aomarl_set_env_gains(self.ctx, None, 0))
            return
        g = np.ascontiguousarray(gains, dtype=np.float32).reshape(-1)
        if g.size != self.nenv:
            raise ValueError("one gain per environment: expected %d, got %d" % (self.nenv, g.size))
        la.check(self.lib.aomarl_set_env_gains(self.ctx, la.fptr(g), int(g.size)))

    def set_modal_gains(self, mgain):
        if mgain is None:
            la.check(self.lib.aomarl_set_modal_gains(self.ctx, None, 0, 0))
            return
        g = np.ascontiguousarray(mgain, dtype=np.float32)
        if g.ndim == 1:
            g = g[None, :]
        if g.ndim != 2:
            raise ValueError("mgain must be [nmodes] or [nenv][nmodes], got shape %s" % (g.shape,))
        if g.shape[0] not in (1, self.nenv):
            raise ValueError("mgain: nrows = %d, expected 1 or nenv = %d" % (g.shape[0], self.nenv))
        la.check(self.lib.aomarl_set_modal_gains(self.ctx, la.fptr(g), int(g.shape[0]), int(g.shape[1])))

    def get_modal_gains(self):
        nr, nm = C.c_int(0), C.c_int(0)
        la.check(self.lib.aomarl_get_modal_gains(self.ctx, None, C.byref(nr), C.byref(nm)))
        if nr.value == 0:
            return None
        out = np.empty((nr.value, nm.value), dtype=np.float32)
        la.check(self.lib.aomarl_get_modal_gains(self.ctx, la.fptr(out), C.byref(nr), C.byref(nm)))
        return out

    def set_modal(self, v2m, m2v, freedom=None, action_modes=None):
        v2m = np.ascontiguousarray(v2m, dtype=np.float32)
        m2v = np.ascontiguousarray(m2v, dtype=np.float32)
        nm = v2m.shape[0]
        if v2m.shape != (nm, self.s.nactu) or m2v.shape != (self.s.nactu, nm):
            raise ValueError("v2m must be [nmodes, nactu] and m2v [nactu, nmodes]")
        fr = np.zeros(nm, dtype=np.float32) if freedom is None else \
            np.ascontiguousarray(freedom, dtype=np.float32)
        am = np.zeros(0, dtype=np.int32) if action_modes is None else \
            np.ascontiguousarray(np.asarray(action_modes) % nm, dtype=np.int32)
        la.check(self.lib.aomarl_set_modal(self.ctx, nm, la.fptr(v2m), la.fptr(m2v), la.fptr(fr),
                                           int(am.size), la.iptr(am) if am.size else None))
        self.nmodes, self.nact = nm, int(am.size)

    @staticmethod
    def calibration_id():
        return hip_calibration_id()

    def reload_dms(self):
        torch.cuda.synchronize(self.device)
        self._s2m_rows = 0
        self._create_ctx()
        self._alloc()

    def prefetch_reset_begin(self, seeds):
        n = self.nenv
        seeds = np.ascontiguousarray(np.broadcast_to(np.asarray(seeds, dtype=np.int64) & 0xFFFFFFFF, (n,)), dtype=np.uint32)
        if getattr(self, "_rp", None) is None:
            f32, i32 = dict(dtype=torch.float32, device=self.device), dict(dtype=torch.int32, device=self.device)
            t = {"screens": torch.zeros(n, self.screen_stride, **f32), "origin": torch.zeros_like(self.t["origin"]),
                 "seeds": torch.zeros(n, **i32), "ext_count": torch.zeros_like(self.t["ext_count"]),
                 "frame": torch.zeros(n, **i32), "work": torch.zeros(self.t["work"].numel(), **f32)}
            for k in ("com", "com1", "com2", "err", "voltage"):
                t[k] = torch.zeros(n, self.ld_actu, **f32)
            st2 = la.State()
            for name, _ in la.State._fields_:
                setattr(st2, name, getattr(self.st, name))
            for k, v in t.items():
                setattr(st2, k, v.data_ptr())
            own = torch.cuda.Stream(device=self.device) if getattr(self, "rp_own_stream", False) else None
            self._rp = dict(t=t, st=st2, stream=own, seeds=None, left=0)
            torch.cuda.current_stream(self.device).synchronize()
        rp = self._rp
        if rp["stream"] is not None:
            rp["stream"].wait_stream(torch.cuda.current_stream(self.device))
        la.check(self.lib.aomarl_reset_prefetch_begin(self.ctx, C.byref(rp["st"]), 0, n, la.uptr(seeds), self._rp_stream()))
        rp["seeds"], rp["left"] = seeds.copy(), -1

    def _rp_stream(self):
        st = self._rp["stream"]
        return C.c_void_p(st.cuda_stream) if st is not None else None

    def prefetch_reset_advance(self, nrounds):
        rp = getattr(self, "_rp", None)
        if rp is None or rp["seeds"] is None or rp["left"] == 0:
            return 0
        left = C.c_int(0)
        la.check(self.lib.aomarl_reset_prefetch_advance(self.ctx, int(nrounds), self._rp_stream(), C.byref(left)))
        rp["left"] = int(left.value)
        return rp["left"]

    def prefetch_reset_pending(self, seeds=None):
        rp = getattr(self, "_rp", None)
        if rp is None or rp["seeds"] is None:
            return False
        if seeds is None:
            return True
        seeds = np.ascontiguousarray(np.broadcast_to(np.asarray(seeds, dtype=np.int64) & 0xFFFFFFFF, (self.nenv,)), dtype=np.uint32)
        return bool(np.array_equal(seeds, rp["seeds"]))

    def reset(self, seeds, env_begin=0, env_count=None):
        b, n = self._range(env_begin, env_count)
        seeds = np.ascontiguousarray(np.broadcast_to(np.asarray(seeds, dtype=np.int64) &
                                                     0xFFFFFFFF, (n,)), dtype=np.uint32)
        rp = getattr(self, "_rp", None)
# ... 452 lines not shown
```

### include/aomarl.h

```cpp
#ifndef AOMARL_H
#define AOMARL_H
#include <stddef.h>
#include <stdint.h>

#ifdef __cplusplus
extern "C" {
#endif

#define AOMARL_MAX_LAYERS 8
#define AOMARL_MAX_DMS 4
#define AOMARL_ABI_VERSION 4

enum { AOMARL_DM_PZT = 0, AOMARL_DM_TT = 1 };

enum { AOMARL_TRACE_ATMOS = 1, AOMARL_TRACE_DMS = 2, AOMARL_TRACE_RESET = 4,
       AOMARL_TRACE_MASK = 8  };
enum {
  AOMARL_IMG_FROM_PHASE_BUFFER = 1,
  AOMARL_IMG_NOISE = 2,
  AOMARL_IMG_WRITE_BINCUBE = 4,
  AOMARL_IMG_COG = 8,
  AOMARL_IMG_NO_ATMOS = 16,
  AOMARL_IMG_NO_DMS = 32,
  AOMARL_IMG_DM_FROM_VOLTAGE = 64
// ... 64 lines not shown
  float *slopes;
  float *dm_shape;
  float *bincube;
  float *wfs_phase;
  float *tar_phase;
  float *strehl;
  float *le_img;
  uint32_t *frame;
  float *work;
} aomarl_state;

typedef struct aomarl_ctx aomarl_ctx;

const char *aomarl_last_error(void);
int aomarl_abi_version(void);

enum { AOMARL_PRECISION_F32 = 0, AOMARL_PRECISION_SPLIT_F16 = 1 };
int aomarl_set_precision(int mode);
int aomarl_get_precision(void);
int aomarl_gemm_saturated(unsigned *count, void *stream);
int aomarl_arith_families(void);
const char *aomarl_arith_family_name(int family);
unsigned long long aomarl_arith_launches(int family);
void aomarl_arith_reset(void);

int aomarl_create(const aomarl_desc *desc, aomarl_ctx **out);
int aomarl_destroy(aomarl_ctx *ctx);
int aomarl_set_cmat(aomarl_ctx *ctx, const float *cmat);
int aomarl_set_gain(aomarl_ctx *ctx, float gain);
int aomarl_set_env_gains(aomarl_ctx *ctx, const float *gains, int nenv);
int aomarl_set_modal_gains(aomarl_ctx *ctx, const float *mgain, int nrows, int nmodes);
int aomarl_get_modal_gains(aomarl_ctx *ctx, float *mgain_out, int *nrows_out, int *nmodes_out);
int aomarl_set_modal(aomarl_ctx *ctx, int nmodes, const float *v2m, const float *m2v,
                     const float *freedom, int nact, const int32_t *action_modes);
size_t aomarl_workspace_floats(const aomarl_ctx *ctx, int nenv);
size_t aomarl_screen_stride(const aomarl_ctx *ctx);
size_t aomarl_dmshape_stride(const aomarl_ctx *ctx);

int aomarl_reset(aomarl_ctx *ctx, aomarl_state *st, int env_begin, int env_count,
                 const uint32_t *seeds, float *accumx, float *accumy, void *stream);

int aomarl_reset_prefetch_begin(aomarl_ctx *ctx, const aomarl_state *shadow, int env_begin, int env_count,
                                const uint32_t *seeds, void *stream);
int aomarl_reset_prefetch_advance(aomarl_ctx *ctx, int nrounds, void *stream, int *remaining);
int aomarl_reset_prefetch_cancel(aomarl_ctx *ctx);
int aomarl_reset_adopt(aomarl_ctx *ctx, aomarl_state *st, int env_begin, int env_count, const uint32_t *seeds,
                       float *accumx, float *accumy, void *prefetch_stream, void *stream);
int aomarl_move_atmos(aomarl_ctx *ctx, aomarl_state *st, int env_begin, int env_count,
                      float *accumx, float *accumy, void *stream);
int aomarl_prefetch_atmos(aomarl_ctx *ctx, aomarl_state *st, int env_begin, int env_count,
                          float *accumx, float *accumy, void *stream);
int aomarl_set_wind(aomarl_ctx *ctx, int layer, float deltax, float deltay, int mirror_stencils);
int aomarl_set_stencil(aomarl_ctx *ctx, int layer, int axis, const uint32_t *istencil, int n);
int aomarl_set_r0(aomarl_ctx *ctx, const float *amplitude, int nlayers);
int aomarl_get_layer(const aomarl_ctx *ctx, int layer, float *deltax, float *deltay, float *amplitude);
int aomarl_extrude(aomarl_ctx *ctx, aomarl_state *st, int env_begin, int env_count, int nops,
                   const int32_t *layer, const int32_t *dir, void *stream);
int aomarl_set_screen(aomarl_ctx *ctx, aomarl_state *st, int env_begin, int env_count, int layer,
                      const float *src, void *stream);
int aomarl_get_screen(aomarl_ctx *ctx, aomarl_state *st, int env_begin, int env_count, int layer,
                      float *dst, void *stream);

int aomarl_raytrace_wfs(aomarl_ctx *ctx, aomarl_state *st, int env_begin, int env_count,
                        int flags, void *stream);
int aomarl_raytrace_target(aomarl_ctx *ctx, aomarl_state *st, int env_begin, int env_count,
                           int flags, void *stream);
int aomarl_comp_image(aomarl_ctx *ctx, aomarl_state *st, int env_begin, int env_count, int flags,
                      void *stream);
int aomarl_do_centroids(aomarl_ctx *ctx, aomarl_state *st, int env_begin, int env_count,
                        void *stream);
int aomarl_slopes_geom(aomarl_ctx *ctx, aomarl_state *st, int env_begin, int env_count,
                       void *stream);
int aomarl_do_control(aomarl_ctx *ctx, aomarl_state *st, int env_begin, int env_count,
                      void *stream);
int aomarl_set_com(aomarl_ctx *ctx, aomarl_state *st, int env_begin, int env_count,
                   const float *com_dev, void *stream);
int aomarl_rl_control(aomarl_ctx *ctx, aomarl_state *st, int env_begin, int env_count,
                      const float *action_dev, void *stream);
int aomarl_rl_control_modes(aomarl_ctx *ctx, aomarl_state *st, int env_begin, int env_count,
                            const float *m0_dev, const float *m1_dev, float g,
                            const float *action_dev, float *modes_out_dev, void *stream);
int aomarl_apply_control(aomarl_ctx *ctx, aomarl_state *st, int env_begin, int env_count,
                         int comp_voltage, void *stream);
int aomarl_dm_from_voltage_available(aomarl_ctx *ctx);
int aomarl_materialize_dm_shape(aomarl_ctx *ctx, aomarl_state *st, int env_begin, int env_count,
                                void *stream);
int aomarl_comp_dm_shape(aomarl_ctx *ctx, aomarl_state *st, int env_begin, int env_count,
                         const float *volts_dev, void *stream);
int aomarl_get_dm_shape(aomarl_ctx *ctx, aomarl_state *st, int env_begin, int env_count, int k,
                        float *dst, void *stream);
int aomarl_set_option(aomarl_ctx *ctx, const char *name, int value);
int aomarl_target_psf(aomarl_ctx *ctx, aomarl_state *st, int env_begin, int env_count,
                      void *stream);
int aomarl_frame_fused_available(aomarl_ctx *ctx);
const char *aomarl_frame_kernel_name(aomarl_ctx *ctx);
int aomarl_frame_kernel_time(aomarl_ctx *ctx, double *total_ms, int *launches);
int aomarl_frame_fused(aomarl_ctx *ctx, aomarl_state *st, int env_begin, int env_count, int flags,
                       void *stream);
int aomarl_gemm_batched(int batch, int transA, int transB, int M, int N, int K, const float *A, int lda,
                        long long strideA, const float *B, int ldb, long long strideB, const float *bias,
                        long long strideBias, float *C, int ldc, long long strideC, int relu,
                        int accumulate, void *stream);
typedef struct {
  int32_t n_agents, batch, in_max, act_max, hidden, hidden_critic, n_hidden;
  int32_t state_dim, action_dim;
  const int32_t *state_gather;
  const int32_t *action_gather;
  const int32_t *n_act;
  const float *target_entropy;
  float gamma, tau, lr, beta1, beta2, adam_eps;
  float log_sig_min, log_sig_max, action_scale, action_bias;
  float *policy, *policy_m, *policy_v, *policy_grad;
  float *critic, *critic_m, *critic_v, *critic_grad, *critic_target;
  float *log_alpha, *log_alpha_m, *log_alpha_v, *log_alpha_grad, *alpha;
} aomarl_sac_desc;
typedef struct aomarl_sac aomarl_sac;
#define AOMARL_SAC_SOFT_UPDATE 1
#define AOMARL_SAC_TUNE_ALPHA 2
int aomarl_sac_layout(const aomarl_sac_desc *d, long long *policy_off, long long *critic_off,
                      long long *policy_len, long long *critic_len);
int aomarl_sac_create(const aomarl_sac_desc *d, aomarl_sac **out);
int aomarl_sac_destroy(aomarl_sac *s);
int aomarl_sac_update(aomarl_sac *s, const float *state, const float *next_state, const float *action,
                      const float *reward, const float *mask, long long replay_rows, const int64_t *idx,
                      const float *eps_next, const float *eps_pi, uint32_t seed, uint32_t counter,
                      int adam_step, int flags, float *losses, void *stream);
int aomarl_split_states(int nenv, int state_dim, int n_agents, int in_max, const int32_t *gather,
                        const float *state, float *out, void *stream);
int aomarl_policy_sample(int nenv, int act_max, int action_dim, const float *head, float log_sig_min,
                         float log_sig_max, float scale, float bias, const int32_t *sc_agent,
                         const int32_t *sc_local, const float *eps, uint32_t seed, uint32_t counter,
                         float *action, float *mean, void *stream);
int aomarl_assemble_state(int nenv, int nblocks, const float *const *src, const int32_t *ld,
                          const int32_t *dim, const float *const *mean, const float *const *std_,
                          float *out, void *stream);
int aomarl_assemble_state_cols(int nenv, int nblocks, const float *const *src, const int32_t *ld,
                          const int32_t *dim, const float *const *mean, const float *const *std_,
                          const int32_t *sel, float *out, void *stream);
int aomarl_agent_rewards(int nenv, int nmodes, int n_agents, const float *res_modes, int ld,
                         const int32_t *lohi, float factor, float *out, void *stream);
typedef struct {
  int32_t n_agents, nenv, state_dim, in_max, act_max, hidden, n_hidden, action_dim;
  const int32_t *gather;
  const float *W1, *b1;
  const float *const *Wh, *const *bh;
  const float *Whead, *bhead;
  const int32_t *sc_agent, *sc_local;
  float log_sig_min, log_sig_max, scale, bias;
  float *x, *h0, *h1, *head;
  int32_t flags;
  const float *W1_tiled;
  const float *const *Wh_tiled;
  const float *Whead_tiled;
} aomarl_actor_desc;
#define AOMARL_ACTOR_LAYER_BY_LAYER 1
long long aomarl_actor_tiled_floats(int n_agents, int N, int K);
int aomarl_actor_tile_weights(int n_agents, int N, int K, const float *src, float *dst, void *stream);
int aomarl_actor_forward(const aomarl_actor_desc *d, const float *state, const float *eps, uint32_t seed,
                         uint32_t counter, float *action, float *mean, void *stream);
typedef struct {
  int32_t nmodes, dm_dim, n_agents, nhist;
  int32_t ring_pos;
  const int32_t *sel;
  const float *mean_dm, *std_dm, *mean_res, *std_res;
  const int32_t *lohi;
  float reward_factor;
  float *modes_ring;
  float *res_modes;
  void *denoiser;
  int32_t denoiser_f32;
  int32_t flags;
} aomarl_env_glue;
#define AOMARL_ENV_STEP_UNFUSED 1
int aomarl_env_step(aomarl_ctx *ctx, aomarl_state *st, aomarl_env_glue *glue, const float *action_dev,
                    float gain, float *accumx, float *accumy, float *state_out, float *reward_out,
                    void *stream);
int aomarl_policy_env_step(aomarl_ctx *ctx, aomarl_state *st, aomarl_env_glue *glue, const aomarl_actor_desc *d,
                           const float *state_dev, const float *eps_dev, uint32_t seed, uint32_t counter, float gain,
                           float *accumx, float *accumy, float *action_dev, float *mean_dev, float *state_out,
                           float *reward_out, void *stream);
int aomarl_env_step_shortcut(aomarl_ctx *ctx, const aomarl_env_glue *glue);
int aomarl_do_control_reduced(aomarl_ctx *ctx, aomarl_state *st, void *stream);
int aomarl_graph_stats(aomarl_ctx *ctx, unsigned long long *captures, unsigned long long *replays);

int aomarl_set_frame_pipeline(aomarl_ctx *ctx, const aomarl_state *st, const aomarl_state *twin);
int aomarl_frame_pipeline_state(aomarl_ctx *ctx, int *in_flight, int *consumed_in_twin,
                                unsigned long long *steps, unsigned long long *overlapped);

typedef struct aomarl_denoiser aomarl_denoiser;
int aomarl_denoiser_create(const float *const *weights, const float *const *biases,
                           aomarl_denoiser **out);
int aomarl_denoiser_apply(aomarl_denoiser *dn, float *cube, long long nimg, void *stream);
int aomarl_denoiser_apply_f32(aomarl_denoiser *dn, float *cube, long long nimg, void *stream);
int aomarl_denoiser_apply_split_f16(aomarl_denoiser *dn, float *cube, long long nimg, void *stream);
int aomarl_denoiser_overflow(aomarl_denoiser *dn, unsigned *count, void *stream);
int aomarl_denoiser_destroy(aomarl_denoiser *dn);
typedef struct aomarl_denoiser_trainer aomarl_denoiser_trainer;
int aomarl_denoiser_trainer_create(const float *const *weights, const float *const *biases, double lr,
                                   double beta1, double beta2, double eps, int max_batch,
                                   aomarl_denoiser_trainer **out);
int aomarl_denoiser_trainer_destroy(aomarl_denoiser_trainer *tr);
int aomarl_denoiser_trainer_step(aomarl_denoiser_trainer *tr, const float *noisy, const float *clean,
                                 long long nimg, float *loss_out, void *stream);
int aomarl_denoiser_trainer_grads(aomarl_denoiser_trainer *tr, const float *noisy, const float *clean,
                                  long long nimg, float *const *grads_w, float *const *grads_b,
                                  float *loss_out, void *stream);
int aomarl_denoiser_trainer_get(aomarl_denoiser_trainer *tr, float *const *weights, float *const *biases,
                                void *stream);
typedef struct {
  int32_t nenv, nactu, ld_actu, nmodes, nfiltered, delay;
  float g, gamma;
  const float *RD, *P, *Btt;
} aomarl_roket_desc;
typedef struct aomarl_roket aomarl_roket;
int aomarl_roket_create(const aomarl_roket_desc *desc, aomarl_roket **out);
int aomarl_roket_destroy(aomarl_roket *r);
int aomarl_roket_step(aomarl_roket *r, const float *derr, const float *E, const float *F, const float *ageom,
                      const float *B, const float *G, const float *rl_com, int accumulate, void *stream);
int aomarl_roket_moments(aomarl_roket *r, double *S1_out, double *S2_out, long long *frames_out, void *stream);
int aomarl_roket_reset(aomarl_roket *r);
int aomarl_roket_history(aomarl_roket *r, float *x_out, float *bufs_out, void *stream);
typedef struct {
  int32_t nenv, nmodes, ngain, nskip;
  float delay;
  const float *gains;
} aomarl_modopti_desc;
typedef struct aomarl_modopti aomarl_modopti;
int aomarl_modopti_create(const aomarl_modopti_desc *desc, aomarl_modopti **out);
int aomarl_modopti_destroy(aomarl_modopti *m);
int aomarl_modopti_reset(aomarl_modopti *m);
int aomarl_modopti_accumulate(aomarl_modopti *m, const float *x_dev, int nframes, long long frame_stride, void *stream);
int aomarl_modopti_result(aomarl_modopti *m, double *J_out, int32_t *argmin_out, int32_t *stable_out,
                          long long *frames_out, void *stream);
typedef struct {
  int32_t p, N, npts, nactu, ld_actu;
  const int32_t *lit;
  const float *if_data;
  const int32_t *if_indices, *if_indptr;
  const float *tt;
  const float *denmask, *mask, *otftel;
} aomarl_psfrec_desc;
typedef struct aomarl_psfrec aomarl_psfrec;
int aomarl_psfrec_create(const aomarl_psfrec_desc *desc, aomarl_psfrec **out);
int aomarl_psfrec_destroy(aomarl_psfrec *r);
int aomarl_psfrec_accumulate(aomarl_psfrec *r, const float *com, const float *w, int nk, void *stream);
int aomarl_psfrec_finish(aomarl_psfrec *r, const float *otf_other, float *dphi, float *otf2, float *psf, void *stream);
int aomarl_psfrec_reset(aomarl_psfrec *r);
typedef struct {
  int32_t n_max, batch_max, m_max, k_max;
  const double *tabx, *taby;
} aomarl_groot_desc;
#define AOMARL_GROOT_CERR 0
#define AOMARL_GROOT_CALIAS_XX 1
#define AOMARL_GROOT_CALIAS_YY 2
#define AOMARL_GROOT_DCMM_XX 3
#define AOMARL_GROOT_DCMM_YY 4
typedef struct {
  int32_t model, batch, nlayers, npts;
  double x0;
  const double *w, *sx, *sy, *L0;
} aomarl_groot_form_desc;
typedef struct aomarl_groot aomarl_groot;
int aomarl_groot_create(const aomarl_groot_desc *desc, aomarl_groot **out);
int aomarl_groot_destroy(aomarl_groot *g);
int aomarl_groot_form(aomarl_groot *g, const aomarl_groot_form_desc *f, const double *px, const double *py, int n,
                      float *out, int ldo, long long stride_o, void *stream);
int aomarl_groot_sandwich(aomarl_groot *g, const float *G, int ldg, int m, const float *C, int ldc, int n, float *out,
                          int ldo, int accumulate, void *stream);
int aomarl_target_psf_buffer(aomarl_ctx *ctx, aomarl_state *st, int env_begin, int env_count,
                             void *stream);
int aomarl_target_image(aomarl_ctx *ctx, aomarl_state *st, int env_begin, int env_count, float *out, void *stream);
int aomarl_set_geo(aomarl_ctx *ctx, const float *W);
size_t aomarl_geo_workspace_floats(aomarl_ctx *ctx, int nenv);
int aomarl_geo_control(aomarl_ctx *ctx, aomarl_state *st, int env_begin, int env_count,
                       float *work, void *stream);
int aomarl_comp_strehl(aomarl_ctx *ctx, aomarl_state *st, int env_begin, int env_count,
                       void *stream);
int aomarl_strehl_fit(aomarl_ctx *ctx, aomarl_state *st, int env_begin, int env_count, void *stream);
int aomarl_reset_strehl(aomarl_ctx *ctx, aomarl_state *st, int env_begin, int env_count,
                        void *stream);
int aomarl_volts2modes(aomarl_ctx *ctx, aomarl_state *st, int nrows, const float *vec_dev,
                       int ldvec, float *modes_dev, void *stream);
int aomarl_set_slopes2modes(aomarl_ctx *ctx, int nmodes, const float *s2m);
int aomarl_slopes2modes(aomarl_ctx *ctx, aomarl_state *st, int env_begin, int env_count, float *modes,
                        void *stream);

int aomarl_next_part_one(aomarl_ctx *ctx, aomarl_state *st, int env_begin, int env_count,
                         float *accumx, float *accumy, int image_flags, void *stream);
int aomarl_next_part_two(aomarl_ctx *ctx, aomarl_state *st, int env_begin, int env_count,
                         const float *action_dev, void *stream);

int aomarl_gemm_nt(int M, int N, int K, float alpha, const float *A, int lda, const float *B,
                   int ldb, float beta, float *C, int ldc, void *stream);

int aomarl_gemm_nt_split(int M, int N, int K, float alpha, const float *A, int lda, const float *B, int ldb,
                         float beta, float *C, int ldc, float scale_a, float scale_b, float *work,
                         long long work_floats, void *stream);

typedef struct aomarl_gemm_probe {
  int32_t kernel, wm, wn, ksplit, xcd, pick_M, slabs_only;
  float scale_a, scale_b;
  int32_t r_kernel, r_wm, r_wn, r_nz, r_kchunk, r_slabs;
  float r_alpha;
  int32_t p_wm, p_wn, p_nz, p_kchunk;
  int32_t epi_mode, epi_ldcom, epi_nact;
  float epi_gain;
  float *epi_com;
  const float *epi_gain_row, *epi_action;
  const int32_t *epi_amode_inv;
  const float *epi_freedom;
  int32_t r_fused;
} aomarl_gemm_probe;
int aomarl_gemm_nt_probe(int M, int N, int K, float alpha, const float *A, int lda, const float *B, int ldb,
                         float beta, float *C, int ldc, float *work, long long work_floats, aomarl_gemm_probe *probe,
                         void *stream);

typedef struct aomarl_gemm_g_args {
  int32_t groups, ak, bk, M, N, K;
  const float *A; int32_t lda; long long sA;
  const float *B; int32_t ldb; long long sB;
  float *C; int32_t ldc; long long sC;
  const float *bias; long long sBias;
  int32_t relu;
  const float *mask; int32_t ldm; long long sM;
  float *colsum; long long sCs;
  int32_t force_wm, force_wn;
} aomarl_gemm_g_args;
int aomarl_gemm_g_probe(const aomarl_gemm_g_args *args, void *stream);

int aomarl_gemm_nt_batched(int batch, int M, int N, int K, const float *A, int lda, long long strideA,
                           const float *B, int ldb, long long strideB, const float *bias,
                           long long strideBias, float *C, int ldc, long long strideC, int relu,
                           void *stream);

#ifdef __cplusplus
}
// ... 3 lines not shown
```

Baseline: 569,100.

## Fuse mode composition and rewards into the actor kernel epilogue; skip padded agent work

```diff
diff --git a/ao_marl_amd/agents.py b/ao_marl_amd/agents.py
--- a/ao_marl_amd/agents.py
+++ b/ao_marl_amd/agents.py
@@ -160,6 +160,8 @@
         self.gen = torch.Generator(device=dev).manual_seed(seed)
         self.gather_i32 = self.gather.to(torch.int32).contiguous()
         self.sc_agent_i32, self.sc_local_i32 = self.sc_agent.to(torch.int32), self.sc_local.to(torch.int32)
+        self.agent_in_i32 = torch.tensor(ins, dtype=torch.int32, device=dev)
+        self.agent_nact_i32 = torch.tensor(acts, dtype=torch.int32, device=dev)
         self.seed, self._draws = int(seed), 0
         self._native = None
         self.use_native = self.device.type == "cuda"
@@ -235,6 +237,7 @@
         for k, t in scratch.items():
             setattr(d, k, t.data_ptr())
         d.flags = la.ACTOR_LAYER_BY_LAYER if self.layer_by_layer else 0
+        d.agent_in, d.agent_nact = self.agent_in_i32.data_ptr(), self.agent_nact_i32.data_ptr()
         tiled = None
         if not self.layer_by_layer and H % 16 == 0:
             tiled = dict(W1=la.tile_weights(n["W1"]), Wh=[la.tile_weights(w) for w in n["Wh"]],
diff --git a/ao_marl_amd/csrc/aomarl_capi.hip b/ao_marl_amd/csrc/aomarl_capi.hip
--- a/ao_marl_amd/csrc/aomarl_capi.hip
+++ b/ao_marl_amd/csrc/aomarl_capi.hip
@@ -41,6 +41,8 @@
   int small_chain = 1;
   hipEvent_t ride_ev = nullptr;
   bool rode = false;
+  unsigned long long epilogue_steps = 0;
+  int actor_epilogue = 0;
   int residual_shortcut = 0;
   int small_move = 1;
   bool small_ok = false;
diff --git a/ao_marl_amd/csrc/aomarl_capi_agents.hip b/ao_marl_amd/csrc/aomarl_capi_agents.hip
--- a/ao_marl_amd/csrc/aomarl_capi_agents.hip
+++ b/ao_marl_amd/csrc/aomarl_capi_agents.hip
@@ -33,6 +33,12 @@
   const float *state, *eps;
   uint32_t seed, counter;
   float *action, *mean;
+  const int32_t *agent_in, *agent_nact;
+  int compose, nm, ldm, n_agents_rew;
+  float gain, factor;
+  const float *m0, *m1, *freedom;
+  const int32_t *amodes, *amode_inv, *lohi;
+  float *modes, *mnew, *rew;
 };
 
 __global__ void k_actor_tile_weights(int N, int K, int ntile, int ksteps, const float *__restrict__ src,
@@ -52,14 +58,16 @@
   return (((col >> 4) * 64 + ((col >> 2) & 3) * 16 + row) << 2) + (col & 3);
 }
 
-__device__ __forceinline__ void af_layer(const float *__restrict__ Xs, int ksteps, const float *__restrict__ W,
-                                         const float *__restrict__ b, int N, bool relu, float *__restrict__ Out) {
+template <class Keep>
+__device__ __forceinline__ void af_layer(const float *__restrict__ Xs, int ksteps, int kstride, const float *__restrict__ W,
+                                         const float *__restrict__ b, int N, bool relu, float *__restrict__ Out, Keep keep) {
   const int lane = threadIdx.x & 63, wave = threadIdx.x >> 6, r = lane & 15, kk = lane >> 4;
   const int ntile = (N + 15) / 16, npairs = (ntile + 1) / 2;
   constexpr int D = 2;
   for (int pair = wave; pair < npairs; pair += 8) {
-    const float4 *wa = reinterpret_cast<const float4 *>(W) + (long long)(2 * pair) * ksteps * 64 + lane;
-    const float4 *wb = reinterpret_cast<const float4 *>(W) + (long long)min(2 * pair + 1, ntile - 1) * ksteps * 64 + lane;
+    if (!keep(pair)) continue;
+    const float4 *wa = reinterpret_cast<const float4 *>(W) + (long long)(2 * pair) * kstride * 64 + lane;
+    const float4 *wb = reinterpret_cast<const float4 *>(W) + (long long)min(2 * pair + 1, ntile - 1) * kstride * 64 + lane;
     const float4 *xs = reinterpret_cast<const float4 *>(Xs) + lane;
     f32x4 acc0 = {0.f, 0.f, 0.f, 0.f}, acc1 = {0.f, 0.f, 0.f, 0.f};
     auto fma8 = [&](const float4 x, const float4 a, const float4 c) {
@@ -126,13 +134,28 @@
   const int H = p.H, no = 2 * p.act_max;
   const int ks1 = (p.in_max + 15) / 16, ksh = H / 16, nth = H / 16, nto = (no + 15) / 16;
   const int img1 = 256 * max(ksh, nto), img0 = max(256 * ks1, img1);
+  const int in_a = p.agent_in ? min(max(p.agent_in[a], 1), p.in_max) : p.in_max;
+  const int na_a = p.agent_nact ? min(max(p.agent_nact[a], 0), p.act_max) : p.act_max;
+  const int ks1a = (in_a + 15) / 16;
   float *R0 = af_lds, *R1 = af_lds + img0;
   int *alist = reinterpret_cast<int *>(af_lds + img0 + img1);
   if (tid == 0) alist[0] = 0;
   __syncthreads();
   for (int g = tid; g < p.action_dim; g += 512)
     if (p.sc_agent[g] == a) alist[1 + atomicAdd(&alist[0], 1)] = g;
-  for (int k = tid; k < 16 * ks1; k += 512) {
+  const int lane = tid & 63, wave = tid >> 6;
+  float rs[2] = {0.f, 0.f};
+  int rlo = 0, rhi = 0;
+  if (p.compose && a < p.n_agents_rew) {
+    rlo = p.lohi[2 * a]; rhi = p.lohi[2 * a + 1];
+#pragma unroll
+    for (int u = 0; u < 2; u++) {
+      const int e = e0 + wave + 8 * u;
+      if (e < p.nenv)
+        for (int m = rlo + lane; m < rhi; m += 64) { const float v = p.m1[(long long)e * p.nm + m]; rs[u] += v * v; }
+    }
+  }
+  for (int k = tid; k < 16 * ks1a; k += 512) {
     const int g = k < p.in_max ? p.gather[a * p.in_max + k] : p.state_dim;
     const bool col = g < p.state_dim;
     const float *src = p.state + (col ? g : 0);
@@ -142,31 +165,59 @@
 #pragma unroll
     for (int r = 0; r < 16; r++) R0[af_at(r, k)] = (col && e0 + r < p.nenv) ? v[r] : 0.f;
   }
+  if (p.compose && a < p.n_agents_rew) {
+#pragma unroll
+    for (int u = 0; u < 2; u++) {
+      const int e = e0 + wave + 8 * u;
+      const float s = wave_sum(rs[u]);
+      if (lane == 0 && e < p.nenv) p.rew[(long long)e * p.n_agents_rew + a] = -p.factor * s / (float)(rhi - rlo);
+    }
+  }
   __syncthreads();
-  af_layer(R0, ks1, p.W1 + (long long)a * nth * ks1 * 256, p.b1 + (long long)a * H, H, true, R1);
+  auto all = [](int) { return true; };
+  af_layer(R0, ks1a, ks1, p.W1 + (long long)a * nth * ks1 * 256, p.b1 + (long long)a * H, H, true, R1, all);
   __syncthreads();
   float *cur = R1, *nxt = R0;
   for (int l = 0; l + 1 < p.n_hidden; l++) {
-    af_layer(cur, ksh, p.Wh[l] + (long long)a * nth * ksh * 256, p.bh[l] + (long long)a * H, H, true, nxt);
+    af_layer(cur, ksh, ksh, p.Wh[l] + (long long)a * nth * ksh * 256, p.bh[l] + (long long)a * H, H, true, nxt, all);
     __syncthreads();
     float *t = cur; cur = nxt; nxt = t;
   }
-  af_layer(cur, ksh, p.Whead + (long long)a * nto * ksh * 256, p.bhead + (long long)a * no, no, false, nxt);
+  const int am = p.act_max;
+  af_layer(cur, ksh, ksh, p.Whead + (long long)a * nto * ksh * 256, p.bhead + (long long)a * no, no, false, nxt,
+           [=](int pair) { return 32 * pair < na_a || (32 * pair < am + na_a && 32 * pair + 32 > am); });
   __syncthreads();
   const int r = tid & 15, e = e0 + r;
-  if (e >= p.nenv) return;
-  const int nact = min(alist[0], p.act_max);
-  for (int i = tid >> 4; i < nact; i += 32) {
-    const int g = alist[1 + i];
-    const int l = p.sc_local[g];
-    const float m = nxt[af_at(r, l)];
-    const float ls = fminf(fmaxf(nxt[af_at(r, p.act_max + l)], p.ls_min), p.ls_max);
-    const float eps = p.eps ? p.eps[(long long)e * p.action_dim + g]
-                            : philox_normal(p.seed, 7u, p.counter, (uint32_t)e, (uint32_t)g);
-    const float x = m + expf(ls) * eps;
-    p.action[(long long)e * p.action_dim + g] = tanhf(x) * p.scale + p.bias;
-    p.mean[(long long)e * p.action_dim + g] = tanhf(m) * p.scale + p.bias;
-  }
+  if (e < p.nenv) {
+    const int nact = min(alist[0], p.act_max);
+    for (int i = tid >> 4; i < nact; i += 32) {
+      const int g = alist[1 + i];
+      const int l = p.sc_local[g];
+      const float m = nxt[af_at(r, l)];
+      const float ls = fminf(fmaxf(nxt[af_at(r, p.act_max + l)], p.ls_min), p.ls_max);
+      const float eps = p.eps ? p.eps[(long long)e * p.action_dim + g]
+                              : philox_normal(p.seed, 7u, p.counter, (uint32_t)e, (uint32_t)g);
+      const float x = m + expf(ls) * eps;
+      const float act = tanhf(x) * p.scale + p.bias;
+      p.action[(long long)e * p.action_dim + g] = act;
+      p.mean[(long long)e * p.action_dim + g] = tanhf(m) * p.scale + p.bias;
+      if (p.compose) {
+        const int md = p.amodes[g];
+        float v = p.m0[(long long)e * p.nm + md] + p.gain * p.m1[(long long)e * p.nm + md];
+        v += act * p.freedom[md];
+        p.modes[(long long)e * p.ldm + md] = v;
+        p.mnew[(long long)e * p.nm + md] = v;
+      }
+    }
+  }
+  if (p.compose && a == 0)
+    for (int md = tid; md < p.nm; md += 512)
+      if (p.amode_inv[md] < 0)
+        for (int rr = 0; rr < 16 && e0 + rr < p.nenv; rr++) {
+          const float v = p.m0[(long long)(e0 + rr) * p.nm + md] + p.gain * p.m1[(long long)(e0 + rr) * p.nm + md];
+          p.modes[(long long)(e0 + rr) * p.ldm + md] = v;
+          p.mnew[(long long)(e0 + rr) * p.nm + md] = v;
+        }
 }
 
 struct StateBlocks {
diff --git a/ao_marl_amd/csrc/aomarl_capi_stages.hip b/ao_marl_amd/csrc/aomarl_capi_stages.hip
--- a/ao_marl_amd/csrc/aomarl_capi_stages.hip
+++ b/ao_marl_amd/csrc/aomarl_capi_stages.hip
@@ -64,6 +64,7 @@
   }
   if (!strcmp(name, "small_move")) { c->small_move = value != 0; return 0; }
   if (!strcmp(name, "small_chain")) { c->small_chain = value != 0; return 0; }
+  if (!strcmp(name, "actor_epilogue")) { c->actor_epilogue = value != 0; return 0; }
   if (!strcmp(name, "renew_frame_stream")) {
     auto &P = c->pipe;
     if (P.active) return fail("renew_frame_stream: a frame is in flight (reset first)");
diff --git a/ao_marl_amd/csrc/aomarl_capi_step.hip b/ao_marl_amd/csrc/aomarl_capi_step.hip
--- a/ao_marl_amd/csrc/aomarl_capi_step.hip
+++ b/ao_marl_amd/csrc/aomarl_capi_step.hip
@@ -13,22 +13,36 @@
   return 0;
 }
 
-int aomarl_actor_forward(const aomarl_actor_desc *d, const float *state, const float *eps, uint32_t seed,
-                         uint32_t counter, float *action, float *mean, void *stream) {
+static size_t actor_fused_lds(const aomarl_actor_desc *d) {
+  const int H = d->hidden;
+  if ((d->flags & AOMARL_ACTOR_LAYER_BY_LAYER) || !d->W1_tiled || !d->Whead_tiled || H % 16 != 0) return 0;
+  const int ks1 = (d->in_max + 15) / 16, nto = (2 * d->act_max + 15) / 16;
+  const size_t img1 = (size_t)256 * std::max(H / 16, nto), img0 = std::max((size_t)256 * ks1, img1);
+  const size_t lds = (img0 + img1 + d->act_max + 4) * sizeof(float);
+  return lds <= 128 * 1024 ? lds : 0;
+}
+
+struct ActorCompose {
+  int nm, ldm, n_agents_rew;
+  float gain, factor;
+  const float *m0, *m1, *freedom;
+  const int32_t *amodes, *amode_inv, *lohi;
+  float *modes, *mnew, *rew;
+};
+
+static int actor_forward_impl(const aomarl_actor_desc *d, const float *state, const float *eps, uint32_t seed,
+                              uint32_t counter, float *action, float *mean, void *stream, const ActorCompose *ep) {
   if (!d || !state || !action || !mean) return fail("actor_forward: null argument");
   if (d->n_hidden < 1 || d->n_hidden > 8) return fail("actor_forward: 1..8 hidden layers");
   const int A = d->n_agents, n = d->nenv, H = d->hidden;
-  if (A <= 0 || n <= 0) return 0;
-  if (!(d->flags & AOMARL_ACTOR_LAYER_BY_LAYER) && d->W1_tiled && d->Whead_tiled && H % 16 == 0) {
-    const int ks1 = (d->in_max + 15) / 16, nto = (2 * d->act_max + 15) / 16;
-    const size_t img1 = (size_t)256 * std::max(H / 16, nto), img0 = std::max((size_t)256 * ks1, img1);
-    const size_t lds = (img0 + img1 + d->act_max + 4) * sizeof(float);
+  if (A <= 0 || n <= 0) return ep ? fail("actor_forward: nothing to launch, but the step counts on the epilogue") : 0;
+  if (const size_t lds = actor_fused_lds(d)) {
     static bool big_lds = false;
-    if (!big_lds && lds > 64 * 1024 && lds <= 128 * 1024) {
+    if (!big_lds && lds > 64 * 1024) {
       HIPCHK(hipFuncSetAttribute(reinterpret_cast<const void *>(k_actor_fused), hipFuncAttributeMaxDynamicSharedMemorySize, 128 * 1024));
       big_lds = true;
     }
-    if (lds <= 128 * 1024) {
+    {
       ActorArgs p;
       p.A = A; p.nenv = n; p.state_dim = d->state_dim; p.in_max = d->in_max; p.act_max = d->act_max; p.H = H;
       p.n_hidden = d->n_hidden; p.action_dim = d->action_dim;
@@ -42,6 +56,13 @@
       p.Whead = d->Whead_tiled; p.bhead = d->bhead; p.sc_agent = d->sc_agent; p.sc_local = d->sc_local;
       p.ls_min = d->log_sig_min; p.ls_max = d->log_sig_max; p.scale = d->scale; p.bias = d->bias;
       p.state = state; p.eps = eps; p.seed = seed; p.counter = counter; p.action = action; p.mean = mean;
+      p.agent_in = d->agent_in; p.agent_nact = d->agent_nact;
+      p.compose = ep ? 1 : 0;
+      p.nm = ep ? ep->nm : 0; p.ldm = ep ? ep->ldm : 0; p.n_agents_rew = ep ? ep->n_agents_rew : 0;
+      p.gain = ep ? ep->gain : 0.f; p.factor = ep ? ep->factor : 0.f;
+      p.m0 = ep ? ep->m0 : nullptr; p.m1 = ep ? ep->m1 : nullptr; p.freedom = ep ? ep->freedom : nullptr;
+      p.amodes = ep ? ep->amodes : nullptr; p.amode_inv = ep ? ep->amode_inv : nullptr; p.lohi = ep ? ep->lohi : nullptr;
+      p.modes = ep ? ep->modes : nullptr; p.mnew = ep ? ep->mnew : nullptr; p.rew = ep ? ep->rew : nullptr;
       const int tiles = (n + 15) / 16, groups = (A + 7) / 8;
       hipLaunchKernelGGL(k_actor_fused, dim3(8 * tiles * groups), dim3(512), lds, (hipStream_t)stream, p);
       g_arith[AR_ACTOR_F32]++;
@@ -49,6 +70,7 @@
       return 0;
     }
   }
+  if (ep) return fail("actor_forward: the step counts on the epilogue of the one-launch actors, which do not apply");
   if (!d->x || !d->h0 || !d->h1 || !d->head) return fail("actor_forward: the layer-by-layer path needs its scratch buffers");
   int rc = aomarl_split_states(n, d->state_dim, A, d->in_max, d->gather, state, d->x, stream);
   if (rc) return rc;
@@ -68,6 +90,11 @@
   if (rc) return rc;
   return aomarl_policy_sample(n, d->act_max, d->action_dim, d->head, d->log_sig_min, d->log_sig_max, d->scale,
                               d->bias, d->sc_agent, d->sc_local, eps, seed, counter, action, mean, stream);
+}
+
+int aomarl_actor_forward(const aomarl_actor_desc *d, const float *state, const float *eps, uint32_t seed,
+                         uint32_t counter, float *action, float *mean, void *stream) {
+  return actor_forward_impl(d, state, eps, seed, counter, action, mean, stream, nullptr);
 }
 
 static int env_step_validate(aomarl_ctx *c, aomarl_state *st, aomarl_env_glue *g, const float *action, float *state_out,
@@ -245,7 +272,8 @@
 }
 
 static int env_step_head_fused(aomarl_ctx *c, aomarl_state *st, aomarl_state *stv, aomarl_env_glue *g, const float *action,
-                               float gain, float *reward_out, HeadKind head, int ktt, bool ahead, hipEvent_t psf_ev, void *stream) {
+                               float gain, float *reward_out, HeadKind head, bool composed, int ktt, bool ahead, hipEvent_t psf_ev,
+                               void *stream) {
   hipStream_t s = (hipStream_t)stream;
   const int n = st->nenv, nm = g->nmodes, R = g->nhist + 1, na = c->sys.nactu;
   const size_t slot = (size_t)n * nm;
@@ -272,10 +300,12 @@
   const int cx = (nm + 255) / 256;
   bool psf_waited = false;
   if (ahead && psf_ev) { HIPCHK(hipStreamWaitEvent(s, psf_ev, 0)); psf_waited = true; }
-  hipLaunchKernelGGL(k_compose_rewards, dim3(cx + (reward_out ? g->n_agents : 0), n), dim3(256), 0, s, nm, newest,
-                     g->res_modes, gain, action, c->nact, c->amode_inv, c->freedom, modes, w.ldm, mnew, cx,
-                     g->n_agents, g->lohi, g->reward_factor, reward_out);
-  LAUNCHCHK();
+  if (!composed) {
+    hipLaunchKernelGGL(k_compose_rewards, dim3(cx + (reward_out ? g->n_agents : 0), n), dim3(256), 0, s, nm, newest,
+                       g->res_modes, gain, action, c->nact, c->amode_inv, c->freedom, modes, w.ldm, mnew, cx,
+                       g->n_agents, g->lohi, g->reward_factor, reward_out);
+    LAUNCHCHK();
+  }
   GemmArgs ga(n, na, nm, 1.0f, modes, w.ldm, c->m2v, c->ld_m2v, 0.0f, st->com, st->ld_actu, s);
   ga.ws = st->work + w.GEMM; ga.ws_floats = w.gemm_floats; ga.slabs_only = true; ga.min_chunk = 288;
   ga.fast = true; ga.sa = 16.f; ga.sb = c->m2v_scale;
@@ -392,7 +422,7 @@
   float *newest = g->modes_ring + (size_t)g->ring_pos * slot;
   float *mnew = g->modes_ring + (size_t)((g->ring_pos + 1) % R) * slot;
   if (plan.head != HEAD_STAGES) {
-    rc = env_step_head_fused(c, st, st, g, action, gain, reward_out, plan.head, f.ktt, false, nullptr, stream);
+    rc = env_step_head_fused(c, st, st, g, action, gain, reward_out, plan.head, plan.actor_composes, f.ktt, false, nullptr, stream);
     if (rc) return rc;
   } else {
     rc = aomarl_rl_control_modes(c, st, 0, n, newest, g->res_modes, gain, action, mnew, stream);
@@ -544,7 +574,7 @@
   int rc = env_step_validate(c, st, g, action, state_out, reward_out);
   aomarl_state vq = pipe_view(c, st, q), vp = pipe_view(c, st, p);
   hipEvent_t pe = P.psf_out[q] ? P.ev_psf[q] : nullptr;
-  if (!rc) rc = env_step_head_fused(c, st, &vq, g, action, gain, reward_out, plan.head, ktt, true, pe, stream);
+  if (!rc) rc = env_step_head_fused(c, st, &vq, g, action, gain, reward_out, plan.head, plan.actor_composes, ktt, true, pe, stream);
   if (!rc && pe && !P.cmd_covers_commit && !P.cmd_covers_psf && hipStreamWaitEvent(P.fstream, pe, 0) != hipSuccess) rc = fail("frame pipeline: hipStreamWaitEvent failed");
   if (!rc) { P.psf_out[q] = false; P.cmd_covers_psf = false; rc = pipe_launch_frame(c, st, q, stream); }
   if (!rc) rc = pipe_prefetch(c, st, accumx, accumy, p, q);
@@ -609,15 +639,50 @@
   return true;
 }
 
+static int env_step_planned(aomarl_ctx *c, aomarl_state *st, aomarl_env_glue *g, const float *action, float gain,
+                            float *accumx, float *accumy, float *state_out, float *reward_out, const StepFacts &f,
+                            const StepPlan &sp, void *stream);
+
 int aomarl_policy_env_step(aomarl_ctx *c, aomarl_state *st, aomarl_env_glue *g, const aomarl_actor_desc *d,
                            const float *state, const float *eps, uint32_t seed, uint32_t counter, float gain,
                            float *accumx, float *accumy, float *action, float *mean, float *state_out,
                            float *reward_out, void *stream) {
   if (!c || !st || !g || !d || !state || !action || !mean || !state_out) return fail("policy_env_step: null argument");
   if (d->nenv != st->nenv) return fail("policy_env_step: the actors are set up for %d environments, the state has %d", d->nenv, st->nenv);
-  int rc = aomarl_actor_forward(d, state, eps, seed, counter, action, mean, stream);
-  if (rc) return rc;
-  return aomarl_env_step(c, st, g, action, gain, accumx, accumy, state_out, reward_out, stream);
+  StepFacts f = step_facts(c, st, g, accumx, accumy);
+  f.policy_actor = actor_fused_lds(d) != 0 && d->n_agents > 0 && c->nact > 0 && d->action_dim == c->nact && c->amodes &&
+                   c->amode_inv && (!reward_out || g->n_agents == d->n_agents);
+  f.epilogue_opt = c->actor_epilogue != 0;
+  const StepPlan sp = step_plan(f);
+  if (!sp.actor_composes) {
+    int rc = aomarl_actor_forward(d, state, eps, seed, counter, action, mean, stream);
+    if (rc) return rc;
+    return env_step_planned(c, st, g, action, gain, accumx, accumy, state_out, reward_out, f, sp, stream);
+  }
+  const bool internal = c->pipe_internal;
+  if (sp.route == PIPELINED) c->pipe_internal = true;
+  int rc = env_step_validate(c, st, g, action, state_out, reward_out);
+  c->pipe_internal = internal;
+  if (rc) return rc;
+  const int n = st->nenv, nm = g->nmodes, R = g->nhist + 1;
+  const size_t slot = (size_t)n * nm;
+  const Work w = work_layout(c, n);
+  ActorCompose ep;
+  ep.nm = nm; ep.ldm = w.ldm; ep.n_agents_rew = reward_out ? g->n_agents : 0;
+  ep.gain = gain; ep.factor = g->reward_factor;
+  ep.m0 = g->modes_ring + (size_t)g->ring_pos * slot; ep.m1 = g->res_modes; ep.freedom = c->freedom;
+  ep.amodes = c->amodes; ep.amode_inv = c->amode_inv; ep.lohi = g->lohi;
+  ep.modes = st->work + w.MODES; ep.mnew = g->modes_ring + (size_t)((g->ring_pos + 1) % R) * slot; ep.rew = reward_out;
+  rc = actor_forward_impl(d, state, eps, seed, counter, action, mean, stream, &ep);
+  if (rc) return rc;
+  c->epilogue_steps++;
+  return env_step_planned(c, st, g, action, gain, accumx, accumy, state_out, reward_out, f, sp, stream);
+}
+
+int aomarl_actor_epilogue_steps(aomarl_ctx *c, unsigned long long *steps) {
+  if (!c || !steps) return fail("actor_epilogue_steps: null argument");
+  *steps = c->epilogue_steps;
+  return 0;
 }
 
 int aomarl_do_control_reduced(aomarl_ctx *c, aomarl_state *st, void *stream) {
@@ -640,7 +705,12 @@
                     float *accumx, float *accumy, float *state_out, float *reward_out, void *stream) {
   if (!c || !st || !g || !state_out) return fail("env_step: null argument");
   const StepFacts f = step_facts(c, st, g, accumx, accumy);
-  const StepPlan sp = step_plan(f);
+  return env_step_planned(c, st, g, action, gain, accumx, accumy, state_out, reward_out, f, step_plan(f), stream);
+}
+
+static int env_step_planned(aomarl_ctx *c, aomarl_state *st, aomarl_env_glue *g, const float *action, float gain,
+                            float *accumx, float *accumy, float *state_out, float *reward_out, const StepFacts &f,
+                            const StepPlan &sp, void *stream) {
   if (sp.route == PIPELINED)
     return env_step_pipelined(c, st, g, action, gain, accumx, accumy, state_out, reward_out, f, sp, stream);
   if (sp.route == REFUSED_IN_FLIGHT)
diff --git a/ao_marl_amd/csrc/aomarl_step_plan_host.h b/ao_marl_amd/csrc/aomarl_step_plan_host.h
--- a/ao_marl_amd/csrc/aomarl_step_plan_host.h
+++ b/ao_marl_amd/csrc/aomarl_step_plan_host.h
@@ -20,6 +20,8 @@
   bool prefetch, delay_one, noiseless, accum, subpixel, frame_fused;
   bool in_flight;
   bool graph_step, capturing;
+  bool policy_actor = false;
+  bool epilogue_opt = false;
 };
 
 enum StepRoute { PIPELINED, REFUSED_IN_FLIGHT, PLAIN, PLAIN_MAY_REPLAY };
@@ -32,6 +34,7 @@
   HeadKind head;
   SenseKind sense;
   TailKind tail;
+  bool actor_composes;
 };
 
 static inline bool step_small_fits(int nactu, int nslope, int nmodes) {
@@ -53,6 +56,8 @@
   p.route = pipelined ? PIPELINED
           : f.in_flight ? REFUSED_IN_FLIGHT
           : (!f.graph_step || f.capturing || f.mgain) ? PLAIN : PLAIN_MAY_REPLAY;
+  p.actor_composes = f.policy_actor && f.epilogue_opt && p.head == HEAD_FUSED && !f.capturing &&
+                     (p.route == PIPELINED || p.route == PLAIN);
   return p;
 }
 
diff --git a/ao_marl_amd/csrc/step_plan_host_check.cpp b/ao_marl_amd/csrc/step_plan_host_check.cpp
--- a/ao_marl_amd/csrc/step_plan_host_check.cpp
+++ b/ao_marl_amd/csrc/step_plan_host_check.cpp
@@ -71,6 +71,15 @@
     if (p.route == PLAIN_MAY_REPLAY) REQUIRE(f.graph_step && !f.capturing);
     if (p.route == PLAIN && !f.mgain) REQUIRE(!f.graph_step || f.capturing);
     { const StepPlan &q = chain[b & ((1u << CHAIN_BITS) - 1)]; REQUIRE(q.head == p.head && q.sense == p.sense && q.tail == p.tail); }
+    REQUIRE(!p.actor_composes);
+    for (int k = 1; k < 4; k++) {
+      StepFacts fe = f;
+      fe.policy_actor = (k & 1) != 0; fe.epilogue_opt = (k & 2) != 0;
+      const StepPlan pe = step_plan(fe);
+      REQUIRE(pe.route == p.route && pe.head == p.head && pe.sense == p.sense && pe.tail == p.tail);
+      REQUIRE(pe.actor_composes == (k == 3 && p.head == HEAD_FUSED && !f.capturing && (p.route == PIPELINED || p.route == PLAIN)));
+      if (pe.actor_composes) REQUIRE(!f.mgain && !f.unfused && !(f.graph_step && p.route != PIPELINED));
+    }
   }
   for (int k = 0; k < 4; k++) REQUIRE(seen_route[k] > 0 && seen_tail[k] > 0);
   for (int k = 0; k < 3; k++) REQUIRE(seen_head[k] > 0);
diff --git a/ao_marl_amd/libaomarl.py b/ao_marl_amd/libaomarl.py
--- a/ao_marl_amd/libaomarl.py
+++ b/ao_marl_amd/libaomarl.py
@@ -139,6 +139,7 @@
     ("aomarl_env_step_shortcut", _i, [_vp, _vp]),
     ("aomarl_do_control_reduced", _i, [_vp, C.POINTER(State), _vp]),
     ("aomarl_graph_stats", _i, [_vp, C.POINTER(C.c_ulonglong), C.POINTER(C.c_ulonglong)]),
+    ("aomarl_actor_epilogue_steps", _i, [_vp, C.POINTER(C.c_ulonglong)]),
     ("aomarl_set_frame_pipeline", _i, [_vp, C.POINTER(State), C.POINTER(State)]),
     ("aomarl_frame_pipeline_state", _i, [_vp, C.POINTER(_i), C.POINTER(_i), C.POINTER(C.c_ulonglong),
                                          C.POINTER(C.c_ulonglong)]),
@@ -252,7 +253,8 @@
                 ("sc_local", C.c_void_p)] + \
                [(n, C.c_float) for n in ("log_sig_min", "log_sig_max", "scale", "bias")] + \
                [(n, C.c_void_p) for n in ("x", "h0", "h1", "head")] + [("flags", C.c_int32)] + \
-               [("W1_tiled", C.c_void_p), ("Wh_tiled", C.POINTER(C.c_void_p)), ("Whead_tiled", C.c_void_p)]
+               [("W1_tiled", C.c_void_p), ("Wh_tiled", C.POINTER(C.c_void_p)), ("Whead_tiled", C.c_void_p),
+                ("agent_in", C.c_void_p), ("agent_nact", C.c_void_p)]
 
 
 ACTOR_LAYER_BY_LAYER = 1
diff --git a/ao_marl_amd/sim.py b/ao_marl_amd/sim.py
--- a/ao_marl_amd/sim.py
+++ b/ao_marl_amd/sim.py
@@ -220,6 +220,11 @@
     def renew_frame_stream(self):
         la.check(self.lib.aomarl_set_option(self.ctx, b"renew_frame_stream", 1))
 
+    def actor_epilogue_steps(self):
+        a = C.c_ulonglong(0)
+        la.check(self.lib.aomarl_actor_epilogue_steps(self.ctx, C.byref(a)))
+        return a.value
+
     def graph_stats(self):
         a, b = C.c_ulonglong(0), C.c_ulonglong(0)
         la.check(self.lib.aomarl_graph_stats(self.ctx, C.byref(a), C.byref(b)))
diff --git a/include/aomarl.h b/include/aomarl.h
--- a/include/aomarl.h
+++ b/include/aomarl.h
@@ -240,6 +240,7 @@
   const float *W1_tiled;
   const float *const *Wh_tiled;
   const float *Whead_tiled;
+  const int32_t *agent_in, *agent_nact;
 } aomarl_actor_desc;
 #define AOMARL_ACTOR_LAYER_BY_LAYER 1
 long long aomarl_actor_tiled_floats(int n_agents, int N, int K);
@@ -270,6 +271,7 @@
 int aomarl_env_step_shortcut(aomarl_ctx *ctx, const aomarl_env_glue *glue);
 int aomarl_do_control_reduced(aomarl_ctx *ctx, aomarl_state *st, void *stream);
 int aomarl_graph_stats(aomarl_ctx *ctx, unsigned long long *captures, unsigned long long *replays);
+int aomarl_actor_epilogue_steps(aomarl_ctx *ctx, unsigned long long *steps);
 
 int aomarl_set_frame_pipeline(aomarl_ctx *ctx, const aomarl_state *st, const aomarl_state *twin);
 int aomarl_frame_pipeline_state(aomarl_ctx *ctx, int *in_flight, int *consumed_in_twin,
```

Measured after the change: 568,900. About the same (-0.0%).
